# reilabs/gnark-whir

Measured on AMD Instinct MI355X. Metric: Groth16 proofs/sec for WHIR-verifier circuit (2^20 poly); G1 MSM pts/sec, higher is better.
Workload: dtype u32x8 Montgomery (BN254 Fr/Fp, exact modular integers)

## Files before the change

### gnark-whir_amd/binding.py

```python
from __future__ import annotations
import ctypes as C
import os
import numpy as np

_HERE = os.path.dirname(os.path.abspath(__file__))
LIB_PATH = os.environ.get("MI355X_GROTH16_LIB", os.path.join(_HERE, "libmi355x_groth16.so"))
_LIB = None

EXPORTS = [
    "mi_init", "mi_init_prio", "mi_shutdown", "mi_last_error", "mi_set_stream", "mi_pk_load", "mi_pk_load_dev", "mi_pk_free",
    "mi_ntt", "mi_ntt_dev", "mi_compute_h", "mi_compute_h_dev", "mi_msm_g1", "mi_msm_g1_dev", "mi_msm_g2",
    "mi_msm_g2_dev", "mi_groth16_prove", "mi_groth16_prove_dev", "mi_get_stats", "mi_g1_compress",
    "mi_g2_compress", "mi_proof_write", "mi_g1_sum", "mi_g2_sum", "mi_gen_scalars_dev", "mi_gen_g1_dev",
    "mi_gen_g2_dev", "mi_field_op_dev", "mi_debug_limb29_op_dev", "mi_debug_lazy_op_dev", "mi_debug_field_shape_dev", "mi_debug_pairing_dev", "mi_debug_fp12_op_dev", "mi_debug_decode_g1_dev", "mi_debug_decode_g2_dev", "mi_debug_hash_to_field_dev", "mi_debug_witness_decode_dev", "mi_debug_fp12_product_dev", "mi_debug_g1_scale128_dev", "mi_debug_g1_sum_tree_dev", "mi_debug_locate_points_dev", "mi_debug_locate_colsums_dev", "mi_debug_set_locate_round_nodes", "mi_g1_add_dev", "mi_g2_add_dev", "mi_bench_modmul_dev", "mi_bench_valu_dev", "mi_bench_gather_dev",
    "mi_dev_alloc", "mi_dev_free", "mi_dev_upload", "mi_dev_download", "mi_dev_sync",
    "mi_msm_precompute_g1_dev", "mi_msm_precompute_g2_dev", "mi_msm_g1_fixed_dev", "mi_msm_g2_fixed_dev", "mi_msm_table_to_rprime_g1_dev", "mi_msm_table_to_rprime_g2_dev", "mi_pk_table_plan",
    "mi_batch_scalar_mul_g1", "mi_batch_scalar_mul_g1_dev", "mi_batch_scalar_mul_g2", "mi_batch_scalar_mul_g2_dev",
    "mi_pedersen_pk_load", "mi_pedersen_pk_free", "mi_pedersen_commit", "mi_pedersen_prove_knowledge", "mi_pedersen_fold",
    "mi_debug_set_prove_fixed_base", "mi_debug_set_prove_schedule", "mi_debug_set_msm_batch_affine", "mi_debug_set_msm_group_bits", "mi_debug_inject_hip_failure", "mi_debug_set_ntt_plan", "mi_debug_set_ntt_threads", "mi_debug_set_ntt_wave_stages",
    "mi_debug_set_msm_plan", "mi_debug_set_msm_chunk", "mi_debug_set_msm_one_pass_sort", "mi_debug_set_msm_bound_levels", "mi_debug_set_msm_limb29", "mi_debug_set_msm_l1_waves", "mi_debug_set_msm_precompute_batched", "mi_debug_set_ntt_fuse_pair", "mi_debug_set_knob", "mi_debug_get_counter", "mi_debug_set_stream_plan", "mi_debug_set_trace_ranges", "mi_set_trace_ranges",
    "mi_prover_create", "mi_prover_destroy", "mi_prover_in_flight", "mi_prover_ctx", "mi_prover_last_error",
    "mi_prover_submit", "mi_prover_submit_dev", "mi_prover_wait", "mi_prover_commit", "mi_prover_submit_bsb22", "mi_prover_trim", "mi_ctx_trim",
    "mi_group_create", "mi_group_unique_id", "mi_group_create_rank", "mi_group_create_rank_ex", "mi_group_rank", "mi_group_destroy", "mi_group_world", "mi_group_local", "mi_group_ctx",
    "mi_group_last_error", "mi_group_transport", "mi_group_comm_ranks", "mi_group_device_pci", "mi_group_set_lead_share", "mi_group_wire_range", "mi_group_set_sharded_compute_h", "mi_compute_h_sharded_dev", "mi_groth16_prove_sharded_slices_dev", "mi_group_exchange_selftest", "mi_pk_load_sharded", "mi_pk_sharded_free",
    "mi_groth16_prove_sharded", "mi_groth16_prove_sharded_dev", "mi_pk_load_sharded_dev", "mi_msm_g1_sharded", "mi_msm_g2_sharded",
    "mi_msm_g1_sharded_dev", "mi_msm_g2_sharded_dev",
    "mi_pk_raw_inspect", "mi_pk_load_raw",
    "mi_whir_proof_decode", "mi_whir_proof_free", "mi_whir_proof_elements", "mi_whir_proof_statement_values", "mi_whir_element_shape", "mi_whir_parse_paths",
    "mi_whir_reverse", "mi_whir_prefix_decode_path", "mi_whir_limbs_to_fr", "mi_whir_interner_decode", "mi_whir_matrix_cells", "mi_whir_config_parse", "mi_whir_config_free",
]

SETUP_EXPORTS = ["mi_groth16_setup", "mi_groth16_setup_exponents", "mi_groth16_setup_get_stats"]
MAX_COMMITMENTS = 16
R1CS_EXPORTS = ["mi_r1cs_load", "mi_r1cs_free", "mi_r1cs_bytes", "mi_r1cs_eval", "mi_r1cs_eval_dev", "mi_r1cs_check_dev", "mi_r1cs_get_stats",
                "mi_groth16_prove_w", "mi_groth16_prove_w_dev", "mi_prover_submit_w", "mi_prover_submit_w_dev", "mi_prover_submit_w_bsb22"]
R1CS_A, R1CS_B, R1CS_C = 1, 2, 4
PROVE_W_EVAL_C = 1
VERIFY_EXPORTS = ["mi_vk_load", "mi_vk_free", "mi_pedersen_vk_make", "mi_groth16_verify", "mi_groth16_verify_batch"]
VERIFY_OK, VERIFY_PAIRING, VERIFY_PEDERSEN, VERIFY_MALFORMED = 0, 1, 2, 3
PAIRING_FINAL_EXP = 1
VERIFY_BYTES_EXPORTS = ["mi_vk_set_public_committed", "mi_groth16_verify_bytes", "mi_groth16_verify_bytes_batch", "mi_proof_read", "mi_hash_to_field"]
VERIFY_COMBINED_EXPORTS = ["mi_groth16_verify_combined", "mi_groth16_verify_bytes_combined"]
VERIFY_LOCATE_EXPORTS = ["mi_groth16_verify_locate", "mi_groth16_verify_bytes_locate"]
KEYFILE_EXPORTS = ["mi_g1_decompress_dev", "mi_g2_decompress_dev", "mi_g1_compress_dev", "mi_g2_compress_dev", "mi_pk_stream_inspect", "mi_pk_load_stream",
                   "mi_keyfile_get_stats", "mi_pk_stream_size", "mi_pk_write_dev", "mi_groth16_setup_to_stream"]
KEYFILE_RAW, KEYFILE_COMPRESSED = 0, 1
KEYFILE_NO_SUBGROUP_CHECK, KEYFILE_SUBGROUP_BY_R = 1, 2
NO_BAD_INDEX = (1 << 64) - 1
VKFILE_EXPORTS = ["mi_vk_stream_inspect", "mi_vk_stream_size", "mi_vk_write", "mi_vk_load_stream", "mi_groth16_setup_to_streams",
                  "mi_public_witness_write", "mi_public_witness_read", "mi_groth16_verify_files", "mi_groth16_verify_files_batch",
                  "mi_groth16_verify_files_combined", "mi_groth16_verify_files_locate"]
PHASE2_EXPORTS = ["mi_phase2_init", "mi_phase2_contribute", "mi_phase2_seal", "mi_phase2_to_streams", "mi_phase2_free", "mi_phase2_get_stats",
                  "mi_phase2_get_array"]
PHASE2_G1_A, PHASE2_G1_B, PHASE2_G2_B, PHASE2_G1_K, PHASE2_G1_Z, PHASE2_VK_K, PHASE2_BASIS = 0, 1, 2, 3, 4, 5, 6
PHASE2_CHECK_EXPORTS = ["mi_srs_check_powers", "mi_srs_check_get_stats", "mi_phase2_set_transcript_id", "mi_phase2_contribute_proved",
                        "mi_phase2_records_verify", "mi_phase2_verify_adopt", "mi_phase2_verify_get_stats"]
SRS_BAD_GENERATORS, SRS_BAD_TAU_G1, SRS_BAD_ALPHA_G1, SRS_BAD_BETA_G1, SRS_BAD_TAU_G2, SRS_BAD_BETA_G2 = 1, 2, 4, 8, 16, 32
PHASE2_BAD_RECORD, PHASE2_BAD_DELTA, PHASE2_BAD_Z, PHASE2_BAD_K = 1, 2, 4, 8
PHASE2_RECORD_WORDS = 24


class PkDesc(C.Structure):
    _fields_ = [
        ("log_n", C.c_uint32), ("nb_public", C.c_uint32), ("nb_wires", C.c_uint64),
        ("g1_a", C.c_void_p), ("n_g1_a", C.c_uint64), ("g1_b", C.c_void_p), ("n_g1_b", C.c_uint64),
        ("g1_k", C.c_void_p), ("n_g1_k", C.c_uint64), ("g1_z", C.c_void_p), ("n_g1_z", C.c_uint64),
        ("g2_b", C.c_void_p), ("n_g2_b", C.c_uint64),
        ("alpha1", C.c_uint64 * 8), ("beta1", C.c_uint64 * 8), ("delta1", C.c_uint64 * 8),
        ("beta2", C.c_uint64 * 16), ("delta2", C.c_uint64 * 16),
        ("infinity_a", C.c_void_p), ("infinity_b", C.c_void_p),
        ("committed_wires", C.c_void_p), ("n_committed", C.c_uint64),
    ]

# ... 202 lines not shown
    d.n_commitments = 0 if ped is None else int(ped.shape[0])
    d.ped = None if ped is None else ped.ctypes.data
    off = idx = None
    if lists is not None:
        off = np.cumsum([0] + [len(l) for l in lists]).astype(np.uint32)
        idx = np.array([j for l in lists for j in l], np.uint32)
        d.pc_offsets = off.ctypes.data
        d.pc_indices = idx.ctypes.data if len(idx) else None
    return d, (k, ped, off, idx)


def vk_stream_size(n_k, n_commitments=0, n_indices=0, encoding=KEYFILE_COMPRESSED):
    d = VkFileDesc(); d.n_k, d.n_commitments = int(n_k), int(n_commitments)
    off = np.array([0] * int(n_commitments) + [int(n_indices)], np.uint32); d.pc_offsets = off.ctypes.data
    n = C.c_size_t()
    if load().mi_vk_stream_size(C.byref(d), C.c_uint32(encoding), C.byref(n)) != 0:
        raise MiError("mi_vk_stream_size refused its arguments")
    return int(n.value)


def public_witness_write(values, cap=None) -> bytes:
    v = _u64(values).reshape(-1, 4); n = v.shape[0]
    cap = 12 + 32 * n if cap is None else cap
    out = (C.c_uint8 * max(cap, 1))(); need = C.c_size_t()
    if load().mi_public_witness_write(_p(v) if n else None, C.c_size_t(n), out, C.c_size_t(cap), C.byref(need)) != 0:
        raise MiError(f"mi_public_witness_write: MI_EINVAL ({need.value} bytes needed)")
    return C.string_at(out, need.value)


def public_witness_read(data: bytes, cap=None):
    buf = (C.c_uint8 * max(len(data), 1)).from_buffer_copy(data or b"\0")
    cap = max((len(data) - 12) // 32, 0) if cap is None else cap
    out = np.zeros((max(cap, 1), 4), np.uint64); n = C.c_size_t()
    if load().mi_public_witness_read(buf, C.c_size_t(len(data)), _p(out), C.c_size_t(cap), C.byref(n)) != 0:
        raise MiError("mi_public_witness_read: MI_EINVAL")
    return out[:int(n.value)].copy()


class VerifyLocateStats(C.Structure):
    _fields_ = [("rounds", C.c_uint32), ("nodes_tested", C.c_uint64), ("judged_alone", C.c_uint64), ("malformed", C.c_uint64), ("rejected", C.c_uint64)]

    def as_dict(self):
        return {n: int(getattr(self, n)) for n, _ in self._fields_}


class Bsb22Input(C.Structure):
    _fields_ = [("key", C.c_void_p), ("values", C.c_void_p), ("n", C.c_size_t)]


class Stats(C.Structure):
    _fields_ = [(n, C.c_float) for n in ("h2d_ms", "compute_h_ms", "filter_ms", "msm_a_ms", "msm_b1_ms", "msm_k_ms",
                                         "msm_z_ms", "msm_b2_ms", "assemble_ms", "total_ms")] + [
        ("g1_accum_kernel_ms", C.c_float), ("g1_accum_pairs", C.c_uint64), ("g1_accum_launches", C.c_uint32),
        ("ntt_kernel_ms", C.c_float), ("ntt_elems", C.c_uint64), ("ntt_launches", C.c_uint32), ("g1_accum_entries", C.c_uint64), ("g1_level1_additions", C.c_uint64)]

    def as_dict(self):
        return {n: getattr(self, n) for n, _ in self._fields_}


class MiError(RuntimeError):
    pass


def load():
    global _LIB
    if _LIB is None:
        if not os.path.exists(LIB_PATH):
            raise MiError(f"{LIB_PATH} missing: run `python -c 'import __graft_entry__ as g; g.build()'`")
        _LIB = C.CDLL(LIB_PATH)
        _LIB.mi_last_error.restype = C.c_char_p
        _LIB.mi_proof_write.restype = C.c_size_t
        _LIB.mi_prover_last_error.restype = C.c_char_p
        _LIB.mi_prover_ctx.restype = C.c_void_p
        _LIB.mi_prover_in_flight.restype = C.c_uint32
        _LIB.mi_group_ctx.restype = C.c_void_p
        _LIB.mi_group_last_error.restype = C.c_char_p
    return _LIB


DIST_UNIFORM, DIST_WHIR = 0, 1


def dist_mix(bit_pm, byte_pm, u64_pm=0):
    assert 0 <= bit_pm and 0 <= byte_pm and 0 <= u64_pm and bit_pm + byte_pm + u64_pm <= 1000
    return 0x40000000 | (bit_pm << 20) | (byte_pm << 10) | u64_pm


def _p(a):
    if a is None:
        return None
    if isinstance(a, np.ndarray):
        return a.ctypes.data_as(C.c_void_p)
    return C.c_void_p(int(a))


def _u64(a):
    return np.ascontiguousarray(a, dtype=np.uint64)


class DevArray:

    def __init__(self, ctx, nbytes):
        self.ctx, self.nbytes = ctx, int(nbytes)
        ptr = C.c_void_p()
        ctx._ck(ctx.lib.mi_dev_alloc(ctx.h, C.c_size_t(self.nbytes), C.byref(ptr)))
        self.ptr = ptr.value

# ... 91 lines not shown
        recs = np.ascontiguousarray(recs, dtype=np.uint32).reshape(-1, 24); n = recs.shape[0]
        di = self.to_dev(recs); do = self.alloc(max(64 * n, 32))
        self._ck(self.lib.mi_debug_lazy_op_dev(self.h, C.c_int(op), _p(do.ptr), _p(di.ptr), C.c_size_t(n)))
        out = do.download((n, 16), np.uint32) if n else np.zeros((0, 16), np.uint32)
        di.free(); do.free()
        return out

    def field_shape(self, shape, recs):
        recs = np.ascontiguousarray(recs, dtype=np.uint32).reshape(-1, 32); n = recs.shape[0]
        di = self.to_dev(recs); do = self.alloc(max(128 * n, 32))
        self._ck(self.lib.mi_debug_field_shape_dev(self.h, C.c_int(shape), _p(do.ptr), _p(di.ptr), C.c_size_t(n)))
        out = do.download((n, 32), np.uint32) if n else np.zeros((0, 32), np.uint32)
        di.free(); do.free()
        return out

    def ec_add(self, a, b, g2=False):
        a, b = _u64(a), _u64(b); n = a.shape[0]
        da, db = self.to_dev(a), self.to_dev(b); do = self.alloc(a.nbytes)
        f = self.lib.mi_g2_add_dev if g2 else self.lib.mi_g1_add_dev
        self._ck(f(self.h, _p(do.ptr), _p(da.ptr), _p(db.ptr), C.c_size_t(n)))
        out = do.download(a.shape)
        for x in (da, db, do): x.free()
        return out

    def bench_modmul(self, field, n_threads, iters):
        s = self.alloc(1024 * 32); ms = C.c_float()
        self._ck(self.lib.mi_bench_modmul_dev(self.h, field, C.c_size_t(n_threads), C.c_uint32(iters), _p(s.ptr), C.byref(ms)))
        s.free(); return ms.value

    def bench_gather(self, table_ptr, n_entries, n_threads, iters):
        s = self.alloc(1024); ms = C.c_float()
        self._ck(self.lib.mi_bench_gather_dev(self.h, _p(table_ptr), C.c_size_t(n_entries), C.c_size_t(n_threads), C.c_uint32(iters), _p(s.ptr), C.byref(ms)))
        s.free(); return ms.value

    def bench_valu(self, kind, n_threads, iters):
        s = self.alloc(1024); ms = C.c_float()
        self._ck(self.lib.mi_bench_valu_dev(self.h, kind, C.c_size_t(n_threads), C.c_uint32(iters), _p(s.ptr), C.byref(ms)))
        s.free(); return ms.value

    def ntt(self, a, log_n, flags):
        a = _u64(a).copy(); self._ck(self.lib.mi_ntt(self.h, _p(a), C.c_uint32(log_n), C.c_uint32(flags))); return a

    def ntt_dev(self, dptr, log_n, flags):
        self._ck(self.lib.mi_ntt_dev(self.h, _p(dptr), C.c_uint32(log_n), C.c_uint32(flags)))

    def compute_h(self, log_n, a, b, c):
        h = np.zeros((1 << log_n, 4), np.uint64)
        a, b, c = _u64(a), _u64(b), (None if c is None else _u64(c))
        self._ck(self.lib.mi_compute_h(self.h, C.c_uint32(log_n), _p(a), _p(b), _p(c), C.c_size_t(a.shape[0]), _p(h)))
        return h

    def compute_h_dev(self, log_n, a, b, c, n_constraints, h):
        self._ck(self.lib.mi_compute_h_dev(self.h, C.c_uint32(log_n), _p(a), _p(b), _p(c), C.c_size_t(n_constraints), _p(h)))

    def msm_g1(self, pts, sc, flags=0):
        out = np.zeros(12, np.uint64); pts, sc = _u64(pts), _u64(sc)
        self._ck(self.lib.mi_msm_g1(self.h, _p(pts), _p(sc), C.c_size_t(pts.shape[0]), C.c_uint32(flags), _p(out))); return out

    def msm_g2(self, pts, sc, flags=0):
        out = np.zeros(24, np.uint64); pts, sc = _u64(pts), _u64(sc)
        self._ck(self.lib.mi_msm_g2(self.h, _p(pts), _p(sc), C.c_size_t(pts.shape[0]), C.c_uint32(flags), _p(out))); return out

    def msm_g1_dev(self, pts_ptr, sc_ptr, n, flags=0):
        out = np.zeros(12, np.uint64)
        self._ck(self.lib.mi_msm_g1_dev(self.h, _p(pts_ptr), _p(sc_ptr), C.c_size_t(n), C.c_uint32(flags), _p(out))); return out

    def msm_g2_dev(self, pts_ptr, sc_ptr, n, flags=0):
        out = np.zeros(24, np.uint64)
        self._ck(self.lib.mi_msm_g2_dev(self.h, _p(pts_ptr), _p(sc_ptr), C.c_size_t(n), C.c_uint32(flags), _p(out))); return out

    def msm_precompute(self, base_ptr, n, c, g2=False):
        nwin = (256 + c - 1) // c
        pre = self.alloc((128 if g2 else 64) * n * nwin)
        f = self.lib.mi_msm_precompute_g2_dev if g2 else self.lib.mi_msm_precompute_g1_dev
        self._ck(f(self.h, _p(base_ptr), C.c_size_t(n), C.c_uint32(c), _p(pre.ptr)))
        return pre

    def msm_table_to_rprime(self, pre_ptr, n_points, g2=False):
        f = self.lib.mi_msm_table_to_rprime_g2_dev if g2 else self.lib.mi_msm_table_to_rprime_g1_dev
        self._ck(f(self.h, _p(pre_ptr), C.c_size_t(n_points)))

    def pk_table_plan(self, pkh):
        c = (C.c_uint32 * 3)()
        self._ck(self.lib.mi_pk_table_plan(pkh, c))
        return tuple(int(x) for x in c)

    def msm_fixed_dev(self, pre_ptr, sc_ptr, n, c, flags=0, g2=False):
        out = np.zeros(24 if g2 else 12, np.uint64)
        f = self.lib.mi_msm_g2_fixed_dev if g2 else self.lib.mi_msm_g1_fixed_dev
        self._ck(f(self.h, _p(pre_ptr), _p(sc_ptr), C.c_size_t(n), C.c_uint32(c), C.c_uint32(flags), _p(out)))
        return out

    def pk_load(self, pk: dict, device_points=False):
        d = PkDesc(); keep = []
        d.log_n, d.nb_public, d.nb_wires = pk["log_n"], pk["nb_public"], pk["nb_wires"]
        for name in ("g1_a", "g1_b", "g1_k", "g1_z", "g2_b"):
            if device_points:
                ptr, cnt = pk[name]
                setattr(d, name, int(ptr)); setattr(d, "n_" + name, int(cnt))
            else:
                arr = _u64(pk[name]); keep.append(arr)
                setattr(d, name, arr.ctypes.data); setattr(d, "n_" + name, arr.shape[0])
        for name, k in (("alpha1", 8), ("beta1", 8), ("delta1", 8), ("beta2", 16), ("delta2", 16)):
            setattr(d, name, (C.c_uint64 * k)(*[int(v) for v in _u64(pk[name]).reshape(-1)]))
        ia = np.ascontiguousarray(pk["infinity_a"], dtype=np.uint8); ib = np.ascontiguousarray(pk["infinity_b"], dtype=np.uint8)
        keep += [ia, ib]
# ... 920 lines not shown
```

### gnark-whir_amd/csrc/ctx.h

```cpp
#pragma once
#include <hip/hip_runtime.h>
#include <atomic>
#include <functional>
#include <mutex>
#include <string>
#include <vector>
#include <cstdio>
#include "../../include/mi355x_groth16.h"
#include "../../include/mi355x_groth16_group.h"
#include "../../include/mi355x_whir_ingest.h"
#include "../../include/mi355x_groth16_debug.h"
#include "../../include/mi355x_groth16_setup.h"
#include "../../include/mi355x_groth16_r1cs.h"
#include "../../include/mi355x_groth16_keyfile.h"
#include "../../include/mi355x_groth16_phase2.h"
#include "../../include/mi355x_groth16_phase2_check.h"

struct DevBuf {
    void *p = nullptr;
    size_t cap = 0;
};

enum {
    WS_H_B = 0,
    WS_H_C = 1,
    WS_HOST_IO0 = 2,
    WS_HOST_IO1 = 3,
    WS_FB_SUMS = 4,
    WS_FB_INV = 5,
    WS_R1CS_A = 6,
    WS_R1CS_B = 7,
    WS_R1CS_C = 8,
    WS_R1CS_PARTIAL = 9,
    WS_R1CS_CHECK = 10,
    WS_R1CS_W = 11,
    WS_SCAN = 12,
    WS_VERIFY = 13,
    WS_H = 14,
    WS_VERIFY_BYTES = 15,
    WS_PROVE_IN = 16,
    WS_B_WIRES = 17,
    WS_VERIFY_LOCATE = 18,
    WS_POK_VALUES = 19,
    WS_FB_TABLE = 20,
    WS_FB_SCALARS = 21,
    WS_FB_OUT = 22,
    WS_RPRIME = 23,
    WS_COUNT = 24
};
enum {
    EV_T0 = 0,
    EV_T1 = 1,
    EV_W_READY = 2,
    EV_H_READY = 3,
    EV_PROVE_BEGIN = 11,
    EV_R1CS_BEGIN = 12,
    EV_R1CS_END = 13,
    EV_COUNT = 24
};

enum {
    MSM_SLOT_A = 0,
    MSM_SLOT_B1 = 1,
    MSM_SLOT_B2 = 2,
    MSM_SLOT_K = 3,
    MSM_SLOT_Z = 4,
    MSM_SLOT_POK = 5,
    MI_MSM_SLOTS = 6
};
#define MI_ZHOOK_SLOT MSM_SLOT_Z
enum {
    MSM_EV_SORT_DONE = 0,
    MSM_EV_L1_BEGIN = 1,
    MSM_EV_L1_END = 2,
    MSM_EV_JOB_BEGIN = 3,
    MSM_EV_JOB_END = 4,
    MSM_EV_BUCKETS = 5,
    MSM_EV_MAX_LANDED = 6,
    MSM_EV_COUNT = 7
};
enum { B_DIGITS, B_H, B_S, B_SORTED, B_LEVELS, B_PART0, B_PART1, B_BUCKET, B_SCAN, B_WIN, B_PVAL, B_C1, B_CHUNKS, B_ITEMTAB, B_MAX, B_BA_NODES, B_BA_PREFIX, B_BA_TOT, B_COUNT_ };
struct MsmHostWords {
    unsigned char wsum[128][256];
    uint32_t entries, pad0_[3];
    uint32_t exact_total, pad1_[3];
    uint32_t max_bucket, pad2_[7];
};
static_assert(offsetof(MsmHostWords, entries) == sizeof(MsmHostWords::wsum) && offsetof(MsmHostWords, exact_total) == offsetof(MsmHostWords, entries) + 16 &&
              offsetof(MsmHostWords, max_bucket) == offsetof(MsmHostWords, entries) + 32 && sizeof(MsmHostWords) == 128 * 256 + 64, "the words lie where the kernels store them");
struct MsmSlot {
    hipStream_t stream = nullptr;
    hipEvent_t ev[MSM_EV_COUNT]{};
    bool max_pending = false;
    uint32_t max_key_count = 0;
    DevBuf buf[B_COUNT_];
    MsmHostWords *host_wsum = nullptr;
    uint32_t n = 0, c = 0, G = 0;
    uint64_t entries_cap = 0;
    uint64_t stat_pairs = 0;
    uint32_t nwin_keys = 0;
    uint32_t nwin_digits = 0;
    bool active = false, timed = false;
    bool deferred = false;
    uint32_t tail_seg = 0;
    const uint32_t *entries_src = nullptr;
    const std::function<hipEvent_t()> *accum_gate = nullptr;
};

struct mi_ctx {
    int dev = 0;
    hipStream_t stream = nullptr;
    bool own_stream = false;
    hipStream_t copy_stream = nullptr;
    std::string err;
    std::mutex err_m;
    mi_stats stats{};
    mi_setup_stats setup_stats{};
    mi_phase2_stats phase2_stats{};
    mi_srs_check_stats srs_check_stats{}, phase2_verify_stats{};
    mi_keyfile_stats keyfile_stats{};
    mi_r1cs_stats r1cs_stats{};
    bool r1cs_timed = false;
    hipEvent_t ev[EV_COUNT]{};
    alignas(16) unsigned char ntt_state[384];
    alignas(16) unsigned char msm_knobs[128];
    DevBuf ws[WS_COUNT];
    MsmSlot msm[MI_MSM_SLOTS];
    int cu_count = 256;
    int prio_scheme = 0;
    uint32_t fixed_knob[3] = {0, 0, 0};
    std::atomic<uint64_t> generic_sorts_two_pass{0}, generic_sorts_one_pass{0};
    std::atomic<uint64_t> dense_item_sorts{0};
    uint64_t z_count_fused_launches = 0;
    struct ZCountHook { bool armed = false, done = false; int slot = -1; uint32_t n = 0, c = 0; alignas(8) unsigned char shape[64]; uint32_t *C1 = nullptr; const void *h = nullptr;  } zhook;
    uint32_t locate_round_nodes = 0;
    uint32_t hold_accum = 0;
};

static_assert(sizeof(mi_ctx::ws) == WS_COUNT * sizeof(DevBuf) && WS_RPRIME == WS_COUNT - 1, "WS_* names every slot of mi_ctx::ws up to its end");
static_assert(EV_R1CS_END < EV_COUNT && sizeof(mi_ctx::ev) == EV_COUNT * sizeof(hipEvent_t), "EV_* index mi_ctx::ev");
static_assert(MSM_SLOT_POK == MI_MSM_SLOTS - 1 && sizeof(mi_ctx::msm) == MI_MSM_SLOTS * sizeof(MsmSlot) && MSM_EV_MAX_LANDED == MSM_EV_COUNT - 1 &&
              sizeof(MsmSlot::buf) == B_COUNT_ * sizeof(DevBuf), "MSM_SLOT_* name every slot of mi_ctx::msm, MSM_EV_* every event of a slot, B_* every workspace");

#include <atomic>
extern std::atomic<int> mi_fault_countdown;
static inline bool mi_fault_hit() {
    if (mi_fault_countdown.load(std::memory_order_relaxed) <= 0) return false;
    return mi_fault_countdown.fetch_sub(1, std::memory_order_relaxed) == 1;
}
static inline void mi_set_err(struct mi_ctx *ctx, const std::string &msg);
#define MI_CHECK_HIP(ctx, call)                                                                       \
    do {                                                                                              \
        hipError_t e__ = mi_fault_hit() ? hipErrorUnknown : (call);                                   \
        if (e__ != hipSuccess) {                                                                      \
                        \
            if (e__ == hipErrorOutOfMemory) (void)hipGetLastError();                                  \
            mi_set_err((ctx), std::string(#call) + ": " + hipGetErrorString(e__));                    \
            return e__ == hipErrorOutOfMemory ? MI_ENOMEM : MI_EHIP;                                  \
        }                                                                                             \
    } while (0)
#define MI_FAIL(ctx, code, msg)                                                                       \
    do {                                                                                              \
        mi_set_err((ctx), (msg));                                                                     \
        return (code);                                                                                \
    } while (0)
#define MI_TRY(expr)                                                                                  \
    do {                                                                                              \
        int32_t rc__ = (expr);                                                                        \
        if (rc__ != MI_OK) return rc__;                                                               \
    } while (0)

extern std::atomic<int> mi_ranges_on;
void mi_range_push(const char *name);
void mi_range_pop();
struct MiRange {
    bool on;
    explicit MiRange(const char *name) : on(mi_ranges_on.load(std::memory_order_relaxed) != 0) { if (on) mi_range_push(name); }
    ~MiRange() { if (on) mi_range_pop(); }
    MiRange(const MiRange &) = delete;
    MiRange &operator=(const MiRange &) = delete;
};
extern thread_local std::string *mi_err_sink;
static inline void mi_set_err(struct mi_ctx *ctx, const std::string &msg) {
    if (mi_err_sink) { *mi_err_sink = msg; return; }
    std::lock_guard<std::mutex> lk(ctx->err_m);
    ctx->err = msg;
}

static inline int32_t mi_reserve(mi_ctx *ctx, DevBuf &b, size_t bytes) {
    if (bytes <= b.cap) return MI_OK;
    if (b.p) { MI_CHECK_HIP(ctx, hipFree(b.p)); b.p = nullptr; b.cap = 0; }
    size_t want = bytes + bytes / 8 + 256;
    MI_CHECK_HIP(ctx, hipMalloc(&b.p, want));
    b.cap = want;
    return MI_OK;
}

static inline bool mi_try_reserve(DevBuf &b, size_t bytes) {
    if (bytes <= b.cap) return true;
    if (b.p) { (void)hipFree(b.p); b.p = nullptr; b.cap = 0; }
    const size_t want = bytes + bytes / 8 + 256;
    if (hipMalloc(&b.p, want) != hipSuccess) { (void)hipGetLastError(); b.p = nullptr; return false; }
    b.cap = want;
    return true;
}

static inline unsigned mi_blocks_of(uint64_t n, uint32_t per) { return (unsigned)((n + per - 1) / per); }

int32_t mi_copy_stream(mi_ctx *ctx, hipStream_t *out);
int32_t mi_ntt_dev_impl(mi_ctx *ctx, mi_fr *inout_dev, uint32_t log_n, uint32_t flags);
int32_t mi_compute_h_dev_impl(mi_ctx *ctx, uint32_t log_n, const mi_fr *a, const mi_fr *b, const mi_fr *c,
                              size_t n_constraints, mi_fr *h_out);
int32_t mi_compute_h_part(mi_ctx *ctx, uint32_t log_n, int part, const mi_fr *src, size_t n_constraints, mi_fr *h_out, const mi_fr *src2 = nullptr);
void mi_ntt_state_init(mi_ctx *ctx);
size_t mi_ntt_table_bytes(mi_ctx *ctx);
void mi_ntt_state_free(mi_ctx *ctx);
bool mi_ntt_set_knob(mi_ctx *ctx, const char *name, int64_t value);
void mi_ntt_state_trim(mi_ctx *ctx);
int32_t mi_msm_state_init(mi_ctx *ctx);
enum { MI_PRIO_SOLO = 0,
       MI_PRIO_POOL_FIRST = 1,
       MI_PRIO_POOL_SECOND = 2,
       MI_PRIO_POOL_REST = 3 };
void mi_msm_state_free(mi_ctx *ctx);
int32_t mi_msm_enqueue(mi_ctx *ctx, int slot, int sort_slot, int curve, const void *pts_dev, const void *scalars_dev, size_t n,
                       uint32_t flags, hipEvent_t wait_ev, bool timed, uint32_t precomp_c = 0, size_t stat_pairs = 0,
                       uint32_t generic_c = 0 );
int32_t mi_msm_precompute(mi_ctx *ctx, int curve, const void *base_dev, void *pre_dev, size_t n, uint32_t c);
int32_t mi_msm_finish(mi_ctx *ctx, int slot, int curve, void *out_xyzz_host);
int32_t mi_msm_z_count_arm(mi_ctx *ctx, int slot, size_t n, uint32_t c);
#define MI_MSM_DEFER_REDUCE 0x100u
#define MI_MSM_EXACT_SIZE 0x200u
#define MI_MSM_PTS_RPRIME 0x400u
struct MsmBucketView {
    void *bucket = nullptr;
    size_t nkeys = 0, xyzz_bytes = 0;
    uint32_t seg = 0, c = 0, nwin = 0;
    hipStream_t stream = nullptr;
    hipEvent_t ready = nullptr;
};
int32_t mi_msm_bucket_view(mi_ctx *ctx, int slot, int curve, MsmBucketView *v);
int32_t mi_msm_reduce_enqueue(mi_ctx *ctx, int slot, int curve);
bool mi_msm_limb29_enabled(mi_ctx *ctx);
uint32_t mi_msm_auto_c(size_t n);
const struct MsmCurveOps &mi_msm_ops(int curve);
```

### gnark-whir_amd/csrc/msm.hip

```cpp
#include "ctx.h"
#include "msm2_core.cuh"
#include "scan_u32.cuh"
#include "msm_curve_ops.h"
#include "key_plan.h"
#include <algorithm>
#include <cstring>
#include <cstdlib>
#include <new>

struct MsmKnobs {
    u32 c = 0, L1 = 0, L2 = 0, seg = 0, G = 0;
    u32 no_rprime = 0;
    u32 ba_rounds = 0;
    u32 l1_waves = 3;
    u32 precompute_unbatched = 0;
    u32 std_partials = 0;
    u32 one_pass_sort = 0;
    u32 chunk = 0;
    u32 gbits = 0;
    u32 bound_levels = 0;
    u32 l1_wg = 4;
    u32 g2_wg = 1;
    u32 z_waves = 0;
    u32 g1_grid_per_cu = 0, g2_grid_per_cu = 0;
// ... 212 lines not shown
__global__ void __launch_bounds__(64) k_msm_prep1_sums(MsmShape s, const u32 *S, u32 L, u32 *start, u32 *cnt, u32 *items, u32 *bucket, u32 bucket_words, u32 *block_sums) {
    size_t base = (size_t)blockIdx.x * SCAN_BLOCK + (size_t)threadIdx.x * SCAN_PER_THREAD;
    u32 sum = 0;
    for (u32 k = 0; k < SCAN_PER_THREAD; k++) {
        const u32 key = (u32)(base + k);
        if (base + k < s.nkeys) {
            msm_prep_level1(s, S, L, start, cnt, items, key);
            sum += items[key];
            if (cnt[key] == 0) {
                uint4 *b = reinterpret_cast<uint4 *>(bucket + (size_t)key * bucket_words);
                for (u32 q = 0; q < bucket_words / 4; q++) b[q] = make_uint4(0, 0, 0, 0);
            }
        }
    }
    if (blockIdx.x == 0 && threadIdx.x < 16) bucket[(size_t)s.nkeys * bucket_words + threadIdx.x] = 0;
    u32 total;
    wave_exclusive_scan(sum, &total);
    if (threadIdx.x == 0) block_sums[blockIdx.x] = total;
}
__global__ void __launch_bounds__(64) k_msm_finish_list(u32 nkeys, const u32 *items, u32 small_max, u32 *list_small, u32 *list_big, u32 *counters) {
    const u32 key = blockIdx.x * 64 + threadIdx.x, lane = threadIdx.x;
    const u32 c = key < nkeys ? items[key] : 0;
    const bool small = c > 1 && c <= small_max, big = c > small_max;
    const unsigned long long ms = __ballot(small), mb = __ballot(big), below = (1ull << lane) - 1;
    u32 base_s = 0, base_b = 0;
    if (lane == 0) {
        if (ms) base_s = atomicAdd(&counters[0], (u32)__popcll(ms));
        if (mb) base_b = atomicAdd(&counters[1], (u32)__popcll(mb));
    }
    base_s = (u32)__shfl((int)base_s, 0); base_b = (u32)__shfl((int)base_b, 0);
    if (small) list_small[base_s + (u32)__popcll(ms & below)] = key;
    if (big) list_big[base_b + (u32)__popcll(mb & below)] = key;
}
static u32 auto_c(u32 n) {
    u32 lg = 0;
    while ((2u << lg) <= n) lg++;
    int c = (int)lg - 4;
    if (c < 3) c = 3;
    if (c > 16) c = 16;
    return (u32)c;
}
static u32 msm_auto_seg(u32 nbuckets) { return nbuckets >= (1u << 16) ? 16u : nbuckets >= 256 ? 8u : 2u; }
static MsmShape slot_shape(const MsmSlot &sl) { return msm_shape(sl.n, sl.c, sl.G); }
static MsmShape key_shape(const MsmSlot &sl) {
    MsmShape s;
    s.c = sl.c; s.nwin = sl.nwin_keys; s.nbuckets = 1u << (sl.c - 1); s.nkeys = s.nwin * s.nbuckets; s.nslices = sl.G; s.n = sl.n;
    return s;
}

static std::atomic<int> g_stream_plan{1};
extern "C" int32_t mi_debug_get_counter(mi_ctx *ctx, const char *name, uint64_t *out) {
    if (!ctx || !name || !out) return MI_EINVAL;
    if (!std::strcmp(name, "z_count_fused_launches")) { *out = ctx->z_count_fused_launches; return MI_OK; }
    if (!std::strcmp(name, "dense_item_sorts")) { *out = ctx->dense_item_sorts.load(); return MI_OK; }
    if (!std::strcmp(name, "generic_sorts_two_pass")) { *out = ctx->generic_sorts_two_pass.load(); return MI_OK; }
    if (!std::strcmp(name, "generic_sorts_one_pass")) { *out = ctx->generic_sorts_one_pass.load(); return MI_OK; }
    if (!std::strcmp(name, "hip_failure_countdown")) { const int v = mi_fault_countdown.load(); *out = v > 0 ? (uint64_t)v : 0; return MI_OK; }
    MI_FAIL(ctx, MI_EINVAL, std::string("unknown counter: ") + name);
}
extern "C" int32_t mi_debug_set_stream_plan(int32_t plan) {
    if (plan < 0 || plan > 2) return MI_EINVAL;
    g_stream_plan.store(plan);
    return MI_OK;
}
int32_t mi_msm_state_init(mi_ctx *ctx) {
    new (ctx->msm_knobs) MsmKnobs();
    (void)hipFuncSetAttribute((const void *)k_msm_hist, hipFuncAttributeMaxDynamicSharedMemorySize, 160 * 1024);
    (void)hipFuncSetAttribute((const void *)k_msm_scatter, hipFuncAttributeMaxDynamicSharedMemorySize, 160 * 1024);
    (void)hipFuncSetAttribute((const void *)k_msm2_hist2, hipFuncAttributeMaxDynamicSharedMemorySize, 160 * 1024);
#define MI_PART_LDS(C) (void)hipFuncSetAttribute((const void *)k_msm2_partition<C>, hipFuncAttributeMaxDynamicSharedMemorySize, 160 * 1024)
    for (u32 c = 15; c <= 22; c++) { MSM2_FOR_C(c, MI_PART_LDS) }
#undef MI_PART_LDS
    (void)hipFuncSetAttribute((const void *)k_msm2_scatter2, hipFuncAttributeMaxDynamicSharedMemorySize, 160 * 1024);
    (void)hipFuncSetAttribute((const void *)k_msm2_scatter2_staged, hipFuncAttributeMaxDynamicSharedMemorySize, 160 * 1024);
    int prio_lo = 0, prio_hi = 0;
    (void)hipDeviceGetStreamPriorityRange(&prio_lo, &prio_hi);
    const int plan = g_stream_plan.load();
    for (int idx = 0; idx < MI_MSM_SLOTS; idx++) {
        if (plan >= 1 && idx == MSM_SLOT_K) continue;
        if (plan >= 2 && idx == MSM_SLOT_B1) continue;
        MsmSlot &sl = ctx->msm[idx];
        int pw = 0, pz = prio_lo;
        if (ctx->prio_scheme == MI_PRIO_POOL_FIRST) { pw = prio_hi; pz = 0; }
        if (ctx->prio_scheme == MI_PRIO_POOL_REST) pw = pz = prio_lo;
        MI_CHECK_HIP(ctx, hipStreamCreateWithPriority(&sl.stream, hipStreamNonBlocking, idx == MSM_SLOT_Z ? pz : pw));
    }
    if (ctx->msm[MSM_SLOT_K].stream) (void)hipStreamDestroy(ctx->msm[MSM_SLOT_K].stream);
    if (plan >= 2) ctx->msm[MSM_SLOT_B1].stream = ctx->msm[MSM_SLOT_A].stream;
    ctx->msm[MSM_SLOT_K].stream = ctx->msm[MSM_SLOT_B1].stream;
    for (auto &sl : ctx->msm) {
        for (auto &e : sl.ev) MI_CHECK_HIP(ctx, hipEventCreate(&e));
        MI_CHECK_HIP(ctx, hipHostMalloc(&sl.host_wsum, sizeof(MsmHostWords)));
    }
    return MI_OK;
}
void mi_msm_state_free(mi_ctx *ctx) {
    for (int i = 0; i < MI_MSM_SLOTS; i++) for (int j = i + 1; j < MI_MSM_SLOTS; j++) if (ctx->msm[j].stream == ctx->msm[i].stream) ctx->msm[j].stream = nullptr;
    for (auto &sl : ctx->msm) {
        if (sl.stream) { (void)hipStreamSynchronize(sl.stream); (void)hipStreamDestroy(sl.stream); }
        for (auto &e : sl.ev) if (e) (void)hipEventDestroy(e);
        if (sl.host_wsum) (void)hipHostFree(sl.host_wsum);
        for (auto &b : sl.buf) if (b.p) (void)hipFree(b.p);
    }
}

__global__ void __launch_bounds__(256) k_max_u32(const u32 *v, u32 n, u32 *out) {
// ... 76 lines not shown
        MI_CHECK_HIP(ctx, hipGetLastError());
        if (p.time_first && level == 0) MI_CHECK_HIP(ctx, hipEventRecord(sl.ev[MSM_EV_L1_END], st));
        const u64 m_next = (m + a.L - 1) / a.L;
        if (m_next <= 1) break;
        const MsmKnobs *kn = knobs_of(ctx);
        if (kn->finisher && ops.finish_keys && m_next <= (kn->finisher_max ? kn->finisher_max : ops.finish_max) && level >= kn->finisher_min_level) {
            u32 *counters = (u32 *)((char *)p.final_out + (size_t)nkeys * ops.xyzz_bytes);
            hipLaunchKernelGGL(k_msm_finish_list, dim3((nkeys + 63) / 64), dim3(64), 0, st, nkeys, cur.items, MSM_FIN_SMALL, nxt.start, nxt.cnt, counters);
            const u32 nb_small = std::min((nkeys + ops.finish_T - 1) / ops.finish_T, (u32)ctx->cu_count * 8), nb_big = std::min(nkeys, (u32)ctx->cu_count * 4);
            ops.finish_keys(st, nb_small, nb_big, a.partial_out, nxt.start, nxt.cnt, counters, cur.item_start, cur.items, p.final_out, l1.form.rp_partials ? 1u : 0u);
            MI_CHECK_HIP(ctx, hipGetLastError());
            break;
        }
        const bool fused = scan_blocks <= SCAN_MAX_INLINE_BLOCKS;
        if (fused) {
            MI_TRY(mi_reserve(ctx, sl.buf[B_SCAN], (size_t)(scan_blocks + 1) * 4));
            hipLaunchKernelGGL(k_msm_prep_next_sums, dim3(scan_blocks), dim3(SCAN_THREADS), 0, st, nkeys, cur.items, cur.item_start, p.L_next, nxt.start, nxt.cnt, nxt.items, (u32 *)sl.buf[B_SCAN].p);
        } else {
            hipLaunchKernelGGL(k_msm_prep_next, dim3((nkeys + 63) / 64), dim3(64), 0, st, nkeys, cur.items, cur.item_start, p.L_next, nxt.start, nxt.cnt, nxt.items);
            MI_CHECK_HIP(ctx, hipGetLastError());
        }
        MI_TRY(exclusive_scan(ctx, st, nxt.items, nkeys, nxt.item_start, sl.buf[B_SCAN], nullptr, nullptr, nullptr, fused));
        u64 nb = items_bound / p.L_next + (items_bound < nkeys ? items_bound : nkeys) + 1;
        items_bound = nb < items_bound ? nb : items_bound;
        m = m_next; a.L = p.L_next; a.partial_in = a.partial_out;
        LevelArrays t = cur; cur = nxt; nxt = t;
    }
    return MI_OK;
}

static int32_t msm2_sort_enqueue(mi_ctx *ctx, MsmSlot &sl, const Fr *scalars, u32 n, u32 flags, u32 c, bool wkeys = false, bool exact = false);
static int32_t msm_sort_enqueue(mi_ctx *ctx, MsmSlot &sl, const Fr *scalars, u32 n, u32 flags, u32 generic_c, bool exact) {
    MsmKnobs *kn = knobs_of(ctx);
    sl.n = n;
    sl.c = kn->c ? kn->c : (generic_c >= 2 && generic_c <= 16 ? generic_c : auto_c(n));
    if (sl.c == 16 && !kn->one_pass_sort && n >= (1u << 18) && (u64)n * 16 < ((u64)1 << 31)) {
        ctx->generic_sorts_two_pass++;
        return msm2_sort_enqueue(ctx, sl, scalars, n, flags, 16, true, exact);
    }
    ctx->generic_sorts_one_pass++;
    sl.G = kn->G ? kn->G : (n / 8192 > 64 ? 64 : (n / 8192 ? n / 8192 : 1));
    const MsmShape s = slot_shape(sl);
    sl.nwin_keys = sl.nwin_digits = s.nwin;
    const u64 T_bound = (u64)s.nwin * n;
    sl.entries_cap = T_bound;
    if (s.nwin > 128) MI_FAIL(ctx, MI_EINVAL, "msm: too many windows");
    MI_TRY(mi_reserve(ctx, sl.buf[B_DIGITS], T_bound * 2 + 64));
    MI_TRY(mi_reserve(ctx, sl.buf[B_H], ((size_t)s.nkeys * s.nslices + 1) * 4));
    MI_TRY(mi_reserve(ctx, sl.buf[B_S], ((size_t)s.nkeys * 2 + 2) * 4));
    MI_TRY(mi_reserve(ctx, sl.buf[B_SORTED], (T_bound + 1) * 4));
    int16_t *digits = (int16_t *)sl.buf[B_DIGITS].p;
    u32 *H = (u32 *)sl.buf[B_H].p, *keystart = (u32 *)sl.buf[B_S].p, *total = keystart + s.nkeys + 1, *sorted = (u32 *)sl.buf[B_SORTED].p;
    hipStream_t st = sl.stream;
    hipLaunchKernelGGL(k_msm_digits, dim3((n + 255) / 256), dim3(256), 0, st, s, scalars, (flags & MI_MSM_SCALARS_CANONICAL) ? 0 : 1, digits);
    const size_t lds_bytes = (size_t)s.nbuckets * 4;
    hipLaunchKernelGGL(k_msm_hist, dim3(s.nslices, s.nwin), dim3(1024), lds_bytes, st, s, digits, H);
    MI_CHECK_HIP(ctx, hipGetLastError());
    hipLaunchKernelGGL(k_msm_colsum, dim3((s.nkeys + 255) / 256), dim3(256), 0, st, s, H, total);
    MI_CHECK_HIP(ctx, hipGetLastError());
    MI_TRY(fetch_max_and_scan_keys(ctx, sl, total, s.nkeys, keystart, true));
    hipLaunchKernelGGL(k_msm_scatter, dim3(s.nslices, s.nwin), dim3(1024), lds_bytes, st, s, digits, keystart, H, sorted);
    MI_CHECK_HIP(ctx, hipGetLastError());
    MI_CHECK_HIP(ctx, hipEventRecord(sl.ev[MSM_EV_SORT_DONE], st));
    return MI_OK;
}

static Msm2Shape msm2_plan_shape(const MsmKnobs *kn, u32 n, u32 c, bool wkeys) {
    const u32 G = n ? (n + MSM2_SLICE - 1) / MSM2_SLICE : 1;
    const u32 chunk = kn->chunk ? kn->chunk : 8192;
    u32 gbits = kn->gbits ? kn->gbits : 11;
    if (gbits > 15) gbits = 15;
    const u32 keys_total = (wkeys ? msm_nwin(c) : 1u) << (c - 1);
    while ((keys_total >> gbits) > MSM2_MAX_GROUPS) gbits++;
    return msm2_shape(n, c, G, chunk, gbits, wkeys ? 1u : 0u);
}
int32_t mi_msm_z_count_arm(mi_ctx *ctx, int slot, size_t n, uint32_t c) {
    static_assert(sizeof(Msm2Shape) <= sizeof(ctx->zhook.shape), "Msm2Shape travels in ctx->zhook.shape");
    ctx->zhook.armed = ctx->zhook.done = false; ctx->zhook.h = nullptr;
    const MsmKnobs *kn = knobs_of(ctx);
    if (!kn->z_count_fused || slot != MSM_SLOT_Z || c < 17 || c > 22 || n < MSM2_SLICE || n > ((size_t)1 << 27)) return MI_OK;
    const Msm2Shape s = msm2_plan_shape(kn, (u32)n, c, false);
    if ((u64)s.nwin * n >= ((u64)1 << 31) || (n + s.nslices - 1) / s.nslices != MSM2_SLICE) return MI_OK;
    MsmSlot &sl = ctx->msm[slot];
    MI_TRY(mi_reserve(ctx, sl.buf[B_C1], ((size_t)s.ngroups * s.nslices + 1) * 4 * 2));
    std::memcpy(ctx->zhook.shape, &s, sizeof(s));
    ctx->zhook.slot = slot; ctx->zhook.n = (u32)n; ctx->zhook.c = c; ctx->zhook.C1 = (u32 *)sl.buf[B_C1].p;
    ctx->zhook.armed = true;
    return MI_OK;
}
static int32_t msm2_sort_enqueue(mi_ctx *ctx, MsmSlot &sl, const Fr *scalars, u32 n, u32 flags, u32 c, bool wkeys, bool exact) {
    MsmKnobs *kn = knobs_of(ctx);
    if (!wkeys && (c < 17 || c > 22)) MI_FAIL(ctx, MI_EINVAL, "fixed-base msm: window bits must be 17..22");
    const Msm2Shape s = msm2_plan_shape(kn, n, c, wkeys);
    const u32 G = s.nslices, chunk = s.chunk;
    sl.n = n; sl.c = c; sl.G = G; sl.nwin_keys = wkeys ? s.nwin : 1; sl.nwin_digits = s.nwin;
    const u64 T_bound = (u64)s.nwin * n;
    if (T_bound >= ((u64)1 << 31)) MI_FAIL(ctx, MI_EINVAL, "fixed-base msm: windows * n must stay below 2^31");
    MI_TRY(mi_reserve(ctx, sl.buf[B_C1], ((size_t)s.ngroups * G + 1) * 4 * 2));
    MI_TRY(mi_reserve(ctx, sl.buf[B_CHUNKS], ((size_t)s.ngroups + 1) * 4 * 3));
    MI_TRY(mi_reserve(ctx, sl.buf[B_S], ((size_t)s.nkeys * 2 + 2) * 4));
    u32 *C1 = (u32 *)sl.buf[B_C1].p, *S1 = C1 + (size_t)s.ngroups * G + 1;
    const int mont = (flags & MI_MSM_SCALARS_CANONICAL) ? 0 : 1;
    hipStream_t st = sl.stream;
    u32 per = kn->count_per >= 1 && kn->count_per <= 64 ? kn->count_per : 32u;
    while (per > 1 && per * s.ngroups > 8192) per >>= 1;
    bool counted = false;
    if (&sl == &ctx->msm[MSM_SLOT_Z]) {
        counted = ctx->zhook.done && ctx->zhook.slot == MSM_SLOT_Z && ctx->zhook.n == n && ctx->zhook.c == c && ctx->zhook.C1 == C1 && ctx->zhook.h == (const void *)scalars && mont && !wkeys;
        ctx->zhook.done = false;
    }
    if (!counted) {
#define MI_LAUNCH_COUNT(C) hipLaunchKernelGGL(k_msm2_count<C>, dim3((G + per - 1) / per), dim3(512), 0, st, s, scalars, mont, per, C1)
    MSM2_FOR_C(s.c, MI_LAUNCH_COUNT)
#undef MI_LAUNCH_COUNT
    }
    MI_CHECK_HIP(ctx, hipGetLastError());
    u32 *host_total = &sl.host_wsum->exact_total;
    MI_TRY(exclusive_scan(ctx, st, C1, (size_t)s.ngroups * G, S1, sl.buf[B_SCAN], exact ? host_total : nullptr));
    u64 T = T_bound;
    if (exact) {
        MI_CHECK_HIP(ctx, hipStreamSynchronize(st));
        T = *host_total;
        if (T > T_bound) MI_FAIL(ctx, MI_EHIP, "msm: counted more entries than windows * n");
    }
    sl.entries_cap = T;
    const u32 chunks_bound = (u32)(T / chunk) + s.ngroups + 1;
    MI_TRY(mi_reserve(ctx, sl.buf[B_DIGITS], T * 2 + 64));
    MI_TRY(mi_reserve(ctx, sl.buf[B_PVAL], (T + 1) * 4));
    MI_TRY(mi_reserve(ctx, sl.buf[B_H], (size_t)chunks_bound * s.gsize * 4));
    MI_TRY(mi_reserve(ctx, sl.buf[B_SORTED], (T + 1) * 4));
    uint16_t *part_lo = (uint16_t *)sl.buf[B_DIGITS].p;
    u32 *part_val = (u32 *)sl.buf[B_PVAL].p, *gstart = (u32 *)sl.buf[B_CHUNKS].p, *cstart = gstart + s.ngroups + 1, *nchunks = cstart + s.ngroups + 1;
    u32 *H2 = (u32 *)sl.buf[B_H].p, *keystart = (u32 *)sl.buf[B_S].p, *total = keystart + s.nkeys + 1, *sorted = (u32 *)sl.buf[B_SORTED].p;
    const u32 cap = ((n + G - 1) / G) * s.nwin;
    const size_t part_lds = ((size_t)3 * s.ngroups + 1 + 256 + cap) * 4 + (size_t)cap * 2 * 2;
    if (part_lds > 160 * 1024) MI_FAIL(ctx, MI_EINVAL, "fixed-base msm: pass-1 slice does not fit in LDS");
#define MI_LAUNCH_PART(C) hipLaunchKernelGGL(k_msm2_partition<C>, dim3(((G + 7) / 8) * 8), dim3(MSM2_PART_THREADS), part_lds, st, s, scalars, mont, S1, cap, part_lo, part_val)
    MSM2_FOR_C(s.c, MI_LAUNCH_PART)
#undef MI_LAUNCH_PART
    MI_TRY(mi_reserve(ctx, sl.buf[B_MAX], 64));
    const u32 key_blocks = (s.nkeys + SCAN_BLOCK - 1) / SCAN_BLOCK;
    const bool fuse_keys = key_blocks > 1 && key_blocks <= SCAN_MAX_INLINE_BLOCKS;
    MI_TRY(mi_reserve(ctx, sl.buf[B_SCAN], (size_t)(key_blocks + 1) * 4));
    u32 *key_bs = (u32 *)sl.buf[B_SCAN].p;
    hipLaunchKernelGGL(k_msm2_chunk_count_scan, dim3(1), dim3(64), 0, st, s, S1, gstart, nchunks, cstart, (u32 *)sl.buf[B_MAX].p, key_bs, fuse_keys ? key_blocks : 0u);
    MI_CHECK_HIP(ctx, hipGetLastError());
    hipLaunchKernelGGL(k_msm2_hist2, dim3(chunks_bound), dim3(1024), s.gsize * 4, st, s, gstart, cstart, part_lo, H2);
    hipLaunchKernelGGL(k_msm2_colsum, dim3((s.nkeys + 63) / 64), dim3(64), 0, st, s, cstart, H2, total, (u32 *)sl.buf[B_MAX].p, fuse_keys ? key_bs : nullptr);
    MI_CHECK_HIP(ctx, hipGetLastError());
    MI_TRY(fetch_max_and_scan_keys(ctx, sl, total, s.nkeys, keystart, false, fuse_keys));
    const bool plain_scatter = kn->plain_scatter != 0;
    const size_t staged_lds = ((size_t)2 * s.gsize + 16 + chunk) * 4 + (size_t)chunk * 2;
    if (!plain_scatter && chunk <= MSM2_STAGE_PER * 1024 && staged_lds <= 80 * 1024)
        hipLaunchKernelGGL(k_msm2_scatter2_staged, dim3(chunks_bound + 8), dim3(1024), staged_lds, st, s, gstart, cstart, keystart, H2, part_lo, part_val, sorted);
    else
        hipLaunchKernelGGL(k_msm2_scatter2, dim3(chunks_bound + 8), dim3(1024), s.gsize * 4, st, s, gstart, cstart, keystart, H2, part_lo, part_val, sorted);
    MI_CHECK_HIP(ctx, hipGetLastError());
    MI_CHECK_HIP(ctx, hipEventRecord(sl.ev[MSM_EV_SORT_DONE], st));
    return MI_OK;
}

static int32_t msm_tail_enqueue(mi_ctx *ctx, const MsmCurveOps &ops, MsmSlot &acc);
static int32_t msm_accum_enqueue(mi_ctx *ctx, const MsmCurveOps &ops, MsmSlot &srt, MsmSlot &acc, const void *pts, bool timed, bool defer_reduce, bool rprime) {
// ... 284 lines not shown
int32_t mi_msm_table_to_rprime_g1_dev(mi_ctx *ctx, mi_g1_affine *pre_dev, size_t n_points) { return table_to_rprime(ctx, 1, pre_dev, n_points); }
int32_t mi_msm_table_to_rprime_g2_dev(mi_ctx *ctx, mi_g2_affine *pre_dev, size_t n_points) { return table_to_rprime(ctx, 2, pre_dev, n_points); }
int32_t mi_msm_g1_fixed_dev(mi_ctx *ctx, const mi_g1_affine *pre_dev, const mi_fr *scalars_dev, size_t n, uint32_t c, uint32_t flags, mi_g1_jac *out) {
    if (!ctx || !out || ((!pre_dev || !scalars_dev) && n) || (flags & ~3u)) return MI_EINVAL;
    return msm_fixed_dev_entry<Fp>(ctx, 1, pre_dev, scalars_dev, n, c, flags, out);
}
int32_t mi_msm_g2_fixed_dev(mi_ctx *ctx, const mi_g2_affine *pre_dev, const mi_fr *scalars_dev, size_t n, uint32_t c, uint32_t flags, mi_g2_jac *out) {
    if (!ctx || !out || ((!pre_dev || !scalars_dev) && n) || (flags & ~3u)) return MI_EINVAL;
    return msm_fixed_dev_entry<Fp2>(ctx, 2, pre_dev, scalars_dev, n, c, flags, out);
}
int32_t mi_debug_set_msm_limb29(mi_ctx *ctx, uint32_t on) {
    if (!ctx || on > 2) return MI_EINVAL;
    knobs_of(ctx)->no_rprime = on ? 0 : 1;
    knobs_of(ctx)->std_partials = on == 2 ? 1 : 0;
    return MI_OK;
}
int32_t mi_debug_set_msm_precompute_batched(mi_ctx *ctx, uint32_t on) {
    if (!ctx || on > 1) return MI_EINVAL;
    knobs_of(ctx)->precompute_unbatched = on ? 0 : 1;
    return MI_OK;
}
int32_t mi_debug_set_msm_batch_affine(mi_ctx *ctx, uint32_t rounds) {
    if (!ctx || rounds > 4) return MI_EINVAL;
    knobs_of(ctx)->ba_rounds = rounds;
    return MI_OK;
}
int32_t mi_debug_set_msm_l1_waves(mi_ctx *ctx, uint32_t waves) {
    if (!ctx || (waves != 2 && waves != 3)) return MI_EINVAL;
    knobs_of(ctx)->l1_waves = waves;
    return MI_OK;
}
int32_t mi_debug_set_knob(mi_ctx *ctx, const char *name, int64_t value) {
    if (!ctx || !name) return MI_EINVAL;
    MsmKnobs *k = knobs_of(ctx);
    const auto is = [name](const char *n) { return std::strcmp(name, n) == 0; };
    const bool wg_ok = value == 1 || value == 2 || value == 4;
    if (is("l1_wg") && wg_ok) k->l1_wg = (u32)value;
    else if (is("g2_wg") && wg_ok) k->g2_wg = (u32)value;
    else if (is("l1_waves") && (value == 2 || value == 3)) k->l1_waves = (u32)value;
    else if (is("z_waves") && (value == 0 || value == 2)) k->z_waves = (u32)value;
    else if (is("g1_grid_per_cu") && value >= 0 && value <= 65536) k->g1_grid_per_cu = (u32)value;
    else if (is("g2_grid_per_cu") && value >= 0 && value <= 65536) k->g2_grid_per_cu = (u32)value;
    else if (is("count_per") && value >= 0 && value <= 64) k->count_per = (u32)value;
    else if (is("plain_scatter") && (value == 0 || value == 1)) k->plain_scatter = (u32)value;
    else if (is("z_count_fused") && (value == 0 || value == 1)) k->z_count_fused = (u32)value;
    else if (is("flat_item_l1") && (value == 0 || value == 1 || (value >= 4 && value <= 64))) k->flat_L1 = (u32)value;
    else if (is("dense_item_l1") && (value == 0 || value == 1 || (value >= 4 && value <= 64))) k->dense_L1 = (u32)value;
    else if (is("finisher") && (value == 0 || value == 1)) k->finisher = (u32)value;
    else if (is("finisher_max") && value >= 0 && value <= (1 << 20)) k->finisher_max = (u32)value;
    else if (is("item_l1") && (value == 0 || (value >= 2 && value <= 64))) k->L1 = (u32)value;
    else if (is("item_l2") && (value == 0 || (value >= 2 && value <= 64))) k->L2 = (u32)value;
    else if (is("reduce_seg") && value >= 0 && value <= 256) k->seg = (u32)value;
    else if (is("hold_accum") && (value == 0 || value == 1)) ctx->hold_accum = (uint32_t)value;
    else if (is("finisher_min_level") && value >= 0 && value <= 16) k->finisher_min_level = (u32)value;
    else if (mi_ntt_set_knob(ctx, name, value)) return MI_OK;
    else MI_FAIL(ctx, MI_EINVAL, std::string("mi_debug_set_knob: unknown knob or value out of range: ") + name);
    return MI_OK;
}
int32_t mi_debug_set_msm_bound_levels(mi_ctx *ctx, uint32_t on) {
    if (!ctx || on > 1) return MI_EINVAL;
    knobs_of(ctx)->bound_levels = on;
    return MI_OK;
}
int32_t mi_debug_set_msm_one_pass_sort(mi_ctx *ctx, uint32_t on) {
    if (!ctx || on > 1) return MI_EINVAL;
    knobs_of(ctx)->one_pass_sort = on;
    return MI_OK;
}
int32_t mi_debug_set_msm_chunk(mi_ctx *ctx, uint32_t chunk) {
    if (!ctx) return MI_EINVAL;
    knobs_of(ctx)->chunk = chunk;
    return MI_OK;
}
int32_t mi_debug_set_msm_group_bits(mi_ctx *ctx, uint32_t gbits) {
    if (!ctx || (gbits && (gbits < 6 || gbits > 15))) return MI_EINVAL;
    knobs_of(ctx)->gbits = gbits;
    return MI_OK;
}
int32_t mi_debug_set_msm_plan(mi_ctx *ctx, uint32_t c, uint32_t L1, uint32_t L2, uint32_t seg, uint32_t G) {
    if (!ctx || c == 1 || c > 16 || G > 1024 || L1 == 1 || L2 == 1) return MI_EINVAL;
    MsmKnobs *k = knobs_of(ctx);
    k->c = c; k->L1 = L1; k->L2 = L2; k->seg = seg; k->G = G;
    return MI_OK;
}
int32_t mi_debug_set_prove_schedule(mi_ctx *ctx, uint32_t hold_accum) {
    if (!ctx || hold_accum > 1) return MI_EINVAL;
    ctx->hold_accum = hold_accum;
    return MI_OK;
}
int32_t mi_debug_set_prove_fixed_base(mi_ctx *ctx, uint32_t c_ak, uint32_t c_b, uint32_t c_z) {
    if (!ctx) return MI_EINVAL;
    for (uint32_t c : {c_ak, c_b, c_z}) if (c > 1 && (c < 17 || c > 22)) return MI_EINVAL;
    ctx->fixed_knob[0] = c_ak; ctx->fixed_knob[1] = c_b; ctx->fixed_knob[2] = c_z;
    return MI_OK;
}
int32_t mi_msm_g1(mi_ctx *ctx, const mi_g1_affine *pts, const mi_fr *scalars, size_t n, uint32_t flags, mi_g1_jac *out) {
    return msm_host_entry<Fp>(ctx, 1, pts, scalars, n, flags, out);
}
int32_t mi_msm_g2(mi_ctx *ctx, const mi_g2_affine *pts, const mi_fr *scalars, size_t n, uint32_t flags, mi_g2_jac *out) {
    return msm_host_entry<Fp2>(ctx, 2, pts, scalars, n, flags, out);
}
int32_t mi_msm_g1_dev(mi_ctx *ctx, const mi_g1_affine *pts_dev, const mi_fr *scalars_dev, size_t n, uint32_t flags, mi_g1_jac *out) {
    if (!ctx || !out || ((!pts_dev || !scalars_dev) && n) || (flags & ~1u)) return MI_EINVAL;
    return msm_dev_entry<Fp>(ctx, 1, pts_dev, scalars_dev, n, flags, out);
}
int32_t mi_msm_g2_dev(mi_ctx *ctx, const mi_g2_affine *pts_dev, const mi_fr *scalars_dev, size_t n, uint32_t flags, mi_g2_jac *out) {
// ... 5 lines not shown
```

### gnark-whir_amd/csrc/ntt.hip

```cpp
#include "ctx.h"
#include "ntt_wave.cuh"
#include "msm2_core.cuh"
#include <cstring>
#include <cstdlib>

struct NttState {
    u32 log_n = 0xffffffffu;
    Fr *small_f = nullptr, *small_i = nullptr, *tw64k_f = nullptr, *tw64k_i = nullptr;
    Fr *tw_lo_f = nullptr, *tw_hi_f = nullptr, *tw_lo_i = nullptr, *tw_hi_i = nullptr;
    Fr *g_lo = nullptr, *g_hi = nullptr, *gi_lo = nullptr, *gi_hi = nullptr, *ninv = nullptr;
    Fr *g_hi_n = nullptr, *gi_hi_nd = nullptr;
    Fr *ninv_den = nullptr;
    u32 tw_h = 0;
    Fr *d_tw_inv = nullptr, *d_tw_fwd = nullptr, *d_sc_fwd = nullptr, *d_sc_inv = nullptr;
    u32 d_log_n = 0xffffffffu, d_log_r0 = 0, d_npass = 0;
    u32 direct_min_log_n = 12;
    u32 log_e = 9, max_contig = 9, max_strided = 7, threads = 256;
    u32 lds_floor = 0;
    u32 plan_set = 0;
    u32 wave_stages = 1;
    u32 fuse_pair = 1;
    u32 fuse_triple = 1;
    u32 fuse_last = 1;
};
struct NttKnobs { u32 log_e, max_contig, max_strided; };
static NttKnobs knobs_for(const struct NttState *st, u32 log_n);
static NttState *state_of(mi_ctx *ctx) {
    static_assert(sizeof(NttState) <= 384, "NttState lives in ctx->ntt_state");
    return reinterpret_cast<NttState *>(ctx->ntt_state);
}

__global__ void k_ntt_pass(Fr *dst, const Fr *src, NttPass p, NttTables t);
__global__ void k_ntt_pass_wave(Fr *dst, const Fr *src, NttPass p, NttTables t);
__global__ void k_ntt_contig_pair(Fr *data, NttPass pi, NttTables ti, NttPass pf, NttTables tf);
__global__ void k_ntt_strided_triple(Fr *a, const Fr *b, NttPass pc, NttTables tc, NttPass pl, NttTables tl);
__global__ void k_ntt_strided_triple8(Fr *a, const Fr *b, NttPass pc, NttTables tc, NttPass pl, NttTables tl);
__global__ void k_ntt_contig_last_sub(Fr *A, const Fr *Cin, NttPass pa, NttTables ta, NttPass pc, NttTables tc);
template <int CC> __global__ void k_ntt_contig_last_sub_count(Fr *A, const Fr *Cin, NttPass pa, NttTables ta, NttPass pc, NttTables tc, Msm2Shape zs, u32 *C1);
void mi_ntt_state_init(mi_ctx *ctx) {
    static_assert(sizeof(NttState) <= sizeof(ctx->ntt_state), "NttState lives in ctx->ntt_state");
    new (ctx->ntt_state) NttState();
    (void)hipFuncSetAttribute((const void *)k_ntt_pass, hipFuncAttributeMaxDynamicSharedMemorySize, 160 * 1024);
    (void)hipFuncSetAttribute((const void *)k_ntt_pass_wave, hipFuncAttributeMaxDynamicSharedMemorySize, 160 * 1024);
    (void)hipFuncSetAttribute((const void *)k_ntt_contig_pair, hipFuncAttributeMaxDynamicSharedMemorySize, 160 * 1024);
    (void)hipFuncSetAttribute((const void *)k_ntt_strided_triple, hipFuncAttributeMaxDynamicSharedMemorySize, 160 * 1024);
    (void)hipFuncSetAttribute((const void *)k_ntt_strided_triple8, hipFuncAttributeMaxDynamicSharedMemorySize, 160 * 1024);
    (void)hipFuncSetAttribute((const void *)k_ntt_contig_last_sub, hipFuncAttributeMaxDynamicSharedMemorySize, 160 * 1024);
    (void)hipFuncSetAttribute((const void *)k_ntt_contig_last_sub_count<17>, hipFuncAttributeMaxDynamicSharedMemorySize, 160 * 1024);
    (void)hipFuncSetAttribute((const void *)k_ntt_contig_last_sub_count<18>, hipFuncAttributeMaxDynamicSharedMemorySize, 160 * 1024);
    (void)hipFuncSetAttribute((const void *)k_ntt_contig_last_sub_count<19>, hipFuncAttributeMaxDynamicSharedMemorySize, 160 * 1024);
    (void)hipFuncSetAttribute((const void *)k_ntt_contig_last_sub_count<20>, hipFuncAttributeMaxDynamicSharedMemorySize, 160 * 1024);
    (void)hipFuncSetAttribute((const void *)k_ntt_contig_last_sub_count<21>, hipFuncAttributeMaxDynamicSharedMemorySize, 160 * 1024);
    (void)hipFuncSetAttribute((const void *)k_ntt_contig_last_sub_count<22>, hipFuncAttributeMaxDynamicSharedMemorySize, 160 * 1024);
}
bool mi_ntt_set_knob(mi_ctx *ctx, const char *name, int64_t value) {
    if (!std::strcmp(name, "ntt_lds_floor_kb") && value >= 0 && value <= 160) { state_of(ctx)->lds_floor = (u32)value * 1024u; return true; }
    return false;
}
void mi_ntt_state_free(mi_ctx *ctx) {
    NttState *st = state_of(ctx);
    Fr **all[] = {&st->small_f, &st->small_i, &st->tw64k_f, &st->tw64k_i, &st->g_hi_n, &st->gi_hi_nd, &st->tw_lo_f, &st->tw_hi_f, &st->tw_lo_i, &st->tw_hi_i,
                  &st->g_lo, &st->g_hi, &st->gi_lo, &st->gi_hi, &st->ninv, &st->ninv_den, &st->d_tw_inv, &st->d_tw_fwd, &st->d_sc_fwd, &st->d_sc_inv};
    for (Fr **p : all) if (*p) { (void)hipFree(*p); *p = nullptr; }
}

void mi_ntt_state_trim(mi_ctx *ctx) {
    mi_ntt_state_free(ctx);
    NttState *st = state_of(ctx);
    st->log_n = 0xffffffffu; st->d_log_n = 0xffffffffu; st->d_log_r0 = 0; st->d_npass = 0;
}
size_t mi_ntt_table_bytes(mi_ctx *ctx) {
    const NttState *st = state_of(ctx);
    size_t b = 0;
    if (st->small_f) b += (size_t)(2 * 2048 + 2 * 65536) * sizeof(Fr);
    if (st->log_n != 0xffffffffu) {
        const size_t nlo = (size_t)1 << st->tw_h, nhi = (size_t)1 << (st->log_n - st->tw_h);
        b += (4 * nlo + 6 * nhi + 2) * sizeof(Fr);
    }
    for (const Fr *p : {st->d_tw_inv, st->d_tw_fwd, st->d_sc_fwd, st->d_sc_inv}) if (p) b += sizeof(Fr) << st->d_log_n;
    return b;
}

static NttKnobs knobs_for(const NttState *st, u32 log_n) {
    if (st->plan_set) return NttKnobs{st->log_e, st->max_contig, st->max_strided};
    if (log_n == 24) return NttKnobs{10, 8, 8};
    if (log_n >= 25) return NttKnobs{10, 10, 8};
    return NttKnobs{st->log_e, st->max_contig, st->max_strided};
}

__global__ void k_pow_table(Fr *out, u32 count, Fr base, Fr c, u32 shift) {
    u32 j = blockIdx.x * blockDim.x + threadIdx.x;
    if (j >= count) return;
    u64 e = (u64)j << shift;
    Fr acc = c, b = base;
    while (e) {
        if (e & 1) acc = acc * b;
        b = fe_sqr(b);
        e >>= 1;
    }
    out[j] = acc;
}

__global__ void __launch_bounds__(1024) k_ntt_pass(Fr *dst, const Fr *src, NttPass p, NttTables t) {
    extern __shared__ U4 lds[];
    const u64 tile = blockIdx.x;
    ntt_tile_load(p, t, src, tile, threadIdx.x, blockDim.x, lds);
    __syncthreads();
    for (u32 s = 0; s < p.log_r; s++) {
        ntt_tile_stage(p, t, s, threadIdx.x, blockDim.x, lds);
        __syncthreads();
    }
    ntt_tile_store(p, t, dst, tile, threadIdx.x, blockDim.x, lds);
}

#ifndef MI_NTT_WAVES_PER_EU
#define MI_NTT_WAVES_PER_EU 1
#endif
__global__ void __launch_bounds__(256, MI_NTT_WAVES_PER_EU) k_ntt_pass_wave(Fr *dst, const Fr *src, NttPass p, NttTables t) {
    extern __shared__ U4 lds[];
    const u64 tile = blockIdx.x;
    const u32 PL = ntt_plane_slots(p);
    ntt_tile_load(p, t, src, tile, threadIdx.x, blockDim.x, lds);
    __syncthreads();
    if (!p.dit)
        for (u32 s = 0; s + 7 < p.log_r; s++) {
            ntt_tile_stage(p, t, s, threadIdx.x, blockDim.x, lds);
            __syncthreads();
        }
    const u32 lane = threadIdx.x & 63, wave = threadIdx.x >> 6, nwaves = blockDim.x >> 6;
    const u32 nsub = 1u << (p.log_r + p.log_c - 7);
    for (u32 sb = wave; sb < nsub; sb += nwaves) {
        const u32 col = sb & ((1u << p.log_c) - 1), base = (sb >> p.log_c) << 7;
// ... 97 lines not shown
    reg_stages(pc, true, tc.small);
    __syncthreads();
#pragma unroll
    for (u32 k = 0; k < 2; k++) {
        if (k >= nb) break;
        const u32 bf = threadIdx.x + 256 * k, col = bf & (C - 1), j = bf >> pc.log_c;
        Fr x = lds_get(lds, PL, ntt_lds_slot(pc, j, col));
        Fr y = lds_get(lds, PL, ntt_lds_slot(pc, j + 128, col));
        ntt_bfly_dit(x, y, j ? &tc.small[j << 4] : nullptr);
        keep[2 * k] = x; keep[2 * k + 1] = y;
    }
    __syncthreads();
    ntt_tile_load(pc, tc, b, tile, threadIdx.x, blockDim.x, lds);
    __syncthreads();
    reg_stages(pc, true, tc.small);
    __syncthreads();
#pragma unroll
    for (u32 k = 0; k < 2; k++) {
        if (k >= nb) break;
        const u32 bf = threadIdx.x + 256 * k, col = bf & (C - 1), j = bf >> pc.log_c;
        Fr x = lds_get(lds, PL, ntt_lds_slot(pc, j, col));
        Fr y = lds_get(lds, PL, ntt_lds_slot(pc, j + 128, col));
        ntt_bfly_dit(x, y, j ? &tc.small[j << 4] : nullptr);
        Fr p0 = ntt_mul_lazy2(x, keep[2 * k]), p1 = ntt_mul_lazy2(y, keep[2 * k + 1]);
        ntt_bfly_dif(p0, p1, j ? &tl.small[j << 4] : nullptr);
        lds_put(lds, PL, ntt_lds_slot(pl, j, col), p0);
        lds_put(lds, PL, ntt_lds_slot(pl, j + 128, col), p1);
    }
    __syncthreads();
    reg_stages(pl, false, tl.small);
    __syncthreads();
    ntt_tile_store(pl, tl, a, tile, threadIdx.x, blockDim.x, lds);
}

__device__ __forceinline__ void ntt_wave_pass_to_lds(const NttPass &p, const NttTables &t, const Fr *src, u64 tile, U4 *lds) {
    const u32 PL = ntt_plane_slots(p);
    ntt_tile_load(p, t, src, tile, threadIdx.x, blockDim.x, lds);
    __syncthreads();
    for (u32 s = 0; s + 7 < p.log_r; s++) {
        ntt_tile_stage(p, t, s, threadIdx.x, blockDim.x, lds);
        __syncthreads();
    }
    const u32 lane = threadIdx.x & 63, wave = threadIdx.x >> 6, nwaves = blockDim.x >> 6;
    const u32 nsub = 1u << (p.log_r + p.log_c - 7);
    for (u32 sb = wave; sb < nsub; sb += nwaves) {
        const u32 col = sb & ((1u << p.log_c) - 1), base = (sb >> p.log_c) << 7;
        Fr x0 = lds_get(lds, PL, ntt_lds_slot(p, base + lane, col)), x1 = lds_get(lds, PL, ntt_lds_slot(p, base + lane + 64, col));
        wave_ntt128(x0, x1, lane, false, t.small);
        lds_put(lds, PL, ntt_lds_slot(p, base + 2 * lane, col), x0);
        lds_put(lds, PL, ntt_lds_slot(p, base + 2 * lane + 1, col), x1);
    }
    __syncthreads();
}
template <int CC>
__device__ __forceinline__ void ntt_contig_last_sub_body(Fr *A, const Fr *Cin, const NttPass &pa, const NttTables &ta, const NttPass &pc, const NttTables &tc,
                                                         const Msm2Shape &zs, u32 *C1) {
    extern __shared__ U4 lds[];
    const u64 tile = blockIdx.x;
    const u32 E = 1u << (pa.log_r + pa.log_c), PL = ntt_plane_slots(pa);
    u32 *cnt = reinterpret_cast<u32 *>(lds + 2 * PL);
    const u32 nsl = E / MSM2_SLICE;
    if (CC >= 0) for (u32 k = threadIdx.x; k < nsl * zs.ngroups; k += blockDim.x) cnt[k] = 0;
    Fr keep[4];
    ntt_wave_pass_to_lds(pc, tc, Cin, tile, lds);
#pragma unroll
    for (u32 k = 0; k < 4; k++) {
        const u32 e = threadIdx.x + k * blockDim.x;
        if (e >= E) break;
        const u32 rho = e & ((1u << pc.log_r) - 1), col = e >> pc.log_r;
        Fr v = lds_get(lds, PL, ntt_lds_slot(pc, rho, col)), f;
        if (ntt_edge_factor(pc, tc, rho, ntt_global_index(pc, tile, rho, col), 1, f)) v = fe_mul_lazy(v, f);
        keep[k] = v;
    }
    __syncthreads();
    ntt_wave_pass_to_lds(pa, ta, A, tile, lds);
#pragma unroll
    for (u32 k = 0; k < 4; k++) {
        const u32 e = threadIdx.x + k * blockDim.x;
        if (e >= E) break;
        const u32 rho = e & ((1u << pa.log_r) - 1), col = e >> pa.log_r;
        const u64 g = ntt_global_index(pa, tile, rho, col);
        Fr v = lds_get(lds, PL, ntt_lds_slot(pa, rho, col)), f;
        if (ntt_edge_factor(pa, ta, rho, g, 1, f)) v = fe_mul_lazy(v, f);
        const Fr hv = fe_canon(fe_sub_plus2p(fe_condsub_2p(v), fe_condsub_2p(keep[k])));
        A[g] = hv;
        if (CC >= 0 && g < zs.n) {
            Msm2Digits dg;
            dg.start(hv, true);
            msm2_count_one<(CC >= 0 ? (u32)CC : 0u)>(zs, dg, cnt + (e / MSM2_SLICE) * zs.ngroups);
        }
    }
    if (CC >= 0) {
        __syncthreads();
        const u32 s0 = (u32)tile * nsl;
        for (u32 k = threadIdx.x; k < nsl * zs.ngroups; k += blockDim.x) {
            const u32 j = k / zs.ngroups, gq = k % zs.ngroups;
            if (s0 + j < zs.nslices) C1[(size_t)gq * zs.nslices + s0 + j] = cnt[k];
        }
    }
}
__global__ void __launch_bounds__(256) k_ntt_contig_last_sub(Fr *A, const Fr *Cin, NttPass pa, NttTables ta, NttPass pc, NttTables tc) {
    ntt_contig_last_sub_body<-1>(A, Cin, pa, ta, pc, tc, Msm2Shape{}, nullptr);
}
template <int CC>
__global__ void __launch_bounds__(256) k_ntt_contig_last_sub_count(Fr *A, const Fr *Cin, NttPass pa, NttTables ta, NttPass pc, NttTables tc, Msm2Shape zs, u32 *C1) {
    ntt_contig_last_sub_body<CC>(A, Cin, pa, ta, pc, tc, zs, C1);
}

__global__ void k_tw_layout(Fr *out, u32 log_n, u32 log_r, Fr w) {
    const u32 g = blockIdx.x * blockDim.x + threadIdx.x;
    if (g >= (1u << log_n)) return;
    const u32 log_s = log_n - log_r;
    u32 e = (g & ((1u << log_s) - 1)) * bitrev_u32(g >> log_s, log_r);
    Fr acc = Fr::one(), b = w;
    while (e) { if (e & 1) acc = acc * b; b = fe_sqr(b); e >>= 1; }
    out[g] = acc;
}
__global__ void k_sc_layout(Fr *out, u32 log_n, Fr base, Fr c) {
    const u32 i = blockIdx.x * blockDim.x + threadIdx.x;
    if (i >= (1u << log_n)) return;
    u32 e = bitrev_u32(i, log_n);
    Fr acc = c, b = base;
    while (e) { if (e & 1) acc = acc * b; b = fe_sqr(b); e >>= 1; }
    out[i] = acc;
}

static int32_t build_table(mi_ctx *ctx, Fr **slot, u32 count, const Fr &base, const Fr &c, u32 shift) {
    if (*slot) { MI_CHECK_HIP(ctx, hipFree(*slot)); *slot = nullptr; }
    MI_CHECK_HIP(ctx, hipMalloc((void **)slot, sizeof(Fr) * (count ? count : 1)));
    hipLaunchKernelGGL(k_pow_table, dim3((count + 127) / 128), dim3(128), 0, ctx->stream, *slot, count, base, c, shift);
    MI_CHECK_HIP(ctx, hipGetLastError());
    return MI_OK;
}

static int32_t ensure_tables(mi_ctx *ctx, u32 log_n) {
    NttState *st = state_of(ctx);
    if (!st->small_f) {
        Fr w4096 = fr_domain_generator(12);
        MI_TRY(build_table(ctx, &st->small_f, 2048, w4096, Fr::one(), 0));
        MI_TRY(build_table(ctx, &st->small_i, 2048, fe_inv(w4096), Fr::one(), 0));
        Fr w64k = fr_domain_generator(16);
        MI_TRY(build_table(ctx, &st->tw64k_f, 65536, w64k, Fr::one(), 0));
        MI_TRY(build_table(ctx, &st->tw64k_i, 65536, fe_inv(w64k), Fr::one(), 0));
    }
    if (st->log_n == log_n) return MI_OK;
    Fr w = fr_domain_generator(log_n), wi = fe_inv(w);
    Fr g = fe_from_u32<FrParams>(5), gi = fe_inv(g);
    Fr nn = Fr::zero();
    nn.l[0] = (u32)(1u << log_n);
    Fr ninv = fe_inv(fe_to_mont(nn));
    u32 h = (log_n + 1) / 2;
    u32 nlo = 1u << h, nhi = 1u << (log_n - h);
    st->tw_h = h;
    MI_TRY(build_table(ctx, &st->tw_lo_f, nlo, w, Fr::one(), 0));
    MI_TRY(build_table(ctx, &st->tw_hi_f, nhi, w, Fr::one(), h));
    MI_TRY(build_table(ctx, &st->tw_lo_i, nlo, wi, Fr::one(), 0));
    MI_TRY(build_table(ctx, &st->tw_hi_i, nhi, wi, Fr::one(), h));
    MI_TRY(build_table(ctx, &st->g_lo, nlo, g, Fr::one(), 0));
    MI_TRY(build_table(ctx, &st->g_hi, nhi, g, Fr::one(), h));
    MI_TRY(build_table(ctx, &st->gi_lo, nlo, gi, Fr::one(), 0));
    MI_TRY(build_table(ctx, &st->gi_hi, nhi, gi, ninv, h));
    MI_TRY(build_table(ctx, &st->ninv, 1, Fr::one(), ninv, 0));
    Fr gn = g;
    for (u32 k = 0; k < log_n; k++) gn = fe_sqr(gn);
    Fr den = fe_inv(gn - Fr::one());
    MI_TRY(build_table(ctx, &st->g_hi_n, nhi, g, ninv, h));
    MI_TRY(build_table(ctx, &st->gi_hi_nd, nhi, gi, ninv * den, h));
    MI_TRY(build_table(ctx, &st->ninv_den, 1, Fr::one(), ninv * den, 0));
    st->log_n = log_n;
    return MI_OK;
}

static int32_t ensure_direct(mi_ctx *ctx, u32 log_n) {
    NttState *st = state_of(ctx);
    const NttKnobs kn = knobs_for(st, log_n);
    const NttPlan pl = ntt_make_plan(log_n, kn.max_contig, kn.max_strided);
    if (st->d_log_n == log_n && st->d_log_r0 == pl.log_r[0] && st->d_npass == pl.n_pass) return MI_OK;
    Fr **four[] = {&st->d_tw_inv, &st->d_tw_fwd, &st->d_sc_fwd, &st->d_sc_inv};
    for (Fr **p : four) if (*p) { (void)hipFree(*p); *p = nullptr; }
    st->d_log_n = 0xffffffffu;
    if (log_n < st->direct_min_log_n) return MI_OK;
    MI_TRY(ensure_tables(ctx, log_n));
    const size_t bytes = sizeof(Fr) << log_n;
    for (Fr **p : four)
        if (hipMalloc((void **)p, bytes) != hipSuccess) {
            (void)hipGetLastError();
            for (Fr **q : four) if (*q) { (void)hipFree(*q); *q = nullptr; }
            return MI_OK;
        }
    const Fr w = fr_domain_generator(log_n), wi = fe_inv(w), g = fe_from_u32<FrParams>(5), gi = fe_inv(g);
    Fr nn = Fr::zero();
    nn.l[0] = (u32)(1u << log_n);
    const Fr ninv = fe_inv(fe_to_mont(nn));
    Fr gn = g;
    for (u32 k = 0; k < log_n; k++) gn = fe_sqr(gn);
    const Fr den = fe_inv(gn - Fr::one());
    const unsigned blocks = (unsigned)(((size_t)1 << log_n) + 255) / 256;
    if (pl.n_pass > 1) {
        hipLaunchKernelGGL(k_tw_layout, dim3(blocks), dim3(256), 0, ctx->stream, st->d_tw_inv, log_n, pl.log_r[0], wi);
        hipLaunchKernelGGL(k_tw_layout, dim3(blocks), dim3(256), 0, ctx->stream, st->d_tw_fwd, log_n, pl.log_r[0], w);
    }
    hipLaunchKernelGGL(k_sc_layout, dim3(blocks), dim3(256), 0, ctx->stream, st->d_sc_fwd, log_n, g, ninv);
    hipLaunchKernelGGL(k_sc_layout, dim3(blocks), dim3(256), 0, ctx->stream, st->d_sc_inv, log_n, gi, ninv * den);
    MI_CHECK_HIP(ctx, hipGetLastError());
    st->d_log_n = log_n; st->d_log_r0 = pl.log_r[0]; st->d_npass = pl.n_pass;
    return MI_OK;
}

static int32_t ntt_run(mi_ctx *ctx, Fr *dst, const Fr *src, u32 n_valid, u32 log_n, u32 flags, u32 variant = 0,
                       const Fr *load_mul = nullptr, const Fr *store_sub = nullptr, u32 skip = 0, NttPass *cap = nullptr, NttTables *cap_t = nullptr) {
    NttState *st = state_of(ctx);
    MI_TRY(ensure_tables(ctx, log_n));
    const bool inverse = flags & MI_NTT_INVERSE, coset = flags & MI_NTT_COSET, dit = flags & MI_NTT_DIT;
    NttTables t{};
    t.small = inverse ? st->small_i : st->small_f;
    t.tw_lo = inverse ? st->tw_lo_i : st->tw_lo_f;
    t.tw_hi = inverse ? st->tw_hi_i : st->tw_hi_f;
    t.tw_h = st->tw_h;
    t.tw_64k = inverse ? st->tw64k_i : st->tw64k_f;
    u32 load_scale = 0, store_scale = 0;
    if (coset && !inverse) { t.sc_lo = st->g_lo; t.sc_hi = variant == 2 ? st->g_hi_n : st->g_hi; load_scale = dit ? 1 : 2; }
    else if (coset && inverse) { t.sc_lo = st->gi_lo; t.sc_hi = variant == 3 ? st->gi_hi_nd : st->gi_hi; store_scale = dit ? 4 : 3; }
    else if (inverse && variant != 1) { t.sc_lo = t.sc_hi = variant == 4 ? st->ninv_den : st->ninv; store_scale = 5; }
    if (load_mul && (load_scale || dit)) MI_FAIL(ctx, MI_EINVAL, "internal: load_mul on a pass whose load side already has a factor");

    const NttKnobs kn = knobs_for(st, log_n);
    NttPlan pl = ntt_make_plan(log_n, kn.max_contig, kn.max_strided);
    u32 log_s[8];
    for (u32 i = 0, acc = log_n; i < pl.n_pass; i++) { acc -= pl.log_r[i]; log_s[i] = acc; }
    const Fr *cur_src = src;
    for (u32 step = 0; step < pl.n_pass; step++) {
        u32 i = dit ? pl.n_pass - 1 - step : step;
        NttPass p{};
        p.log_n = log_n; p.log_r = pl.log_r[i]; p.log_s = log_s[i];
        u32 room = kn.log_e > p.log_r ? kn.log_e - p.log_r : 0;
        u32 avail = p.log_s == 0 ? log_n - p.log_r : p.log_s;
        p.log_c = room < avail ? room : avail;
        p.dit = dit ? 1 : 0;
        p.twiddle = p.log_s != 0;
        p.scale = 0;
        if (step == 0 && load_scale) p.scale = load_scale;
        if (step == pl.n_pass - 1 && store_scale) {
            if (p.scale) MI_FAIL(ctx, MI_EINVAL, "internal: load and store scale on one pass");
            p.scale = store_scale;
        }
        p.n_valid = step == 0 ? n_valid : (1u << log_n);
        if (step == 0) p.load_mul = load_mul;
        if (step == pl.n_pass - 1) p.store_sub = store_sub;
        if (step == pl.n_pass - 1 && (variant == 0 || variant == 3)) p.canon = 1;
        const bool direct = variant != 0 && st->d_log_n == log_n && st->d_sc_fwd;
        if (direct && p.twiddle && i == 0 && pl.n_pass > 1) p.tw_direct = inverse ? st->d_tw_inv : st->d_tw_fwd;
        if (direct && variant == 2 && p.scale == 1) p.sc_direct = st->d_sc_fwd;
        if (direct && variant == 3 && p.scale == 3) p.sc_direct = st->d_sc_inv;
        const bool wave = p.log_r >= 7 && st->wave_stages;
        p.lds_pad = wave && p.log_s != 0 ? 1 : 0;
        if (((skip & 1) && step == 0) || ((skip & 2) && step == pl.n_pass - 1)) {
            if (cap) { *cap = p; *cap_t = t; }
            cur_src = dst;
            continue;
        }
        if (skip & 4) continue;
        u32 tiles = 1u << (log_n - p.log_r - p.log_c);
        size_t lds_bytes = (size_t)32 * ntt_plane_slots(p);
        if (st->lds_floor > lds_bytes) lds_bytes = st->lds_floor;
        u32 E = 1u << (p.log_r + p.log_c);
        u32 threads = E / 2 >= st->threads ? st->threads : (E / 2 >= 64 ? E / 2 : 64);
        if (wave) hipLaunchKernelGGL(k_ntt_pass_wave, dim3(tiles), dim3(threads > 256 ? 256 : threads), lds_bytes, ctx->stream, dst, cur_src, p, t);
        else hipLaunchKernelGGL(k_ntt_pass, dim3(tiles), dim3(threads), lds_bytes, ctx->stream, dst, cur_src, p, t);
        MI_CHECK_HIP(ctx, hipGetLastError());
        cur_src = dst;
        ctx->stats.ntt_launches++;
    }
    if (!(skip & 4)) ctx->stats.ntt_elems += (u64)1 << log_n;
    return MI_OK;
}

int32_t mi_ntt_dev_impl(mi_ctx *ctx, mi_fr *inout_dev, uint32_t log_n, uint32_t flags) {
    return ntt_run(ctx, (Fr *)inout_dev, (const Fr *)inout_dev, 1u << log_n, log_n, flags);
}

struct ComputeHPlan {
    bool pair, triple, last;
    NttPass pc, plast;
    NttTables tc, tlast;
};
static int32_t compute_h_plan(mi_ctx *ctx, uint32_t log_n, Fr *A, ComputeHPlan &cp) {
    const size_t n = (size_t)1 << log_n;
    NttState *st = state_of(ctx);
    const NttKnobs kn = knobs_for(st, log_n);
    const NttPlan pl = ntt_make_plan(log_n, kn.max_contig, kn.max_strided);
    cp.pair = st->fuse_pair && st->wave_stages && pl.n_pass >= 2 && pl.log_r[pl.n_pass - 1] >= 7;
    cp.triple = st->fuse_triple && st->wave_stages && pl.n_pass >= 2 && (pl.log_r[0] == 7 || pl.log_r[0] == 8);
    {
        const u32 lr = pl.log_r[pl.n_pass - 1];
        const u32 room = kn.log_e > lr ? kn.log_e - lr : 0, avail = log_n - lr, lc = room < avail ? room : avail;
        cp.last = st->fuse_last && st->wave_stages && pl.n_pass >= 2 && lr >= 7 && (1u << (lr + lc)) <= 4 * 256;
    }
    cp.pc = NttPass{}; cp.plast = NttPass{}; cp.tc = NttTables{}; cp.tlast = NttTables{};
    if (cp.triple) {
        MI_TRY(ntt_run(ctx, A, A, (u32)n, log_n, MI_NTT_DIT | MI_NTT_COSET, 2, nullptr, nullptr, 2 | 4, &cp.pc, &cp.tc));
        MI_TRY(ntt_run(ctx, A, A, (u32)n, log_n, MI_NTT_INVERSE | MI_NTT_COSET, 3, nullptr, nullptr, 1 | 4, &cp.plast, &cp.tlast));
        const NttPass &pc = cp.pc, &plast = cp.plast;
        cp.triple = pc.log_r == plast.log_r && pc.log_s == plast.log_s && pc.log_c == plast.log_c && pc.log_s != 0 && pc.lds_pad == plast.lds_pad && !pc.scale && !plast.scale &&
                    ((pc.log_r == 7 && pc.log_c <= 3) ||
                     (pc.log_r == 8 && pc.log_c >= 1 && pc.log_c <= 2));
    }
    return MI_OK;
}
int32_t mi_compute_h_part(mi_ctx *ctx, uint32_t log_n, int part, const mi_fr *src, size_t n_constraints, mi_fr *h_out, const mi_fr *src2) {
    static const char *const range_names[4] = {"mi.computeH.a.enqueue", "mi.computeH.b.enqueue", "mi.computeH.c.enqueue", "mi.computeH.last.enqueue"};
    const MiRange range(range_names[part & 3]);
    const size_t n = (size_t)1 << log_n;
    MI_TRY(ensure_direct(ctx, log_n));
    MI_TRY(mi_reserve(ctx, ctx->ws[WS_H_B], n * sizeof(Fr)));
    MI_TRY(mi_reserve(ctx, ctx->ws[WS_H_C], n * sizeof(Fr)));
    Fr *A = (Fr *)h_out, *B = (Fr *)ctx->ws[WS_H_B].p, *C = (Fr *)ctx->ws[WS_H_C].p;
    ComputeHPlan cp;
    MI_TRY(compute_h_plan(ctx, log_n, A, cp));
    const u32 first_skip = cp.pair ? 1u : 0u;
    if (part == 0 || part == 1) {
        Fr *v = part == 0 ? A : B;
        if (!cp.pair) {
            MI_TRY(ntt_run(ctx, v, (const Fr *)src, (u32)n_constraints, log_n, MI_NTT_INVERSE, 1));
        } else {
            NttPass pi{}, pf{};
            NttTables ti{}, tf{};
            MI_TRY(ntt_run(ctx, v, (const Fr *)src, (u32)n_constraints, log_n, MI_NTT_INVERSE, 1, nullptr, nullptr, 2, &pi, &ti));
            MI_TRY(ntt_run(ctx, v, v, (u32)n, log_n, MI_NTT_DIT | MI_NTT_COSET, 2, nullptr, nullptr, 1 | 4, &pf, &tf));
            if (pi.log_r != pf.log_r || pi.log_c != pf.log_c || pi.log_s || pf.log_s) MI_FAIL(ctx, MI_EINVAL, "internal: contiguous pass pair does not match");
            hipLaunchKernelGGL(k_ntt_contig_pair, dim3(1u << (log_n - pi.log_r - pi.log_c)), dim3(256), (size_t)32 * ntt_plane_slots(pi), ctx->stream, v, pi, ti, pf, tf);
            MI_CHECK_HIP(ctx, hipGetLastError());
            ctx->stats.ntt_launches++;
        }
        NttPass px{};
        NttTables tx{};
        return ntt_run(ctx, v, v, (u32)n, log_n, MI_NTT_DIT | MI_NTT_COSET, 2, nullptr, nullptr, first_skip | (cp.triple ? 2u : 0u), &px, &tx);
    }
    if (part == 2) {
        NttPass px{};
        NttTables tx{};
        return ntt_run(ctx, C, (const Fr *)src, (u32)n_constraints, log_n, MI_NTT_INVERSE, 4, (const Fr *)src2, nullptr, cp.last ? 2u : 0u, &px, &tx);
    }
    auto last_fused = [&]() -> int32_t {
        NttPass pa{}, pcl{};
        NttTables ta{}, tcl{};
        MI_TRY(ntt_run(ctx, C, C, (u32)n, log_n, MI_NTT_INVERSE, 4, nullptr, nullptr, 2 | 4, &pcl, &tcl));
        MI_TRY(ntt_run(ctx, A, A, (u32)n, log_n, MI_NTT_INVERSE | MI_NTT_COSET, 3, nullptr, nullptr, 2 | 4, &pa, &ta));
        if (pa.log_r != pcl.log_r || pa.log_c != pcl.log_c || pa.log_s || pcl.log_s || pa.dit || pcl.dit || pa.lds_pad != pcl.lds_pad)
            MI_FAIL(ctx, MI_EINVAL, "internal: the two last passes of computeH do not match");
        const u32 E = 1u << (pa.log_r + pa.log_c);
        Msm2Shape zs{};
        bool count = ctx->zhook.armed && ctx->zhook.C1;
        if (count) {
            std::memcpy(&zs, ctx->zhook.shape, sizeof(zs));
            count = E % MSM2_SLICE == 0 && E / MSM2_SLICE <= 4 && zs.n <= n && (u64)zs.nslices * MSM2_SLICE == n && zs.c >= 17 && zs.c <= 22 && !zs.wkeys &&
                    (size_t)32 * ntt_plane_slots(pa) + (size_t)(E / MSM2_SLICE) * zs.ngroups * 4 <= 160 * 1024;
        }
        ctx->zhook.armed = false;
        if (count) {
            const size_t lds_bytes = (size_t)32 * ntt_plane_slots(pa) + (size_t)(E / MSM2_SLICE) * zs.ngroups * 4;
#define MI_LAST_COUNT(CW) do { \
            hipLaunchKernelGGL(k_ntt_contig_last_sub_count<CW>, dim3(1u << (log_n - pa.log_r - pa.log_c)), dim3(256), lds_bytes, ctx->stream, A, (const Fr *)C, pa, ta, pcl, tcl, zs, ctx->zhook.C1); } while (0)
            switch (zs.c) { case 17: MI_LAST_COUNT(17); break; case 18: MI_LAST_COUNT(18); break; case 19: MI_LAST_COUNT(19); break; case 20: MI_LAST_COUNT(20); break;
                            case 21: MI_LAST_COUNT(21); break; default: MI_LAST_COUNT(22); break; }
#undef MI_LAST_COUNT
            ctx->zhook.done = true; ctx->zhook.h = A;
            ctx->z_count_fused_launches++;
        } else {
            hipLaunchKernelGGL(k_ntt_contig_last_sub, dim3(1u << (log_n - pa.log_r - pa.log_c)), dim3(256), (size_t)32 * ntt_plane_slots(pa), ctx->stream, A, (const Fr *)C, pa, ta, pcl, tcl);
        }
        MI_CHECK_HIP(ctx, hipGetLastError());
        ctx->stats.ntt_launches++;
        return MI_OK;
    };
    if (!cp.triple) {
        if (!cp.last) return ntt_run(ctx, A, A, (u32)n, log_n, MI_NTT_INVERSE | MI_NTT_COSET, 3, B, C);
        NttPass px{};
        NttTables tx{};
        MI_TRY(ntt_run(ctx, A, A, (u32)n, log_n, MI_NTT_INVERSE | MI_NTT_COSET, 3, B, nullptr, 2, &px, &tx));
        return last_fused();
    }
    const NttPass &pc = cp.pc;
    if (pc.log_r == 7)
        hipLaunchKernelGGL(k_ntt_strided_triple, dim3(1u << (log_n - pc.log_r - pc.log_c)), dim3(64u << pc.log_c), (size_t)32 * ntt_plane_slots(pc), ctx->stream,
                           A, (const Fr *)B, pc, cp.tc, cp.plast, cp.tlast);
    else
        hipLaunchKernelGGL(k_ntt_strided_triple8, dim3(1u << (log_n - pc.log_r - pc.log_c)), dim3(256), (size_t)32 * ntt_plane_slots(pc), ctx->stream,
                           A, (const Fr *)B, pc, cp.tc, cp.plast, cp.tlast);
    MI_CHECK_HIP(ctx, hipGetLastError());
    ctx->stats.ntt_launches++;
    if (!cp.last) return ntt_run(ctx, A, A, (u32)n, log_n, MI_NTT_INVERSE | MI_NTT_COSET, 3, nullptr, C, 1);
    NttPass px{};
    NttTables tx{};
    MI_TRY(ntt_run(ctx, A, A, (u32)n, log_n, MI_NTT_INVERSE | MI_NTT_COSET, 3, nullptr, nullptr, 1 | 2, &px, &tx));
    return last_fused();
}
int32_t mi_compute_h_dev_impl(mi_ctx *ctx, uint32_t log_n, const mi_fr *a, const mi_fr *b, const mi_fr *c,
                              size_t n_constraints, mi_fr *h_out) {
    MI_TRY(mi_compute_h_part(ctx, log_n, 0, a, n_constraints, h_out));
    MI_TRY(mi_compute_h_part(ctx, log_n, 1, b, n_constraints, h_out));
    if (c) MI_TRY(mi_compute_h_part(ctx, log_n, 2, c, n_constraints, h_out));
    else MI_TRY(mi_compute_h_part(ctx, log_n, 2, a, n_constraints, h_out, b));
    return mi_compute_h_part(ctx, log_n, 3, nullptr, n_constraints, h_out);
}

static void stats_begin(mi_ctx *ctx) { std::memset(&ctx->stats, 0, sizeof(ctx->stats)); }

extern "C" {
int32_t mi_debug_set_ntt_plan(mi_ctx *ctx, uint32_t log_e, uint32_t max_contig, uint32_t max_strided) {
    if (!ctx || log_e < 1 || log_e > 12 || max_contig < 1 || max_contig > 12 || max_contig > log_e || max_strided < 1 || max_strided > 12 || max_strided > log_e)
        return MI_EINVAL;
    NttState *st = state_of(ctx);
    st->log_e = log_e; st->max_contig = max_contig; st->max_strided = max_strided; st->plan_set = 1;
    return MI_OK;
}
int32_t mi_debug_set_ntt_wave_stages(mi_ctx *ctx, uint32_t on, uint32_t direct_min_log_n) {
    if (!ctx || on > 1) return MI_EINVAL;
    NttState *st = state_of(ctx);
    st->wave_stages = on; st->direct_min_log_n = direct_min_log_n;
    st->d_npass = 0;
    return MI_OK;
}
int32_t mi_debug_set_ntt_fuse_pair(mi_ctx *ctx, uint32_t on) {
    if (!ctx || on > 7) return MI_EINVAL;
    state_of(ctx)->fuse_pair = on & 1u;
    state_of(ctx)->fuse_triple = (on >> 1) & 1u;
    state_of(ctx)->fuse_last = (on >> 2) & 1u;
    return MI_OK;
}
int32_t mi_debug_set_ntt_threads(mi_ctx *ctx, uint32_t threads) {
    if (!ctx || threads < 64 || threads > 1024 || (threads & (threads - 1))) return MI_EINVAL;
    state_of(ctx)->threads = threads;
    return MI_OK;
}
int32_t mi_ntt_dev(mi_ctx *ctx, mi_fr *inout_dev, uint32_t log_n, uint32_t flags) {
    if (!ctx || !inout_dev || log_n > 28 || (flags & ~7u)) return MI_EINVAL;
    stats_begin(ctx);
    MI_CHECK_HIP(ctx, hipEventRecord(ctx->ev[EV_T0], ctx->stream));
    MI_TRY(mi_ntt_dev_impl(ctx, inout_dev, log_n, flags));
    MI_CHECK_HIP(ctx, hipEventRecord(ctx->ev[EV_T1], ctx->stream));
    MI_CHECK_HIP(ctx, hipEventSynchronize(ctx->ev[EV_T1]));
    MI_CHECK_HIP(ctx, hipEventElapsedTime(&ctx->stats.ntt_kernel_ms, ctx->ev[EV_T0], ctx->ev[EV_T1]));
    return MI_OK;
}
int32_t mi_ntt(mi_ctx *ctx, mi_fr *inout, uint32_t log_n, uint32_t flags) {
    if (!ctx || !inout || log_n > 28 || (flags & ~7u)) return MI_EINVAL;
    size_t bytes = sizeof(Fr) << log_n;
    MI_TRY(mi_reserve(ctx, ctx->ws[WS_HOST_IO0], bytes));
    MI_CHECK_HIP(ctx, hipMemcpyAsync(ctx->ws[WS_HOST_IO0].p, inout, bytes, hipMemcpyHostToDevice, ctx->stream));
    MI_TRY(mi_ntt_dev(ctx, (mi_fr *)ctx->ws[WS_HOST_IO0].p, log_n, flags));
    MI_CHECK_HIP(ctx, hipMemcpyAsync(inout, ctx->ws[WS_HOST_IO0].p, bytes, hipMemcpyDeviceToHost, ctx->stream));
    MI_CHECK_HIP(ctx, hipStreamSynchronize(ctx->stream));
    return MI_OK;
}
int32_t mi_compute_h_dev(mi_ctx *ctx, uint32_t log_n, const mi_fr *a, const mi_fr *b, const mi_fr *c,
                         size_t n_constraints, mi_fr *h_out) {
    if (!ctx || !a || !b || !h_out || log_n > 28 || n_constraints > ((size_t)1 << log_n)) return MI_EINVAL;
    stats_begin(ctx);
    MI_CHECK_HIP(ctx, hipEventRecord(ctx->ev[EV_T0], ctx->stream));
    MI_TRY(mi_compute_h_dev_impl(ctx, log_n, a, b, c, n_constraints, h_out));
    MI_CHECK_HIP(ctx, hipEventRecord(ctx->ev[EV_T1], ctx->stream));
    MI_CHECK_HIP(ctx, hipEventSynchronize(ctx->ev[EV_T1]));
    MI_CHECK_HIP(ctx, hipEventElapsedTime(&ctx->stats.compute_h_ms, ctx->ev[EV_T0], ctx->ev[EV_T1]));
    ctx->stats.ntt_kernel_ms = ctx->stats.compute_h_ms;
    return MI_OK;
}
int32_t mi_compute_h(mi_ctx *ctx, uint32_t log_n, const mi_fr *a, const mi_fr *b, const mi_fr *c,
                     size_t n_constraints, mi_fr *h_out) {
    if (!ctx || !a || !b || !h_out || log_n > 28 || n_constraints > ((size_t)1 << log_n)) return MI_EINVAL;
    size_t nb = n_constraints * sizeof(Fr), full = sizeof(Fr) << log_n;
    MI_TRY(mi_reserve(ctx, ctx->ws[WS_HOST_IO0], full));
    MI_TRY(mi_reserve(ctx, ctx->ws[WS_HOST_IO1], nb * 3 + 96));
    char *in = (char *)ctx->ws[WS_HOST_IO1].p;
    MI_CHECK_HIP(ctx, hipMemcpyAsync(in, a, nb, hipMemcpyHostToDevice, ctx->stream));
    MI_CHECK_HIP(ctx, hipMemcpyAsync(in + nb, b, nb, hipMemcpyHostToDevice, ctx->stream));
    if (c) MI_CHECK_HIP(ctx, hipMemcpyAsync(in + 2 * nb, c, nb, hipMemcpyHostToDevice, ctx->stream));
    MI_TRY(mi_compute_h_dev(ctx, log_n, (mi_fr *)in, (mi_fr *)(in + nb), c ? (mi_fr *)(in + 2 * nb) : nullptr, n_constraints, (mi_fr *)ctx->ws[WS_HOST_IO0].p));
    MI_CHECK_HIP(ctx, hipMemcpyAsync(h_out, ctx->ws[WS_HOST_IO0].p, full, hipMemcpyDeviceToHost, ctx->stream));
    MI_CHECK_HIP(ctx, hipStreamSynchronize(ctx->stream));
    return MI_OK;
}
}
```

### gnark-whir_amd/csrc/prove.hip

```cpp
#include "prove_internal.h"
#include "r1cs_internal.h"
#include <cstring>
#include <vector>
#include <chrono>
#include <cstdlib>

__global__ void k_expand_points(G1Aff *full, const G1Aff *compact, const u32 *idx, size_t n) {
    size_t i = (size_t)blockIdx.x * blockDim.x + threadIdx.x;
    if (i < n) full[idx[i]] = compact[i];
}
__global__ void k_gather_fr(Fr *out, const Fr *W, const u32 *idx, size_t n) {
    size_t i = (size_t)blockIdx.x * blockDim.x + threadIdx.x;
    if (i < n) out[i] = W[idx[i]];
}

static size_t point_bytes(int curve) { return curve == 1 ? sizeof(G1Aff) : sizeof(G2Aff); }
static int32_t upload(mi_ctx *ctx, void **dst, const void *src, size_t bytes) {
    MI_CHECK_HIP(ctx, hipMalloc(dst, bytes ? bytes : 32));
    if (bytes) MI_CHECK_HIP(ctx, hipMemcpyAsync(*dst, src, bytes, hipMemcpyHostToDevice, ctx->stream));
    return MI_OK;
}

static int32_t check_header(mi_ctx *ctx, const mi_pk_desc *d, bool slices, const ShardRange *sr, ShardRange *r) {
    if (d->log_n > 28 || d->nb_public > d->nb_wires || !d->infinity_a || !d->infinity_b) MI_FAIL(ctx, MI_EINVAL, "pk: bad header");
    const u64 N = (u64)1 << d->log_n;
    if (!slices && d->n_g1_z + 1 < N) MI_FAIL(ctx, MI_EINVAL, "pk: G1.Z needs at least 2^log_n - 1 points");
    if (d->nb_wires >= ((u64)1 << 31)) MI_FAIL(ctx, MI_EINVAL, "pk: too many wires");
    if (d->n_g2_b != d->n_g1_b) MI_FAIL(ctx, MI_EINVAL, "pk: G1.B and G2.B differ in length");
    *r = sr ? *sr : ShardRange{0, d->nb_wires, 0, N - 1};
    if (r->w_lo > r->w_hi || r->w_hi > d->nb_wires || r->z_lo > r->z_hi || r->z_hi > N - 1) MI_FAIL(ctx, MI_EINVAL, "pk: bad shard range");
    if (r->w_hi - r->w_lo > MI_MSM_MAX_PAIRS || r->z_hi - r->z_lo > MI_MSM_MAX_PAIRS)
        MI_FAIL(ctx, MI_EINVAL, "pk: a per-device MSM would exceed 2^27 pairs (log_n = 28, or more than 2^27 wires on one device): "
                                "load the key with mi_pk_load_sharded over enough devices");
    return MI_OK;
}
enum { ARR_A, ARR_B1, ARR_K, ARR_Z, ARR_B2 };
static int32_t take_arrays(mi_ctx *ctx, mi_pk *pk, const mi_pk_desc *d, const WireIndices &wi, u64 n_z, bool device_points, bool adopt, void *arr[5], u32 *idx[3]) {
    const void *given[5] = {d->g1_a, d->g1_b, d->g1_k, d->g1_z, d->g2_b};
    const u64 first[5] = {wi.a0, wi.b0, wi.k0, pk->z_lo, wi.b0}, n[5] = {wi.a.size(), wi.b.size(), wi.k.size(), n_z, wi.b.size()};
    auto key_upload = [&](void **dst, const void *src, size_t bytes, int kind) { const int32_t rc = upload(ctx, dst, src, bytes); if (*dst) pk->own(*dst, bytes, kind); return rc; };
    for (int i = 0; i < 5; i++) {
        const size_t size = point_bytes(i == ARR_B2 ? 2 : 1);
        if (!device_points) MI_TRY(key_upload(&arr[i], (const char *)given[i] + first[i] * size, n[i] * size, KEY_MEM_BASES));
        else { arr[i] = (void *)given[i]; if (adopt) pk->own(arr[i], n[i] * size, KEY_MEM_BASES); }
    }
    const std::vector<u32> *wires[3] = {&wi.a, &wi.b, &wi.k};
    for (int i = 0; i < 3; i++) MI_TRY(key_upload((void **)&idx[i], wires[i]->data(), wires[i]->size() * 4, KEY_MEM_INDICES));
    return MI_OK;
}
static int32_t expand_per_wire(mi_ctx *ctx, mi_pk *pk, void **full, const void *compact, const u32 *idx, size_t n) {
    const size_t bytes = (size_t)pk->nb_wires * sizeof(G1Aff);
    MI_CHECK_HIP(ctx, hipMalloc(full, bytes ? bytes : 64));
    pk->own(*full, bytes, KEY_MEM_BASES);
    MI_CHECK_HIP(ctx, hipMemsetAsync(*full, 0, bytes, ctx->stream));
    if (n) hipLaunchKernelGGL(k_expand_points, dim3((unsigned)((n + 255) / 256)), dim3(256), 0, ctx->stream, (G1Aff *)*full, (const G1Aff *)compact, idx, n);
    MI_CHECK_HIP(ctx, hipGetLastError());
    return MI_OK;
}
static void plan_tables(mi_ctx *ctx, mi_pk *pk, const FixedBasePlan *forced) {
    size_t free_b = 0, total_b = 0;
    if (hipMemGetInfo(&free_b, &total_b) != hipSuccess) free_b = 0;
    const FixedBasePlan own = fixed_base_plan(ctx->fixed_knob, free_b / 3, pk->group[KEY_AK].n, pk->group[KEY_B].n, pk->group[KEY_Z].n);
    for (int g = 0; g < 3; g++) pk->group[g].c = forced && !ctx->fixed_knob[g] ? forced->c[g] : own.c[g];
}
static int32_t build_table(mi_ctx *ctx, mi_pk *pk, void **table, const void *plain, size_t n, int curve, u32 c) {
    const size_t bytes = msm_nwin(c) * n * point_bytes(curve);
// ... 166 lines not shown
    if (!pk) return MI_EINVAL;
    return pedersen_msm(ctx, pk, true, values, n, pok);
}
int32_t mi_pedersen_fold(const mi_g1_affine *points, size_t n, const mi_fr *challenge, mi_g1_affine *out) {
    if ((!points && n) || !challenge || !out) return MI_EINVAL;
    Fr ch, pw = Fr::one();
    std::memcpy(&ch, challenge, 32);
    G1X acc = G1X::inf();
    for (size_t i = 0; i < n; i++) {
        G1Aff p;
        std::memcpy(&p, &points[i], sizeof(p));
        G1X t = i ? host_scalar_mul<Fp>(p, fe_from_mont(pw)) : G1X::from_affine(p);
        xyzz_add(acc, t);
        pw = pw * ch;
    }
    if (n == 1) { std::memcpy(out, &points[0], sizeof(*out)); return MI_OK; }
    G1Aff a = xyzz_to_affine(acc);
    std::memcpy(out, &a, sizeof(a));
    return MI_OK;
}
int32_t mi_get_mem_ledger(mi_ctx *ctx, const mi_pk *pk, mi_mem_ledger *out) {
    if (!ctx || !out) return MI_EINVAL;
    std::memset(out, 0, sizeof(*out));
    if (pk) { out->key_bases = pk->mem[KEY_MEM_BASES]; out->key_tables = pk->mem[KEY_MEM_TABLES]; out->key_indices = pk->mem[KEY_MEM_INDICES]; }
    out->ctx_ntt_tables = mi_ntt_table_bytes(ctx);
    for (int i = 0; i < WS_COUNT; i++) {
        const size_t cap = ctx->ws[i].cap;
        if (i == WS_H_B || i == WS_H_C || i == WS_H) out->ctx_ntt_vectors += cap; else out->ctx_other += cap;
    }
    for (const auto &sl : ctx->msm) for (const auto &b : sl.buf) out->ctx_msm += b.cap;
    return MI_OK;
}
int32_t mi_pk_table_plan(const mi_pk *pk, uint32_t c_out[3]) {
    if (!pk || !c_out) return MI_EINVAL;
    for (int g = 0; g < 3; g++) c_out[g] = pk->group[g].c;
    return MI_OK;
}
int32_t mi_pk_load(mi_ctx *ctx, const mi_pk_desc *d, mi_pk **out) {
    if (d && (!d->g1_a && d->n_g1_a)) return MI_EINVAL;
    return mi_pk_load_range(ctx, d, out, false, nullptr);
}
int32_t mi_pk_load_dev(mi_ctx *ctx, const mi_pk_desc *d, mi_pk **out) { return mi_pk_load_range(ctx, d, out, true, nullptr); }
int32_t mi_pk_free(mi_ctx *ctx, mi_pk *pk) {
    if (!ctx || !pk) return MI_EINVAL;
    (void)hipStreamSynchronize(ctx->stream);
    for (const mi_pk::Alloc &a : pk->owned) if (a.p) (void)hipFree(a.p);
    delete pk;
    return MI_OK;
}

}

static void arm_accum_gate(mi_ctx *ctx, int slot, const std::function<hipEvent_t()> *accum_gate) { ctx->msm[slot].accum_gate = accum_gate; }
static int32_t enqueue_b_msms(mi_ctx *ctx, mi_pk *pk, const mi_fr *W, hipEvent_t ev_w, bool defer, const std::function<hipEvent_t()> *accum_gate) {
    (void)hipSetDevice(ctx->dev);
    const uint32_t fl = (defer ? MI_MSM_DEFER_REDUCE : 0) | MI_MSM_EXACT_SIZE | (pk->rprime ? MI_MSM_PTS_RPRIME : 0);
    const KeyGroup &B = pk->group[KEY_B];
    MI_TRY(mi_reserve(ctx, ctx->ws[WS_B_WIRES], (B.n + 1) * sizeof(Fr)));
    hipStream_t st = ctx->msm[MSM_SLOT_B1].stream;
    if (ev_w) MI_CHECK_HIP(ctx, hipStreamWaitEvent(st, ev_w, 0));
    if (B.n) hipLaunchKernelGGL(k_gather_fr, dim3((unsigned)((B.n + 255) / 256)), dim3(256), 0, st, (Fr *)ctx->ws[WS_B_WIRES].p, (const Fr *)W, pk->idx_b, B.n);
    MI_CHECK_HIP(ctx, hipGetLastError());
    arm_accum_gate(ctx, MSM_SLOT_B1, accum_gate);
    MI_TRY(mi_msm_enqueue(ctx, MSM_SLOT_B1, -1, 1, B.bases[0].pts, ctx->ws[WS_B_WIRES].p, B.n, fl, nullptr, false, B.c, B.bases[0].stat_pairs, B.gen_c));
    arm_accum_gate(ctx, MSM_SLOT_B2, accum_gate);
    return mi_msm_enqueue(ctx, MSM_SLOT_B2, MSM_SLOT_B1, 2, B.bases[1].pts, nullptr, B.n, fl, nullptr, false, B.c, B.bases[1].stat_pairs);
}
static int32_t enqueue_ak_msms(mi_ctx *ctx, mi_pk *pk, const mi_fr *W, hipEvent_t ev_w, bool defer, const std::function<hipEvent_t()> *accum_gate) {
    (void)hipSetDevice(ctx->dev);
    const uint32_t fl = (defer ? MI_MSM_DEFER_REDUCE : 0) | MI_MSM_EXACT_SIZE | (pk->rprime ? MI_MSM_PTS_RPRIME : 0);
    const KeyGroup &AK = pk->group[KEY_AK];
    arm_accum_gate(ctx, MSM_SLOT_A, accum_gate);
    MI_TRY(mi_msm_enqueue(ctx, MSM_SLOT_A, -1, 1, AK.bases[0].pts, W, AK.n, fl, ev_w, true, AK.c, AK.bases[0].stat_pairs, AK.gen_c));
    arm_accum_gate(ctx, MSM_SLOT_K, accum_gate);
    return mi_msm_enqueue(ctx, MSM_SLOT_K, MSM_SLOT_A, 1, AK.bases[1].pts, nullptr, AK.n, fl, nullptr, false, AK.c, AK.bases[1].stat_pairs);
}
void WireMsms::start(mi_ctx *ctx, mi_pk *pk, const mi_fr *W, hipEvent_t ev_w, bool defer, const std::function<hipEvent_t()> *accum_gate) {
    auto group = [&](std::future<int32_t> &f, int32_t (*enqueue)(mi_ctx *, mi_pk *, const mi_fr *, hipEvent_t, bool, const std::function<hipEvent_t()> *)) {
        try {
            f = std::async(std::launch::async, [=]() -> int32_t { try { return enqueue(ctx, pk, W, ev_w, defer, accum_gate); } catch (...) { return MI_ENOMEM; } });
        } catch (...) {
            int32_t r = MI_ENOMEM;
            try { r = enqueue(ctx, pk, W, ev_w, defer, nullptr); } catch (...) {}
            if (rc_inline == MI_OK) rc_inline = r;
        }
    };
    group(f_b, enqueue_b_msms);
    group(f_ak, enqueue_ak_msms);
}
int32_t WireMsms::join() {
    int32_t rc = rc_inline;
    for (std::future<int32_t> *f : {&f_b, &f_ak})
        if (f->valid()) { const int32_t r = f->get(); if (rc == MI_OK) rc = r; }
    return rc;
}
int32_t mi_prove_enqueue_wire_msms(mi_ctx *ctx, mi_pk *pk, const mi_fr *W, hipEvent_t ev_w, bool defer) {
    WireMsms wires;
    wires.start(ctx, pk, W, ev_w, defer, nullptr);
    return wires.join();
}
int32_t mi_prove_enqueue_z_msm(mi_ctx *ctx, mi_pk *pk, const mi_fr *h, hipEvent_t ev_h, bool defer) {
    const uint32_t fl = (defer ? MI_MSM_DEFER_REDUCE : 0) | (pk->rprime ? MI_MSM_PTS_RPRIME : 0);
    const KeyGroup &Z = pk->group[KEY_Z];
    return mi_msm_enqueue(ctx, MSM_SLOT_Z, -1, 1, Z.bases[0].pts, h, Z.n, fl, ev_h, true, Z.c, Z.bases[0].stat_pairs, Z.gen_c);
}

template <class Fn>
static auto async_or_inline(Fn fn) -> std::future<decltype(fn())> {
    try {
        return std::async(std::launch::async, fn);
    } catch (...) {
        std::promise<decltype(fn())> p;
        p.set_value(fn());
        return p.get_future();
    }
}
void ProofAssembler::start(const mi_pk *pk_, const mi_fr *r_m, const mi_fr *s_m) {
    pk = pk_;
    Fr r, s;
    std::memcpy(&r, r_m, 32); std::memcpy(&s, s_m, 32);
    rc = fe_from_mont(r); sc = fe_from_mont(s); krc = fe_from_mont(fe_neg(r * s));
    f_r = async_or_inline([this] { return host_scalar_mul<Fp>(pk->delta1, rc); });
    f_s = async_or_inline([this] { return host_scalar_mul<Fp>(pk->delta1, sc); });
    f_kr = async_or_inline([this] { return host_scalar_mul<Fp>(pk->delta1, krc); });
    s_delta2 = host_scalar_mul<Fp2>(pk->delta2, sc);
    r_delta = f_r.get(); s_delta = f_s.get(); kr_delta = f_kr.get();
}
void ProofAssembler::have_a_b1(const G1X &msm_a, const G1X &msm_b1) {
    G1X ar = msm_a;
    xyzz_madd(ar, pk->alpha1, false);
    xyzz_add(ar, r_delta);
    G1X bs1 = msm_b1;
    xyzz_madd(bs1, pk->beta1, false);
    xyzz_add(bs1, s_delta);
    ar_aff = xyzz_to_affine(ar); bs1_aff = xyzz_to_affine(bs1);
    f_sar = async_or_inline([this] { return host_scalar_mul<Fp>(ar_aff, sc); });
    r_bs1 = host_scalar_mul<Fp>(bs1_aff, rc);
}
void ProofAssembler::finish(const G1X &msm_k, const G2X &msm_b2, const G1X &msm_z, mi_proof_out *out) {
    G1X s_ar = f_sar.get();
    G1X krs = msm_k;
    xyzz_add(krs, msm_z);
    xyzz_add(krs, kr_delta);
    xyzz_add(krs, s_ar);
    xyzz_add(krs, r_bs1);
    G2X bs = msm_b2;
    xyzz_madd(bs, pk->beta2, false);
    xyzz_add(bs, s_delta2);
    G1Aff krs_aff = xyzz_to_affine(krs);
    G2Aff bs_aff = xyzz_to_affine(bs);
    std::memcpy(&out->ar, &ar_aff, 64); std::memcpy(&out->bs, &bs_aff, 128); std::memcpy(&out->krs, &krs_aff, 64);
}

struct HostInputs { const mi_fr *W, *a, *b, *c; };
struct WEval { const mi_r1cs *r1cs; bool eval_c; };
struct AbcGate { const std::function<bool(int)> *abc;  bool abc_arrived;  };

static int32_t check_key_fits(mi_ctx *ctx, const mi_pk *pk, size_t n_wires) {
    if (pk->wire_lo || pk->n_z_msm != ((u64)1 << pk->log_n) - 1) MI_FAIL(ctx, MI_EINVAL, "prove: this key is one part of a sharded key (use mi_groth16_prove_sharded)");
    if (n_wires != pk->nb_wires) MI_FAIL(ctx, MI_EINVAL, "prove: witness size (n_wires) does not match the proving key");
    return MI_OK;
}

static int32_t prove_common(mi_ctx *ctx, mi_pk *pk, const mi_fr *W, size_t n_wires, const mi_fr *a, const mi_fr *b, const mi_fr *c,
                            size_t n_constraints, const mi_fr *r_m, const mi_fr *s_m, mi_proof_out *out, mi_stats *stats, const HostInputs *host,
                            const AbcGate *gate = nullptr, const WEval *weval = nullptr) {
    if (!ctx || !pk || !r_m || !s_m || !out) return MI_EINVAL;
    const MiRange range_all("mi.prove");
    if (weval) n_constraints = weval->r1cs->nc;
    if ((!W && n_wires) || (!weval && (!a || !b) && n_constraints)) MI_FAIL(ctx, MI_EINVAL, "prove: null W, a or b with a non-zero count");
    if (host && ((!host->W && n_wires) || (!weval && (!host->a || !host->b) && n_constraints))) MI_FAIL(ctx, MI_EINVAL, "prove: null host W, a or b with a non-zero count");
    const bool derive_c = weval ? !weval->eval_c : host ? !host->c : !c;
    const size_t N = (size_t)1 << pk->log_n;
    MI_TRY(check_key_fits(ctx, pk, n_wires));
    if (n_constraints > N) MI_FAIL(ctx, MI_EINVAL, "prove: witness size does not match the proving key");
    std::memset(&ctx->stats, 0, sizeof(ctx->stats));
    const auto t_begin = std::chrono::steady_clock::now();
    hipEvent_t *ev = ctx->ev;
    MI_TRY(mi_reserve(ctx, ctx->ws[WS_H], N * sizeof(Fr)));
    mi_fr *h = (mi_fr *)ctx->ws[WS_H].p;
    std::promise<hipEvent_t> h_recorded;
    bool h_promised = false;
    const std::shared_future<hipEvent_t> h_fut = h_recorded.get_future().share();
    const std::function<hipEvent_t()> h_gate = [h_fut] { return h_fut.get(); };
    const bool hold = ctx->hold_accum && !host && (!gate || gate->abc_arrived);
    WireMsms wires;

    struct { std::function<int32_t(hipEvent_t *)> w_resident; std::function<int32_t(int)> make_abc; } arrival;
    const mi_fr *abc[3] = {a, b, c};
    std::chrono::steady_clock::time_point t_up;
    hipStream_t cps = nullptr;
    if (host) {
        auto upload = [&, ctx](const mi_fr *dst, const mi_fr *src, size_t bytes) -> int32_t {
            const MiRange range("mi.prove.upload");
            if (bytes) MI_CHECK_HIP(ctx, hipMemcpyAsync((void *)dst, src, bytes, hipMemcpyHostToDevice, cps));
            MI_CHECK_HIP(ctx, hipStreamSynchronize(cps));
            ctx->stats.h2d_ms = std::chrono::duration<float, std::milli>(std::chrono::steady_clock::now() - t_up).count();
            return MI_OK;
        };
        arrival.w_resident = [&, upload](hipEvent_t *ev_w) -> int32_t {
            t_up = std::chrono::steady_clock::now();
            MI_TRY(mi_copy_stream(ctx, &cps));
            MI_CHECK_HIP(ctx, hipStreamSynchronize(ctx->stream));
            *ev_w = nullptr;
            return upload(W, host->W, n_wires * sizeof(mi_fr));
        };
        arrival.make_abc = [&, upload](int k) -> int32_t { return upload(abc[k], k == 0 ? host->a : k == 1 ? host->b : host->c, n_constraints * sizeof(mi_fr)); };
    } else if (gate) {
        arrival.w_resident = [](hipEvent_t *ev_w) -> int32_t { *ev_w = nullptr; return MI_OK; };
        arrival.make_abc = [&](int k) -> int32_t { if (!(*gate->abc)(k + 1)) MI_FAIL(ctx, MI_EHIP, "prove: the upload of a, b, c failed"); return MI_OK; };
    } else {
        arrival.w_resident = [&](hipEvent_t *ev_w) -> int32_t { *ev_w = ev[EV_PROVE_BEGIN]; return MI_OK; };
        arrival.make_abc = [](int) -> int32_t { return MI_OK; };
    }
    if (weval) arrival.make_abc = [&](int k) -> int32_t { return k ? MI_OK : mi_r1cs_eval_ws(ctx, weval->r1cs, W, weval->eval_c, &abc[0], &abc[1], &abc[2]); };

    auto main_part = [&]() -> int32_t {
        MI_CHECK_HIP(ctx, hipEventRecord(ev[EV_PROVE_BEGIN], ctx->stream));
        hipEvent_t ev_w = nullptr;
        MI_TRY(arrival.w_resident(&ev_w));
        wires.start(ctx, pk, W, ev_w, false, hold ? &h_gate : nullptr);
        MI_TRY(arrival.make_abc(0));
        MI_TRY(mi_compute_h_part(ctx, pk->log_n, 0, abc[0], n_constraints, h));
        MI_TRY(arrival.make_abc(1));
        MI_TRY(mi_compute_h_part(ctx, pk->log_n, 1, abc[1], n_constraints, h));
        if (derive_c) MI_TRY(mi_compute_h_part(ctx, pk->log_n, 2, abc[0], n_constraints, h, abc[1]));
        else { MI_TRY(arrival.make_abc(2)); MI_TRY(mi_compute_h_part(ctx, pk->log_n, 2, abc[2], n_constraints, h)); }
        if (pk->group[KEY_Z].c) MI_TRY(mi_msm_z_count_arm(ctx, MSM_SLOT_Z, pk->n_z_msm, pk->group[KEY_Z].c));
        const int32_t rc_h = mi_compute_h_part(ctx, pk->log_n, 3, nullptr, n_constraints, h);
        ctx->zhook.armed = false;
        MI_TRY(rc_h);
        MI_CHECK_HIP(ctx, hipEventRecord(ev[EV_H_READY], ctx->stream));
        h_recorded.set_value(ev[EV_H_READY]); h_promised = true;
        return mi_prove_enqueue_z_msm(ctx, pk, h, ev[EV_H_READY]);
    };
    {
        int32_t rc = main_part();
        if (!h_promised) h_recorded.set_value(nullptr);
        { const int32_t r = wires.join(); if (rc == MI_OK) rc = r; }
        if (rc != MI_OK) {
            ctx->zhook.armed = ctx->zhook.done = false;
            const std::string keep = ctx->err;
            G1X t1; G2X t2;
            for (int sl : {MSM_SLOT_A, MSM_SLOT_B1, MSM_SLOT_K, MSM_SLOT_Z}) (void)mi_msm_finish(ctx, sl, 1, &t1);
            (void)mi_msm_finish(ctx, MSM_SLOT_B2, 2, &t2);
            (void)hipStreamSynchronize(ctx->stream);
            mi_set_err(ctx, keep);
            return rc;
        }
    }
    ProofAssembler as;
    { const MiRange range("mi.prove.blinding"); as.start(pk, r_m, s_m); }
    G1X msm_a, msm_b1, msm_k, msm_z;
    G2X msm_b2;
    MI_TRY(mi_msm_finish(ctx, MSM_SLOT_A, 1, &msm_a));
    MI_TRY(mi_msm_finish(ctx, MSM_SLOT_B1, 1, &msm_b1));
    const auto t_asm0 = std::chrono::steady_clock::now();
    as.have_a_b1(msm_a, msm_b1);
    MI_TRY(mi_msm_finish(ctx, MSM_SLOT_K, 1, &msm_k));
    MI_TRY(mi_msm_finish(ctx, MSM_SLOT_B2, 2, &msm_b2));
    MI_TRY(mi_msm_finish(ctx, MSM_SLOT_Z, 1, &msm_z));
    MI_CHECK_HIP(ctx, hipStreamSynchronize(ctx->stream));
    const auto t_gpu_done = std::chrono::steady_clock::now();
    { const MiRange range("mi.prove.assemble"); as.finish(msm_k, msm_b2, msm_z, out); }
    const auto t_end = std::chrono::steady_clock::now();
    mi_stats &st = ctx->stats;
    auto ms = [](std::chrono::steady_clock::time_point x, std::chrono::steady_clock::time_point y) {
        return std::chrono::duration<float, std::milli>(y - x).count();
    };
    auto slot_ms = [&](int slot, float *dst) -> int32_t {
        MI_CHECK_HIP(ctx, hipEventElapsedTime(dst, ctx->msm[slot].ev[MSM_EV_JOB_BEGIN], ctx->msm[slot].ev[MSM_EV_JOB_END]));
        return MI_OK;
    };
    MI_CHECK_HIP(ctx, hipEventElapsedTime(&st.compute_h_ms, ev[EV_PROVE_BEGIN], ev[EV_H_READY]));
    if (pk->nb_wires) MI_TRY(slot_ms(MSM_SLOT_A, &st.msm_a_ms));
    if (pk->group[KEY_B].n) { MI_TRY(slot_ms(MSM_SLOT_B1, &st.msm_b1_ms)); MI_TRY(slot_ms(MSM_SLOT_B2, &st.msm_b2_ms)); }
    if (pk->nb_wires) MI_TRY(slot_ms(MSM_SLOT_K, &st.msm_k_ms));
    if (N > 1) MI_TRY(slot_ms(MSM_SLOT_Z, &st.msm_z_ms));
    st.assemble_ms = ms(t_gpu_done, t_end);
    st.filter_ms = ms(t_asm0, t_gpu_done);
    st.total_ms = ms(t_begin, t_end);
    if (stats) *stats = st;
    return MI_OK;
}

int32_t mi_groth16_prove_dev_gated(mi_ctx *ctx, mi_pk *pk, const mi_fr *W, size_t n_wires, const mi_fr *a, const mi_fr *b, const mi_fr *c, size_t n_constraints,
                                   const mi_fr *r, const mi_fr *s, mi_proof_out *out, mi_stats *stats, const std::function<bool(int)> &abc_ready, bool abc_arrived) {
    const AbcGate gate{&abc_ready, abc_arrived};
    return prove_common(ctx, pk, W, n_wires, a, b, c, n_constraints, r, s, out, stats, nullptr, &gate);
}

static int32_t check_w_inputs(mi_ctx *ctx, const mi_pk *pk, const mi_r1cs *r1cs, const mi_fr *W, size_t n_wires, uint32_t flags) {
    if (!r1cs) MI_FAIL(ctx, MI_EINVAL, "prove_w: r1cs is null");
    if (!W) MI_FAIL(ctx, MI_EINVAL, "prove_w: W is null");
    if (flags & ~MI_PROVE_W_EVAL_C) MI_FAIL(ctx, MI_EINVAL, "prove_w: unknown flag");
    if (r1cs->dev != ctx->dev) MI_FAIL(ctx, MI_EINVAL, "prove_w: the r1cs was loaded on another device");
    MI_TRY(check_key_fits(ctx, pk, n_wires));
    if (n_wires != r1cs->nb_wires) MI_FAIL(ctx, MI_EINVAL, "prove_w: n_wires does not match the r1cs");
    if (pk->log_n != r1cs->log_n) MI_FAIL(ctx, MI_EINVAL, "prove_w: the key's log_n is not the domain of the r1cs's n_constraints");
    return MI_OK;
}

extern "C" {
int32_t mi_groth16_prove_w_dev(mi_ctx *ctx, mi_pk *pk, const mi_r1cs *r1cs, const mi_fr *W_dev, size_t n_wires, uint32_t flags,
                               const mi_fr *r, const mi_fr *s, mi_proof_out *out, mi_stats *stats) {
    if (!ctx || !pk || !r || !s || !out) return MI_EINVAL;
    MI_TRY(check_w_inputs(ctx, pk, r1cs, W_dev, n_wires, flags));
    const WEval we{r1cs, (flags & MI_PROVE_W_EVAL_C) != 0};
    return prove_common(ctx, pk, W_dev, n_wires, nullptr, nullptr, nullptr, 0, r, s, out, stats, nullptr, nullptr, &we);
}
int32_t mi_groth16_prove_w(mi_ctx *ctx, mi_pk *pk, const mi_r1cs *r1cs, const mi_fr *W, size_t n_wires, uint32_t flags,
                           const mi_fr *r, const mi_fr *s, mi_proof_out *out, mi_stats *stats) {
    if (!ctx || !pk || !r || !s || !out) return MI_EINVAL;
    MI_TRY(check_w_inputs(ctx, pk, r1cs, W, n_wires, flags));
    MI_TRY(mi_reserve(ctx, ctx->ws[WS_PROVE_IN], n_wires * 32 + 128));
    const HostInputs host{W, nullptr, nullptr, nullptr};
    const WEval we{r1cs, (flags & MI_PROVE_W_EVAL_C) != 0};
    return prove_common(ctx, pk, (mi_fr *)ctx->ws[WS_PROVE_IN].p, n_wires, nullptr, nullptr, nullptr, 0, r, s, out, stats, &host, nullptr, &we);
}
int32_t mi_groth16_prove_dev(mi_ctx *ctx, mi_pk *pk, const mi_fr *W, size_t n_wires, const mi_fr *a, const mi_fr *b, const mi_fr *c,
                             size_t n_constraints, const mi_fr *r, const mi_fr *s, mi_proof_out *out, mi_stats *stats) {
    return prove_common(ctx, pk, W, n_wires, a, b, c, n_constraints, r, s, out, stats, nullptr);
}
int32_t mi_groth16_prove(mi_ctx *ctx, mi_pk *pk, const mi_fr *W, size_t n_wires, const mi_fr *a, const mi_fr *b, const mi_fr *c,
                         size_t n_constraints, const mi_fr *r, const mi_fr *s, mi_proof_out *out, mi_stats *stats) {
    if (!ctx || !pk || !r || !s || !out) return MI_EINVAL;
    const size_t wb = n_wires * 32, cb = n_constraints * 32;
    MI_TRY(mi_reserve(ctx, ctx->ws[WS_PROVE_IN], wb + 3 * cb + 128));
    char *base = (char *)ctx->ws[WS_PROVE_IN].p;
    const HostInputs host{W, a, b, c};
    return prove_common(ctx, pk, (mi_fr *)base, n_wires, (mi_fr *)(base + wb), (mi_fr *)(base + wb + cb), (mi_fr *)(base + wb + 2 * cb),
                        n_constraints, r, s, out, stats, &host);
}
}
// ... 1 lines not shown
```

### gnark-whir_amd/csrc/prove_internal.h

```cpp
#pragma once
#include "ctx.h"
#include "curve.cuh"
#include "msm_curve_ops.h"
#include "key_plan.h"
#include <functional>
#include <future>

struct KeyGroup {
    u32 c = 0;
    u32 gen_c = 0;
    u64 n = 0;
    struct { void *pts = nullptr; u64 stat_pairs = 0; } bases[2];
};
enum { KEY_AK, KEY_B, KEY_Z };
static constexpr int KEY_GROUP_MSMS[3] = {2, 2, 1}, KEY_GROUP_CURVE[3][2] = {{1, 1}, {1, 2}, {1, 1}};
enum { KEY_MEM_BASES, KEY_MEM_TABLES, KEY_MEM_INDICES };

struct mi_pk {
    u32 log_n = 0, nb_public = 0;
    u64 nb_wires = 0;
    KeyGroup group[3];
    const u32 *idx_b = nullptr;
    bool rprime = false;
    G1Aff alpha1, beta1, delta1;
    G2Aff beta2, delta2;
    u64 wire_lo = 0, z_lo = 0, n_z_msm = 0;
    struct Alloc { void *p; u64 bytes; int kind; };
    std::vector<Alloc> owned;
    u64 mem[3] = {0, 0, 0};
    void own(void *p, u64 bytes, int kind) { owned.push_back({p, bytes, kind}); mem[kind] += bytes; }
    void drop(void *p) { for (Alloc &a : owned) if (p && a.p == p) { (void)hipFree(p); mem[a.kind] -= a.bytes; a.p = nullptr; } }
};

struct ShardRange { u64 w_lo, w_hi, z_lo, z_hi; };
int32_t mi_pk_load_range(mi_ctx *ctx, const mi_pk_desc *d, mi_pk **out, bool device_points, const ShardRange *sr, const FixedBasePlan *forced = nullptr,
                         bool adopt = false, bool *took_arrays = nullptr);
extern "C" int32_t mi_pedersen_pk_adopt(mi_ctx *ctx, void *basis_dev, void *basis_exp_sigma_dev, size_t n, mi_pedersen_pk **out);
int32_t mi_pedersen_pok_enqueue(mi_ctx *ctx, mi_pedersen_pk *pk, const mi_fr *values, size_t n);
int32_t mi_pedersen_pok_collect(mi_ctx *ctx, mi_g1_affine *pok_or_null);
struct WireMsms {
    std::future<int32_t> f_b, f_ak;
    int32_t rc_inline = MI_OK;
    void start(mi_ctx *ctx, mi_pk *pk, const mi_fr *W_dev, hipEvent_t ev_w, bool defer_reduce, const std::function<hipEvent_t()> *accum_gate);
    int32_t join();
};
int32_t mi_prove_enqueue_wire_msms(mi_ctx *ctx, mi_pk *pk, const mi_fr *W_dev, hipEvent_t ev_w, bool defer_reduce = false);
int32_t mi_prove_enqueue_z_msm(mi_ctx *ctx, mi_pk *pk, const mi_fr *h_dev, hipEvent_t ev_h, bool defer_reduce = false);

int32_t mi_groth16_prove_dev_gated(mi_ctx *ctx, mi_pk *pk, const mi_fr *W_dev, size_t n_wires, const mi_fr *a_dev, const mi_fr *b_dev, const mi_fr *c_dev,
                                   size_t n_constraints, const mi_fr *r, const mi_fr *s, mi_proof_out *out, mi_stats *stats,
                                   const std::function<bool(int)> &abc_ready, bool abc_arrived);

struct ProofAssembler {
    const mi_pk *pk = nullptr;
    Fr rc, sc, krc;
    std::future<G1X> f_r, f_s, f_kr, f_sar;
    G2X s_delta2;
    G1X r_delta, s_delta, kr_delta, r_bs1;
    G1Aff ar_aff, bs1_aff;
    void start(const mi_pk *pk_, const mi_fr *r_m, const mi_fr *s_m);
    void have_a_b1(const G1X &msm_a, const G1X &msm_b1);
    void finish(const G1X &msm_k, const G2X &msm_b2, const G1X &msm_z, mi_proof_out *out);
};
```

### include/mi355x_groth16.h

```cpp
#ifndef MI355X_GROTH16_H
#define MI355X_GROTH16_H
#include <stddef.h>
#include <stdint.h>

#ifdef __cplusplus
extern "C" {
#endif

#define MI_OK 0
#define MI_EINVAL (-1)
#define MI_EHIP (-2)
#define MI_ENOMEM (-3)
#define MI_ENODEV (-4)

typedef struct { uint64_t l[4]; } mi_fr;
typedef struct { uint64_t l[4]; } mi_fp;
typedef struct { mi_fp a0, a1; } mi_fp2;
typedef struct { mi_fp x, y; } mi_g1_affine;
typedef struct { mi_fp x, y, z; } mi_g1_jac;
typedef struct { mi_fp2 x, y; } mi_g2_affine;
typedef struct { mi_fp2 x, y, z; } mi_g2_jac;

typedef struct mi_ctx mi_ctx;
typedef struct mi_pk mi_pk;

#define MI_NTT_INVERSE 1u
#define MI_NTT_COSET 2u
#define MI_NTT_DIT 4u

#define MI_MSM_MAX_PAIRS (1ull << 27)
#define MI_MSM_SCALARS_CANONICAL 1u

typedef struct mi_pk_desc {
    uint32_t log_n;
    uint32_t nb_public;
    uint64_t nb_wires;
    const mi_g1_affine *g1_a;  uint64_t n_g1_a;
    const mi_g1_affine *g1_b;  uint64_t n_g1_b;
    const mi_g1_affine *g1_k;  uint64_t n_g1_k;
    const mi_g1_affine *g1_z;  uint64_t n_g1_z;
    const mi_g2_affine *g2_b;  uint64_t n_g2_b;
    mi_g1_affine alpha1, beta1, delta1;
    mi_g2_affine beta2, delta2;
    const uint8_t *infinity_a;
    const uint8_t *infinity_b;
    const uint32_t *committed_wires;
    uint64_t n_committed;
} mi_pk_desc;

typedef struct mi_proof_out {
    mi_g1_affine ar;
    mi_g2_affine bs;
    mi_g1_affine krs;
} mi_proof_out;

typedef struct mi_stats {
    float h2d_ms, compute_h_ms, filter_ms;
    float msm_a_ms, msm_b1_ms, msm_k_ms, msm_z_ms, msm_b2_ms;
    float assemble_ms, total_ms;
    float g1_accum_kernel_ms;
    uint64_t g1_accum_pairs;
    uint32_t g1_accum_launches;
    float ntt_kernel_ms;
    uint64_t ntt_elems;
    uint32_t ntt_launches;
    uint64_t g1_accum_entries;
    uint64_t g1_level1_additions;
} mi_stats;

int32_t mi_init(int device_id, mi_ctx **out);
int32_t mi_init_prio(int device_id, int prio_scheme, mi_ctx **out);
int32_t mi_shutdown(mi_ctx *ctx);
const char *mi_last_error(mi_ctx *ctx);
int32_t mi_set_stream(mi_ctx *ctx, void *hip_stream);

int32_t mi_pk_load(mi_ctx *ctx, const mi_pk_desc *desc, mi_pk **out);
int32_t mi_pk_load_dev(mi_ctx *ctx, const mi_pk_desc *desc, mi_pk **out);
int32_t mi_pk_free(mi_ctx *ctx, mi_pk *pk);

#define MI_PK_RAW_MAX_COMMITMENTS 16
typedef struct mi_pk_raw_info {
    uint32_t log_n, n_commitment_keys;
    uint64_t nb_wires, n_g1_a, n_g1_b, n_g1_z, n_g1_k, n_g2_b;
    uint64_t off_alpha1, off_g1_a, off_g1_b, off_g1_z, off_g1_k, off_beta2, off_g2_b, off_infinity_a, off_infinity_b;
    uint64_t n_basis[MI_PK_RAW_MAX_COMMITMENTS], off_basis[MI_PK_RAW_MAX_COMMITMENTS], off_basis_exp_sigma[MI_PK_RAW_MAX_COMMITMENTS];
} mi_pk_raw_info;
int32_t mi_pk_raw_inspect(const uint8_t *buf, size_t len, mi_pk_raw_info *info);
typedef struct mi_pedersen_pk mi_pedersen_pk;
int32_t mi_pk_load_raw(mi_ctx *ctx, const uint8_t *buf, size_t len, uint32_t nb_public, const uint32_t *committed_wires,
                       size_t n_committed, mi_pk **out, mi_pedersen_pk **ped_out, uint32_t *n_ped_out);

int32_t mi_ntt(mi_ctx *ctx, mi_fr *inout, uint32_t log_n, uint32_t flags);
int32_t mi_ntt_dev(mi_ctx *ctx, mi_fr *inout_dev, uint32_t log_n, uint32_t flags);

int32_t mi_compute_h(mi_ctx *ctx, uint32_t log_n, const mi_fr *a, const mi_fr *b, const mi_fr *c,
                     size_t n_constraints, mi_fr *h_out);
int32_t mi_compute_h_dev(mi_ctx *ctx, uint32_t log_n, const mi_fr *a_dev, const mi_fr *b_dev,
                         const mi_fr *c_dev, size_t n_constraints, mi_fr *h_out_dev);

int32_t mi_msm_g1(mi_ctx *ctx, const mi_g1_affine *pts, const mi_fr *scalars, size_t n,
                  uint32_t flags, mi_g1_jac *out);
int32_t mi_msm_g1_dev(mi_ctx *ctx, const mi_g1_affine *pts_dev, const mi_fr *scalars_dev, size_t n,
                      uint32_t flags, mi_g1_jac *out);
int32_t mi_msm_g2(mi_ctx *ctx, const mi_g2_affine *pts, const mi_fr *scalars, size_t n,
                  uint32_t flags, mi_g2_jac *out);
int32_t mi_msm_g2_dev(mi_ctx *ctx, const mi_g2_affine *pts_dev, const mi_fr *scalars_dev, size_t n,
                      uint32_t flags, mi_g2_jac *out);

int32_t mi_msm_precompute_g1_dev(mi_ctx *ctx, const mi_g1_affine *base_dev, size_t n, uint32_t c, mi_g1_affine *pre_dev);
int32_t mi_msm_precompute_g2_dev(mi_ctx *ctx, const mi_g2_affine *base_dev, size_t n, uint32_t c, mi_g2_affine *pre_dev);
int32_t mi_msm_table_to_rprime_g1_dev(mi_ctx *ctx, mi_g1_affine *pre_dev, size_t n_points);
int32_t mi_msm_table_to_rprime_g2_dev(mi_ctx *ctx, mi_g2_affine *pre_dev, size_t n_points);
#define MI_MSM_TABLE_RPRIME 2u
int32_t mi_msm_g1_fixed_dev(mi_ctx *ctx, const mi_g1_affine *pre_dev, const mi_fr *scalars_dev, size_t n, uint32_t c,
                            uint32_t flags, mi_g1_jac *out);
int32_t mi_msm_g2_fixed_dev(mi_ctx *ctx, const mi_g2_affine *pre_dev, const mi_fr *scalars_dev, size_t n, uint32_t c,
                            uint32_t flags, mi_g2_jac *out);

int32_t mi_groth16_prove(mi_ctx *ctx, mi_pk *pk, const mi_fr *W, size_t n_wires,
                         const mi_fr *a, const mi_fr *b, const mi_fr *c, size_t n_constraints,
// ... 69 lines not shown
```

### include/mi355x_groth16_debug.h

```cpp
#ifndef MI355X_GROTH16_DEBUG_H
#define MI355X_GROTH16_DEBUG_H
#include "mi355x_groth16.h"

#ifdef __cplusplus
extern "C" {
#endif

#define MI_DIST_UNIFORM 0
#define MI_DIST_WHIR 1
#define MI_DIST_MIX_FLAG 0x40000000
#define MI_DIST_MIX(bit_pm, byte_pm, u64_pm) (MI_DIST_MIX_FLAG | ((bit_pm) << 20) | ((byte_pm) << 10) | (u64_pm))
int32_t mi_gen_scalars_dev(mi_ctx *ctx, mi_fr *out_dev, size_t n, uint64_t seed, int dist);
int32_t mi_gen_g1_dev(mi_ctx *ctx, mi_g1_affine *out_dev, size_t n, uint64_t seed);
int32_t mi_gen_g2_dev(mi_ctx *ctx, mi_g2_affine *out_dev, size_t n, uint64_t seed);
int32_t mi_field_op_dev(mi_ctx *ctx, int field, int op, void *z_dev, const void *x_dev,
                        const void *y_dev, size_t n);
int32_t mi_g1_add_dev(mi_ctx *ctx, mi_g1_affine *out_dev, const mi_g1_affine *a_dev,
                      const mi_g1_affine *b_dev, size_t n);
int32_t mi_g2_add_dev(mi_ctx *ctx, mi_g2_affine *out_dev, const mi_g2_affine *a_dev,
                      const mi_g2_affine *b_dev, size_t n);
#define MI_LIMB29_IN_WORDS 144
#define MI_LIMB29_OUT_WORDS 80
int32_t mi_debug_limb29_op_dev(mi_ctx *ctx, int op, void *out_dev, const void *in_dev, size_t n);
#define MI_LAZY_IN_WORDS 24
#define MI_LAZY_OUT_WORDS 16
int32_t mi_debug_lazy_op_dev(mi_ctx *ctx, int op, void *out_dev, const void *in_dev, size_t n);
#define MI_SHAPE_IN_WORDS 32
#define MI_SHAPE_OUT_WORDS 32
int32_t mi_debug_field_shape_dev(mi_ctx *ctx, int shape, void *out_dev, const void *in_dev, size_t n);
#define MI_PAIRING_FINAL_EXP 1u
#define MI_FP12_WORDS 96
int32_t mi_debug_pairing_dev(mi_ctx *ctx, const mi_g1_affine *p_dev, const mi_g2_affine *q_dev, size_t n, mi_fp *gt_dev, uint32_t flags);
int32_t mi_debug_fp12_op_dev(mi_ctx *ctx, int op, mi_fp *z_dev, const mi_fp *x_dev, const mi_fp *y_dev, size_t n);
int32_t mi_debug_decode_g1_dev(mi_ctx *ctx, const uint8_t *enc_dev, size_t n, mi_g1_affine *out_dev, uint8_t *bad_dev);
int32_t mi_debug_decode_g2_dev(mi_ctx *ctx, const uint8_t *enc_dev, size_t n, mi_g2_affine *out_dev, uint8_t *bad_dev);
int32_t mi_debug_hash_to_field_dev(mi_ctx *ctx, const uint8_t *dst_dev, uint32_t dst_len, const uint8_t *msgs_dev, size_t msg_len, size_t n, mi_fr *out_dev);
int32_t mi_debug_witness_decode_dev(mi_ctx *ctx, const uint8_t *values_dev, size_t n, uint32_t n_pub, mi_fr *out_dev, uint8_t *bad_dev);

int32_t mi_debug_fp12_product_dev(mi_ctx *ctx, const mi_fp *x_dev, size_t n, mi_fp *out_dev);
int32_t mi_debug_g1_scale128_dev(mi_ctx *ctx, const mi_g1_affine *p_dev, const uint64_t *k_dev, size_t n, mi_g1_affine *out_dev);
int32_t mi_debug_g1_sum_tree_dev(mi_ctx *ctx, const mi_g1_affine *p_dev, size_t n, mi_g1_affine *levels_dev);
int32_t mi_debug_locate_points_dev(mi_ctx *ctx, const uint64_t *r_dev, const mi_g1_affine *krs_dev, const mi_g1_affine *cm_dev, const mi_g1_affine *pok_dev,
                                   const mi_fr *fold_dev, uint32_t nc, size_t n, mi_g1_affine *out_dev);
int32_t mi_debug_locate_colsums_dev(mi_ctx *ctx, const mi_fr *scal_dev, uint32_t ns, const mi_fr *r_dev, size_t n, uint32_t level, const uint32_t *nodes_dev,
                                    size_t m, mi_fr *sums_dev);
int32_t mi_debug_set_locate_round_nodes(mi_ctx *ctx, uint32_t cap);
int32_t mi_bench_gather_dev(mi_ctx *ctx, const void *table_dev, size_t n_entries, size_t n_threads, uint32_t iters,
                            void *scratch_dev, float *ms_out);
int32_t mi_bench_modmul_dev(mi_ctx *ctx, int field, size_t n_threads, uint32_t iters,
                            void *scratch_dev, float *ms_out);
int32_t mi_bench_valu_dev(mi_ctx *ctx, int kind, size_t n_threads, uint32_t iters,
                          void *scratch_dev, float *ms_out);
int32_t mi_debug_set_ntt_plan(mi_ctx *ctx, uint32_t log_e, uint32_t max_contig, uint32_t max_strided);
int32_t mi_debug_set_ntt_threads(mi_ctx *ctx, uint32_t threads);
int32_t mi_debug_set_ntt_wave_stages(mi_ctx *ctx, uint32_t on, uint32_t direct_min_log_n);
int32_t mi_debug_set_ntt_fuse_pair(mi_ctx *ctx, uint32_t on);
int32_t mi_debug_set_msm_plan(mi_ctx *ctx, uint32_t c, uint32_t L1, uint32_t L2, uint32_t seg, uint32_t G);
int32_t mi_debug_set_msm_chunk(mi_ctx *ctx, uint32_t chunk);
int32_t mi_debug_set_msm_group_bits(mi_ctx *ctx, uint32_t gbits);
int32_t mi_debug_set_prove_fixed_base(mi_ctx *ctx, uint32_t c_ak, uint32_t c_b, uint32_t c_z);
int32_t mi_debug_set_prove_schedule(mi_ctx *ctx, uint32_t hold_accum);
int32_t mi_debug_set_msm_bound_levels(mi_ctx *ctx, uint32_t on);
int32_t mi_debug_set_msm_one_pass_sort(mi_ctx *ctx, uint32_t on);
int32_t mi_debug_set_msm_limb29(mi_ctx *ctx, uint32_t on);
int32_t mi_debug_set_msm_l1_waves(mi_ctx *ctx, uint32_t waves);
int32_t mi_debug_set_msm_batch_affine(mi_ctx *ctx, uint32_t rounds);
int32_t mi_debug_set_msm_precompute_batched(mi_ctx *ctx, uint32_t on);
int32_t mi_debug_set_knob(mi_ctx *ctx, const char *name, int64_t value);
int32_t mi_debug_get_counter(mi_ctx *ctx, const char *name, uint64_t *out);
int32_t mi_debug_set_stream_plan(int32_t plan);
int32_t mi_debug_set_trace_ranges(int32_t on);
int32_t mi_debug_inject_hip_failure(int32_t nth);
int32_t mi_debug_ceremony_coeffs_dev(mi_ctx *ctx, const uint8_t seed[32], size_t n, mi_fr *out_dev);

#ifdef __cplusplus
}
#endif
#endif
```

Before: 33.40.

## Convert MSM scalars out of Montgomery form once instead of per pass

Wire scalars are converted from Montgomery form to canonical form once, into a new workspace buffer, before the A/K and B MSMs, so each MSM pass no longer decodes them again. The H polynomial's final inverse-NTT step now uses plain-form scale tables, so it emits canonical H directly and the fused Z count kernel and Z MSM can skip decoding too. The cost is an extra conversion kernel with a scratch buffer, an event dependency on the A stream, and extra plain twiddle tables. A knob turns it off, and new counters track decode counts.

```diff
diff --git a/gnark-whir_amd/binding.py b/gnark-whir_amd/binding.py
--- a/gnark-whir_amd/binding.py
+++ b/gnark-whir_amd/binding.py
@@ -18,7 +18,7 @@
     "mi_batch_scalar_mul_g1", "mi_batch_scalar_mul_g1_dev", "mi_batch_scalar_mul_g2", "mi_batch_scalar_mul_g2_dev",
     "mi_pedersen_pk_load", "mi_pedersen_pk_free", "mi_pedersen_commit", "mi_pedersen_prove_knowledge", "mi_pedersen_fold",
     "mi_debug_set_prove_fixed_base", "mi_debug_set_prove_schedule", "mi_debug_set_msm_batch_affine", "mi_debug_set_msm_group_bits", "mi_debug_inject_hip_failure", "mi_debug_set_ntt_plan", "mi_debug_set_ntt_threads", "mi_debug_set_ntt_wave_stages",
-    "mi_debug_set_msm_plan", "mi_debug_set_msm_chunk", "mi_debug_set_msm_one_pass_sort", "mi_debug_set_msm_bound_levels", "mi_debug_set_msm_limb29", "mi_debug_set_msm_l1_waves", "mi_debug_set_msm_precompute_batched", "mi_debug_set_ntt_fuse_pair", "mi_debug_set_knob", "mi_debug_get_counter", "mi_debug_set_stream_plan", "mi_debug_set_trace_ranges", "mi_set_trace_ranges",
+    "mi_debug_set_msm_plan", "mi_debug_set_msm_chunk", "mi_debug_set_msm_one_pass_sort", "mi_debug_set_msm_bound_levels", "mi_debug_set_msm_limb29", "mi_debug_set_msm_l1_waves", "mi_debug_set_msm_precompute_batched", "mi_debug_set_ntt_fuse_pair", "mi_debug_set_knob", "mi_debug_get_counter", "mi_debug_compute_h_plain_dev", "mi_debug_set_stream_plan", "mi_debug_set_trace_ranges", "mi_set_trace_ranges",
     "mi_prover_create", "mi_prover_destroy", "mi_prover_in_flight", "mi_prover_ctx", "mi_prover_last_error",
     "mi_prover_submit", "mi_prover_submit_dev", "mi_prover_wait", "mi_prover_commit", "mi_prover_submit_bsb22", "mi_prover_trim", "mi_ctx_trim",
     "mi_group_create", "mi_group_unique_id", "mi_group_create_rank", "mi_group_create_rank_ex", "mi_group_rank", "mi_group_destroy", "mi_group_world", "mi_group_local", "mi_group_ctx",
@@ -327,7 +327,8 @@
     _fields_ = [(n, C.c_float) for n in ("h2d_ms", "compute_h_ms", "filter_ms", "msm_a_ms", "msm_b1_ms", "msm_k_ms",
                                          "msm_z_ms", "msm_b2_ms", "assemble_ms", "total_ms")] + [
         ("g1_accum_kernel_ms", C.c_float), ("g1_accum_pairs", C.c_uint64), ("g1_accum_launches", C.c_uint32),
-        ("ntt_kernel_ms", C.c_float), ("ntt_elems", C.c_uint64), ("ntt_launches", C.c_uint32), ("g1_accum_entries", C.c_uint64), ("g1_level1_additions", C.c_uint64)]
+        ("ntt_kernel_ms", C.c_float), ("ntt_elems", C.c_uint64), ("ntt_launches", C.c_uint32), ("g1_accum_entries", C.c_uint64), ("g1_level1_additions", C.c_uint64),
+        ("scalar_decodes", C.c_uint64)]
 
     def as_dict(self):
         return {n: getattr(self, n) for n, _ in self._fields_}
@@ -525,6 +526,9 @@
 
     def compute_h_dev(self, log_n, a, b, c, n_constraints, h):
         self._ck(self.lib.mi_compute_h_dev(self.h, C.c_uint32(log_n), _p(a), _p(b), _p(c), C.c_size_t(n_constraints), _p(h)))
+
+    def debug_compute_h_plain_dev(self, log_n, a, b, c, n_constraints, h):
+        self._ck(self.lib.mi_debug_compute_h_plain_dev(self.h, C.c_uint32(log_n), _p(a), _p(b), _p(c), C.c_size_t(n_constraints), _p(h)))
 
     def msm_g1(self, pts, sc, flags=0):
         out = np.zeros(12, np.uint64); pts, sc = _u64(pts), _u64(sc)
diff --git a/gnark-whir_amd/csrc/ctx.h b/gnark-whir_amd/csrc/ctx.h
--- a/gnark-whir_amd/csrc/ctx.h
+++ b/gnark-whir_amd/csrc/ctx.h
@@ -46,13 +46,15 @@
     WS_FB_SCALARS = 21,
     WS_FB_OUT = 22,
     WS_RPRIME = 23,
-    WS_COUNT = 24
+    WS_W_CANON = 24,
+    WS_COUNT = 25
 };
 enum {
     EV_T0 = 0,
     EV_T1 = 1,
     EV_W_READY = 2,
     EV_H_READY = 3,
+    EV_W_CANON = 4,
     EV_PROVE_BEGIN = 11,
     EV_R1CS_BEGIN = 12,
     EV_R1CS_END = 13,
@@ -132,13 +134,16 @@
     std::atomic<uint64_t> generic_sorts_two_pass{0}, generic_sorts_one_pass{0};
     std::atomic<uint64_t> dense_item_sorts{0};
     uint64_t z_count_fused_launches = 0;
-    struct ZCountHook { bool armed = false, done = false; int slot = -1; uint32_t n = 0, c = 0; alignas(8) unsigned char shape[64]; uint32_t *C1 = nullptr; const void *h = nullptr;  } zhook;
+    uint64_t z_count_accepted = 0, z_count_form_refused = 0;
+    struct ZCountHook { bool armed = false, done = false; int slot = -1; uint32_t n = 0, c = 0; alignas(8) unsigned char shape[64]; uint32_t *C1 = nullptr; const void *h = nullptr;  bool plain = false;  } zhook;
+    std::atomic<uint64_t> scalar_decodes{0};
+    uint32_t scalars_once = 1;
     uint32_t locate_round_nodes = 0;
     uint32_t hold_accum = 0;
 };
 
-static_assert(sizeof(mi_ctx::ws) == WS_COUNT * sizeof(DevBuf) && WS_RPRIME == WS_COUNT - 1, "WS_* names every slot of mi_ctx::ws up to its end");
-static_assert(EV_R1CS_END < EV_COUNT && sizeof(mi_ctx::ev) == EV_COUNT * sizeof(hipEvent_t), "EV_* index mi_ctx::ev");
+static_assert(sizeof(mi_ctx::ws) == WS_COUNT * sizeof(DevBuf) && WS_W_CANON == WS_COUNT - 1, "WS_* names every slot of mi_ctx::ws up to its end");
+static_assert(EV_W_CANON < EV_PROVE_BEGIN && EV_R1CS_END < EV_COUNT && sizeof(mi_ctx::ev) == EV_COUNT * sizeof(hipEvent_t), "EV_* index mi_ctx::ev");
 static_assert(MSM_SLOT_POK == MI_MSM_SLOTS - 1 && sizeof(mi_ctx::msm) == MI_MSM_SLOTS * sizeof(MsmSlot) && MSM_EV_MAX_LANDED == MSM_EV_COUNT - 1 &&
               sizeof(MsmSlot::buf) == B_COUNT_ * sizeof(DevBuf), "MSM_SLOT_* name every slot of mi_ctx::msm, MSM_EV_* every event of a slot, B_* every workspace");
 
@@ -211,7 +216,7 @@
 int32_t mi_ntt_dev_impl(mi_ctx *ctx, mi_fr *inout_dev, uint32_t log_n, uint32_t flags);
 int32_t mi_compute_h_dev_impl(mi_ctx *ctx, uint32_t log_n, const mi_fr *a, const mi_fr *b, const mi_fr *c,
                               size_t n_constraints, mi_fr *h_out);
-int32_t mi_compute_h_part(mi_ctx *ctx, uint32_t log_n, int part, const mi_fr *src, size_t n_constraints, mi_fr *h_out, const mi_fr *src2 = nullptr);
+int32_t mi_compute_h_part(mi_ctx *ctx, uint32_t log_n, int part, const mi_fr *src, size_t n_constraints, mi_fr *h_out, const mi_fr *src2 = nullptr, bool plain_h = false);
 void mi_ntt_state_init(mi_ctx *ctx);
 size_t mi_ntt_table_bytes(mi_ctx *ctx);
 void mi_ntt_state_free(mi_ctx *ctx);
diff --git a/gnark-whir_amd/csrc/msm.hip b/gnark-whir_amd/csrc/msm.hip
--- a/gnark-whir_amd/csrc/msm.hip
+++ b/gnark-whir_amd/csrc/msm.hip
@@ -288,6 +288,8 @@
 extern "C" int32_t mi_debug_get_counter(mi_ctx *ctx, const char *name, uint64_t *out) {
     if (!ctx || !name || !out) return MI_EINVAL;
     if (!std::strcmp(name, "z_count_fused_launches")) { *out = ctx->z_count_fused_launches; return MI_OK; }
+    if (!std::strcmp(name, "z_count_accepted")) { *out = ctx->z_count_accepted; return MI_OK; }
+    if (!std::strcmp(name, "z_count_form_refused")) { *out = ctx->z_count_form_refused; return MI_OK; }
     if (!std::strcmp(name, "dense_item_sorts")) { *out = ctx->dense_item_sorts.load(); return MI_OK; }
     if (!std::strcmp(name, "generic_sorts_two_pass")) { *out = ctx->generic_sorts_two_pass.load(); return MI_OK; }
     if (!std::strcmp(name, "generic_sorts_one_pass")) { *out = ctx->generic_sorts_one_pass.load(); return MI_OK; }
@@ -470,6 +472,7 @@
     int16_t *digits = (int16_t *)sl.buf[B_DIGITS].p;
     u32 *H = (u32 *)sl.buf[B_H].p, *keystart = (u32 *)sl.buf[B_S].p, *total = keystart + s.nkeys + 1, *sorted = (u32 *)sl.buf[B_SORTED].p;
     hipStream_t st = sl.stream;
+    if (!(flags & MI_MSM_SCALARS_CANONICAL) && &sl != &ctx->msm[MSM_SLOT_POK]) ctx->scalar_decodes += n;
     hipLaunchKernelGGL(k_msm_digits, dim3((n + 255) / 256), dim3(256), 0, st, s, scalars, (flags & MI_MSM_SCALARS_CANONICAL) ? 0 : 1, digits);
     const size_t lds_bytes = (size_t)s.nbuckets * 4;
     hipLaunchKernelGGL(k_msm_hist, dim3(s.nslices, s.nwin), dim3(1024), lds_bytes, st, s, digits, H);
@@ -524,9 +527,13 @@
     while (per > 1 && per * s.ngroups > 8192) per >>= 1;
     bool counted = false;
     if (&sl == &ctx->msm[MSM_SLOT_Z]) {
-        counted = ctx->zhook.done && ctx->zhook.slot == MSM_SLOT_Z && ctx->zhook.n == n && ctx->zhook.c == c && ctx->zhook.C1 == C1 && ctx->zhook.h == (const void *)scalars && mont && !wkeys;
+        counted = ctx->zhook.done && ctx->zhook.slot == MSM_SLOT_Z && ctx->zhook.n == n && ctx->zhook.c == c && ctx->zhook.C1 == C1 && ctx->zhook.h == (const void *)scalars &&
+                  ctx->zhook.plain == !mont && !wkeys;
+        if (counted) ctx->z_count_accepted++;
+        else if (ctx->zhook.done && ctx->zhook.h == (const void *)scalars && ctx->zhook.plain != !mont) ctx->z_count_form_refused++;
         ctx->zhook.done = false;
     }
+    if (mont && &sl != &ctx->msm[MSM_SLOT_POK]) ctx->scalar_decodes += (u64)n * (counted ? 1u : 2u);
     if (!counted) {
 #define MI_LAUNCH_COUNT(C) hipLaunchKernelGGL(k_msm2_count<C>, dim3((G + per - 1) / per), dim3(512), 0, st, s, scalars, mont, per, C1)
     MSM2_FOR_C(s.c, MI_LAUNCH_COUNT)
@@ -917,6 +924,7 @@
     else if (is("item_l2") && (value == 0 || (value >= 2 && value <= 64))) k->L2 = (u32)value;
     else if (is("reduce_seg") && value >= 0 && value <= 256) k->seg = (u32)value;
     else if (is("hold_accum") && (value == 0 || value == 1)) ctx->hold_accum = (uint32_t)value;
+    else if (is("scalars_once") && (value == 0 || value == 1)) ctx->scalars_once = (uint32_t)value;
     else if (is("finisher_min_level") && value >= 0 && value <= 16) k->finisher_min_level = (u32)value;
     else if (mi_ntt_set_knob(ctx, name, value)) return MI_OK;
     else MI_FAIL(ctx, MI_EINVAL, std::string("mi_debug_set_knob: unknown knob or value out of range: ") + name);
diff --git a/gnark-whir_amd/csrc/ntt.hip b/gnark-whir_amd/csrc/ntt.hip
--- a/gnark-whir_amd/csrc/ntt.hip
+++ b/gnark-whir_amd/csrc/ntt.hip
@@ -14,6 +14,8 @@
     u32 tw_h = 0;
     Fr *d_tw_inv = nullptr, *d_tw_fwd = nullptr, *d_sc_fwd = nullptr, *d_sc_inv = nullptr;
     u32 d_log_n = 0xffffffffu, d_log_r0 = 0, d_npass = 0;
+    Fr *gi_hi_nd_plain = nullptr, *ninv_den_plain = nullptr, *d_sc_inv_plain = nullptr;
+    u32 p_log_n = 0xffffffffu, dp_log_n = 0xffffffffu;
     u32 direct_min_log_n = 12;
     u32 log_e = 9, max_contig = 9, max_strided = 7, threads = 256;
     u32 lds_floor = 0;
@@ -36,7 +38,7 @@
 __global__ void k_ntt_strided_triple(Fr *a, const Fr *b, NttPass pc, NttTables tc, NttPass pl, NttTables tl);
 __global__ void k_ntt_strided_triple8(Fr *a, const Fr *b, NttPass pc, NttTables tc, NttPass pl, NttTables tl);
 __global__ void k_ntt_contig_last_sub(Fr *A, const Fr *Cin, NttPass pa, NttTables ta, NttPass pc, NttTables tc);
-template <int CC> __global__ void k_ntt_contig_last_sub_count(Fr *A, const Fr *Cin, NttPass pa, NttTables ta, NttPass pc, NttTables tc, Msm2Shape zs, u32 *C1);
+template <int CC, bool PLAIN> __global__ void k_ntt_contig_last_sub_count(Fr *A, const Fr *Cin, NttPass pa, NttTables ta, NttPass pc, NttTables tc, Msm2Shape zs, u32 *C1);
 void mi_ntt_state_init(mi_ctx *ctx) {
     static_assert(sizeof(NttState) <= sizeof(ctx->ntt_state), "NttState lives in ctx->ntt_state");
     new (ctx->ntt_state) NttState();
@@ -46,12 +48,10 @@
     (void)hipFuncSetAttribute((const void *)k_ntt_strided_triple, hipFuncAttributeMaxDynamicSharedMemorySize, 160 * 1024);
     (void)hipFuncSetAttribute((const void *)k_ntt_strided_triple8, hipFuncAttributeMaxDynamicSharedMemorySize, 160 * 1024);
     (void)hipFuncSetAttribute((const void *)k_ntt_contig_last_sub, hipFuncAttributeMaxDynamicSharedMemorySize, 160 * 1024);
-    (void)hipFuncSetAttribute((const void *)k_ntt_contig_last_sub_count<17>, hipFuncAttributeMaxDynamicSharedMemorySize, 160 * 1024);
-    (void)hipFuncSetAttribute((const void *)k_ntt_contig_last_sub_count<18>, hipFuncAttributeMaxDynamicSharedMemorySize, 160 * 1024);
-    (void)hipFuncSetAttribute((const void *)k_ntt_contig_last_sub_count<19>, hipFuncAttributeMaxDynamicSharedMemorySize, 160 * 1024);
-    (void)hipFuncSetAttribute((const void *)k_ntt_contig_last_sub_count<20>, hipFuncAttributeMaxDynamicSharedMemorySize, 160 * 1024);
-    (void)hipFuncSetAttribute((const void *)k_ntt_contig_last_sub_count<21>, hipFuncAttributeMaxDynamicSharedMemorySize, 160 * 1024);
-    (void)hipFuncSetAttribute((const void *)k_ntt_contig_last_sub_count<22>, hipFuncAttributeMaxDynamicSharedMemorySize, 160 * 1024);
+#define MI_LAST_COUNT_LDS(CW) (void)hipFuncSetAttribute((const void *)k_ntt_contig_last_sub_count<CW, false>, hipFuncAttributeMaxDynamicSharedMemorySize, 160 * 1024); \
+                             (void)hipFuncSetAttribute((const void *)k_ntt_contig_last_sub_count<CW, true>, hipFuncAttributeMaxDynamicSharedMemorySize, 160 * 1024)
+    MI_LAST_COUNT_LDS(17); MI_LAST_COUNT_LDS(18); MI_LAST_COUNT_LDS(19); MI_LAST_COUNT_LDS(20); MI_LAST_COUNT_LDS(21); MI_LAST_COUNT_LDS(22);
+#undef MI_LAST_COUNT_LDS
 }
 bool mi_ntt_set_knob(mi_ctx *ctx, const char *name, int64_t value) {
     if (!std::strcmp(name, "ntt_lds_floor_kb") && value >= 0 && value <= 160) { state_of(ctx)->lds_floor = (u32)value * 1024u; return true; }
@@ -60,7 +60,8 @@
 void mi_ntt_state_free(mi_ctx *ctx) {
     NttState *st = state_of(ctx);
     Fr **all[] = {&st->small_f, &st->small_i, &st->tw64k_f, &st->tw64k_i, &st->g_hi_n, &st->gi_hi_nd, &st->tw_lo_f, &st->tw_hi_f, &st->tw_lo_i, &st->tw_hi_i,
-                  &st->g_lo, &st->g_hi, &st->gi_lo, &st->gi_hi, &st->ninv, &st->ninv_den, &st->d_tw_inv, &st->d_tw_fwd, &st->d_sc_fwd, &st->d_sc_inv};
+                  &st->g_lo, &st->g_hi, &st->gi_lo, &st->gi_hi, &st->ninv, &st->ninv_den, &st->d_tw_inv, &st->d_tw_fwd, &st->d_sc_fwd, &st->d_sc_inv,
+                  &st->gi_hi_nd_plain, &st->ninv_den_plain, &st->d_sc_inv_plain};
     for (Fr **p : all) if (*p) { (void)hipFree(*p); *p = nullptr; }
 }
 
@@ -68,6 +69,7 @@
     mi_ntt_state_free(ctx);
     NttState *st = state_of(ctx);
     st->log_n = 0xffffffffu; st->d_log_n = 0xffffffffu; st->d_log_r0 = 0; st->d_npass = 0;
+    st->p_log_n = 0xffffffffu; st->dp_log_n = 0xffffffffu;
 }
 size_t mi_ntt_table_bytes(mi_ctx *ctx) {
     const NttState *st = state_of(ctx);
@@ -78,6 +80,8 @@
         b += (4 * nlo + 6 * nhi + 2) * sizeof(Fr);
     }
     for (const Fr *p : {st->d_tw_inv, st->d_tw_fwd, st->d_sc_fwd, st->d_sc_inv}) if (p) b += sizeof(Fr) << st->d_log_n;
+    if (st->gi_hi_nd_plain && st->log_n != 0xffffffffu) b += (((size_t)1 << (st->log_n - st->tw_h)) + 1) * sizeof(Fr);
+    if (st->d_sc_inv_plain) b += sizeof(Fr) << st->dp_log_n;
     return b;
 }
 
@@ -281,7 +285,7 @@
     }
     __syncthreads();
 }
-template <int CC>
+template <int CC, bool PLAIN>
 __device__ __forceinline__ void ntt_contig_last_sub_body(Fr *A, const Fr *Cin, const NttPass &pa, const NttTables &ta, const NttPass &pc, const NttTables &tc,
                                                          const Msm2Shape &zs, u32 *C1) {
     extern __shared__ U4 lds[];
@@ -315,7 +319,7 @@
         A[g] = hv;
         if (CC >= 0 && g < zs.n) {
             Msm2Digits dg;
-            dg.start(hv, true);
+            dg.start(hv, !PLAIN);
             msm2_count_one<(CC >= 0 ? (u32)CC : 0u)>(zs, dg, cnt + (e / MSM2_SLICE) * zs.ngroups);
         }
     }
@@ -329,11 +333,11 @@
     }
 }
 __global__ void __launch_bounds__(256) k_ntt_contig_last_sub(Fr *A, const Fr *Cin, NttPass pa, NttTables ta, NttPass pc, NttTables tc) {
-    ntt_contig_last_sub_body<-1>(A, Cin, pa, ta, pc, tc, Msm2Shape{}, nullptr);
-}
-template <int CC>
+    ntt_contig_last_sub_body<-1, false>(A, Cin, pa, ta, pc, tc, Msm2Shape{}, nullptr);
+}
+template <int CC, bool PLAIN>
 __global__ void __launch_bounds__(256) k_ntt_contig_last_sub_count(Fr *A, const Fr *Cin, NttPass pa, NttTables ta, NttPass pc, NttTables tc, Msm2Shape zs, u32 *C1) {
-    ntt_contig_last_sub_body<CC>(A, Cin, pa, ta, pc, tc, zs, C1);
+    ntt_contig_last_sub_body<CC, PLAIN>(A, Cin, pa, ta, pc, tc, zs, C1);
 }
 
 __global__ void k_tw_layout(Fr *out, u32 log_n, u32 log_r, Fr w) {
@@ -373,6 +377,7 @@
         MI_TRY(build_table(ctx, &st->tw64k_i, 65536, fe_inv(w64k), Fr::one(), 0));
     }
     if (st->log_n == log_n) return MI_OK;
+    st->p_log_n = 0xffffffffu;
     Fr w = fr_domain_generator(log_n), wi = fe_inv(w);
     Fr g = fe_from_u32<FrParams>(5), gi = fe_inv(g);
     Fr nn = Fr::zero();
@@ -407,7 +412,8 @@
     if (st->d_log_n == log_n && st->d_log_r0 == pl.log_r[0] && st->d_npass == pl.n_pass) return MI_OK;
     Fr **four[] = {&st->d_tw_inv, &st->d_tw_fwd, &st->d_sc_fwd, &st->d_sc_inv};
     for (Fr **p : four) if (*p) { (void)hipFree(*p); *p = nullptr; }
-    st->d_log_n = 0xffffffffu;
+    if (st->d_sc_inv_plain) { (void)hipFree(st->d_sc_inv_plain); st->d_sc_inv_plain = nullptr; }
+    st->d_log_n = 0xffffffffu; st->dp_log_n = 0xffffffffu;
     if (log_n < st->direct_min_log_n) return MI_OK;
     MI_TRY(ensure_tables(ctx, log_n));
     const size_t bytes = sizeof(Fr) << log_n;
@@ -436,10 +442,42 @@
     return MI_OK;
 }
 
+static Fr ninv_den_plain_of(u32 log_n) {
+    const Fr g = fe_from_u32<FrParams>(5);
+    Fr nn = Fr::zero();
+    nn.l[0] = (u32)(1u << log_n);
+    Fr gn = g;
+    for (u32 k = 0; k < log_n; k++) gn = fe_sqr(gn);
+    return fe_from_mont(fe_inv(fe_to_mont(nn)) * fe_inv(gn - Fr::one()));
+}
+static int32_t ensure_plain(mi_ctx *ctx, u32 log_n) {
+    NttState *st = state_of(ctx);
+    MI_TRY(ensure_tables(ctx, log_n));
+    const Fr gi = fe_inv(fe_from_u32<FrParams>(5));
+    if (st->p_log_n != log_n) {
+        const Fr c = ninv_den_plain_of(log_n);
+        MI_TRY(build_table(ctx, &st->gi_hi_nd_plain, 1u << (log_n - st->tw_h), gi, c, st->tw_h));
+        MI_TRY(build_table(ctx, &st->ninv_den_plain, 1, Fr::one(), c, 0));
+        st->p_log_n = log_n;
+    }
+    if (st->d_log_n == log_n && st->d_sc_inv && st->dp_log_n != log_n) {
+        if (st->d_sc_inv_plain) { (void)hipFree(st->d_sc_inv_plain); st->d_sc_inv_plain = nullptr; }
+        if (hipMalloc((void **)&st->d_sc_inv_plain, sizeof(Fr) << log_n) != hipSuccess) { (void)hipGetLastError(); st->d_sc_inv_plain = nullptr; return MI_OK; }
+        hipLaunchKernelGGL(k_sc_layout, dim3((unsigned)((((size_t)1 << log_n) + 255) / 256)), dim3(256), 0, ctx->stream, st->d_sc_inv_plain, log_n, gi, ninv_den_plain_of(log_n));
+        MI_CHECK_HIP(ctx, hipGetLastError());
+        st->dp_log_n = log_n;
+    }
+    return MI_OK;
+}
+
+static constexpr u32 NTT_PLAIN_OUT = 8;
 static int32_t ntt_run(mi_ctx *ctx, Fr *dst, const Fr *src, u32 n_valid, u32 log_n, u32 flags, u32 variant = 0,
                        const Fr *load_mul = nullptr, const Fr *store_sub = nullptr, u32 skip = 0, NttPass *cap = nullptr, NttTables *cap_t = nullptr) {
     NttState *st = state_of(ctx);
     MI_TRY(ensure_tables(ctx, log_n));
+    const bool plain = (variant & NTT_PLAIN_OUT) != 0;
+    variant &= ~NTT_PLAIN_OUT;
+    if (plain && ((variant != 3 && variant != 4) || st->p_log_n != log_n)) MI_FAIL(ctx, MI_EINVAL, "internal: plain output asked of a transform without plain tables");
     const bool inverse = flags & MI_NTT_INVERSE, coset = flags & MI_NTT_COSET, dit = flags & MI_NTT_DIT;
     NttTables t{};
     t.small = inverse ? st->small_i : st->small_f;
@@ -449,8 +487,8 @@
     t.tw_64k = inverse ? st->tw64k_i : st->tw64k_f;
     u32 load_scale = 0, store_scale = 0;
     if (coset && !inverse) { t.sc_lo = st->g_lo; t.sc_hi = variant == 2 ? st->g_hi_n : st->g_hi; load_scale = dit ? 1 : 2; }
-    else if (coset && inverse) { t.sc_lo = st->gi_lo; t.sc_hi = variant == 3 ? st->gi_hi_nd : st->gi_hi; store_scale = dit ? 4 : 3; }
-    else if (inverse && variant != 1) { t.sc_lo = t.sc_hi = variant == 4 ? st->ninv_den : st->ninv; store_scale = 5; }
+    else if (coset && inverse) { t.sc_lo = st->gi_lo; t.sc_hi = variant == 3 ? (plain ? st->gi_hi_nd_plain : st->gi_hi_nd) : st->gi_hi; store_scale = dit ? 4 : 3; }
+    else if (inverse && variant != 1) { t.sc_lo = t.sc_hi = variant == 4 ? (plain ? st->ninv_den_plain : st->ninv_den) : st->ninv; store_scale = 5; }
     if (load_mul && (load_scale || dit)) MI_FAIL(ctx, MI_EINVAL, "internal: load_mul on a pass whose load side already has a factor");
 
     const NttKnobs kn = knobs_for(st, log_n);
@@ -480,7 +518,7 @@
         const bool direct = variant != 0 && st->d_log_n == log_n && st->d_sc_fwd;
         if (direct && p.twiddle && i == 0 && pl.n_pass > 1) p.tw_direct = inverse ? st->d_tw_inv : st->d_tw_fwd;
         if (direct && variant == 2 && p.scale == 1) p.sc_direct = st->d_sc_fwd;
-        if (direct && variant == 3 && p.scale == 3) p.sc_direct = st->d_sc_inv;
+        if (direct && variant == 3 && p.scale == 3) p.sc_direct = !plain ? st->d_sc_inv : st->dp_log_n == log_n ? st->d_sc_inv_plain : nullptr;
         const bool wave = p.log_r >= 7 && st->wave_stages;
         p.lds_pad = wave && p.log_s != 0 ? 1 : 0;
         if (((skip & 1) && step == 0) || ((skip & 2) && step == pl.n_pass - 1)) {
@@ -536,11 +574,13 @@
     }
     return MI_OK;
 }
-int32_t mi_compute_h_part(mi_ctx *ctx, uint32_t log_n, int part, const mi_fr *src, size_t n_constraints, mi_fr *h_out, const mi_fr *src2) {
+int32_t mi_compute_h_part(mi_ctx *ctx, uint32_t log_n, int part, const mi_fr *src, size_t n_constraints, mi_fr *h_out, const mi_fr *src2, bool plain_h) {
     static const char *const range_names[4] = {"mi.computeH.a.enqueue", "mi.computeH.b.enqueue", "mi.computeH.c.enqueue", "mi.computeH.last.enqueue"};
     const MiRange range(range_names[part & 3]);
     const size_t n = (size_t)1 << log_n;
     MI_TRY(ensure_direct(ctx, log_n));
+    const u32 pv = plain_h && part >= 2 ? NTT_PLAIN_OUT : 0u;
+    if (pv) MI_TRY(ensure_plain(ctx, log_n));
     MI_TRY(mi_reserve(ctx, ctx->ws[WS_H_B], n * sizeof(Fr)));
     MI_TRY(mi_reserve(ctx, ctx->ws[WS_H_C], n * sizeof(Fr)));
     Fr *A = (Fr *)h_out, *B = (Fr *)ctx->ws[WS_H_B].p, *C = (Fr *)ctx->ws[WS_H_C].p;
@@ -568,13 +608,13 @@
     if (part == 2) {
         NttPass px{};
         NttTables tx{};
-        return ntt_run(ctx, C, (const Fr *)src, (u32)n_constraints, log_n, MI_NTT_INVERSE, 4, (const Fr *)src2, nullptr, cp.last ? 2u : 0u, &px, &tx);
+        return ntt_run(ctx, C, (const Fr *)src, (u32)n_constraints, log_n, MI_NTT_INVERSE, 4 | pv, (const Fr *)src2, nullptr, cp.last ? 2u : 0u, &px, &tx);
     }
     auto last_fused = [&]() -> int32_t {
         NttPass pa{}, pcl{};
         NttTables ta{}, tcl{};
-        MI_TRY(ntt_run(ctx, C, C, (u32)n, log_n, MI_NTT_INVERSE, 4, nullptr, nullptr, 2 | 4, &pcl, &tcl));
-        MI_TRY(ntt_run(ctx, A, A, (u32)n, log_n, MI_NTT_INVERSE | MI_NTT_COSET, 3, nullptr, nullptr, 2 | 4, &pa, &ta));
+        MI_TRY(ntt_run(ctx, C, C, (u32)n, log_n, MI_NTT_INVERSE, 4 | pv, nullptr, nullptr, 2 | 4, &pcl, &tcl));
+        MI_TRY(ntt_run(ctx, A, A, (u32)n, log_n, MI_NTT_INVERSE | MI_NTT_COSET, 3 | pv, nullptr, nullptr, 2 | 4, &pa, &ta));
         if (pa.log_r != pcl.log_r || pa.log_c != pcl.log_c || pa.log_s || pcl.log_s || pa.dit || pcl.dit || pa.lds_pad != pcl.lds_pad)
             MI_FAIL(ctx, MI_EINVAL, "internal: the two last passes of computeH do not match");
         const u32 E = 1u << (pa.log_r + pa.log_c);
@@ -589,12 +629,14 @@
         if (count) {
             const size_t lds_bytes = (size_t)32 * ntt_plane_slots(pa) + (size_t)(E / MSM2_SLICE) * zs.ngroups * 4;
 #define MI_LAST_COUNT(CW) do { \
-            hipLaunchKernelGGL(k_ntt_contig_last_sub_count<CW>, dim3(1u << (log_n - pa.log_r - pa.log_c)), dim3(256), lds_bytes, ctx->stream, A, (const Fr *)C, pa, ta, pcl, tcl, zs, ctx->zhook.C1); } while (0)
+            if (pv) hipLaunchKernelGGL((k_ntt_contig_last_sub_count<CW, true>), dim3(1u << (log_n - pa.log_r - pa.log_c)), dim3(256), lds_bytes, ctx->stream, A, (const Fr *)C, pa, ta, pcl, tcl, zs, ctx->zhook.C1); \
+            else hipLaunchKernelGGL((k_ntt_contig_last_sub_count<CW, false>), dim3(1u << (log_n - pa.log_r - pa.log_c)), dim3(256), lds_bytes, ctx->stream, A, (const Fr *)C, pa, ta, pcl, tcl, zs, ctx->zhook.C1); } while (0)
             switch (zs.c) { case 17: MI_LAST_COUNT(17); break; case 18: MI_LAST_COUNT(18); break; case 19: MI_LAST_COUNT(19); break; case 20: MI_LAST_COUNT(20); break;
                             case 21: MI_LAST_COUNT(21); break; default: MI_LAST_COUNT(22); break; }
 #undef MI_LAST_COUNT
-            ctx->zhook.done = true; ctx->zhook.h = A;
+            ctx->zhook.done = true; ctx->zhook.h = A; ctx->zhook.plain = pv != 0;
             ctx->z_count_fused_launches++;
+            if (!pv) ctx->scalar_decodes += zs.n;
         } else {
             hipLaunchKernelGGL(k_ntt_contig_last_sub, dim3(1u << (log_n - pa.log_r - pa.log_c)), dim3(256), (size_t)32 * ntt_plane_slots(pa), ctx->stream, A, (const Fr *)C, pa, ta, pcl, tcl);
         }
@@ -603,10 +645,10 @@
         return MI_OK;
     };
     if (!cp.triple) {
-        if (!cp.last) return ntt_run(ctx, A, A, (u32)n, log_n, MI_NTT_INVERSE | MI_NTT_COSET, 3, B, C);
+        if (!cp.last) return ntt_run(ctx, A, A, (u32)n, log_n, MI_NTT_INVERSE | MI_NTT_COSET, 3 | pv, B, C);
         NttPass px{};
         NttTables tx{};
-        MI_TRY(ntt_run(ctx, A, A, (u32)n, log_n, MI_NTT_INVERSE | MI_NTT_COSET, 3, B, nullptr, 2, &px, &tx));
+        MI_TRY(ntt_run(ctx, A, A, (u32)n, log_n, MI_NTT_INVERSE | MI_NTT_COSET, 3 | pv, B, nullptr, 2, &px, &tx));
         return last_fused();
     }
     const NttPass &pc = cp.pc;
@@ -618,10 +660,10 @@
                            A, (const Fr *)B, pc, cp.tc, cp.plast, cp.tlast);
     MI_CHECK_HIP(ctx, hipGetLastError());
     ctx->stats.ntt_launches++;
-    if (!cp.last) return ntt_run(ctx, A, A, (u32)n, log_n, MI_NTT_INVERSE | MI_NTT_COSET, 3, nullptr, C, 1);
+    if (!cp.last) return ntt_run(ctx, A, A, (u32)n, log_n, MI_NTT_INVERSE | MI_NTT_COSET, 3 | pv, nullptr, C, 1);
     NttPass px{};
     NttTables tx{};
-    MI_TRY(ntt_run(ctx, A, A, (u32)n, log_n, MI_NTT_INVERSE | MI_NTT_COSET, 3, nullptr, nullptr, 1 | 2, &px, &tx));
+    MI_TRY(ntt_run(ctx, A, A, (u32)n, log_n, MI_NTT_INVERSE | MI_NTT_COSET, 3 | pv, nullptr, nullptr, 1 | 2, &px, &tx));
     return last_fused();
 }
 int32_t mi_compute_h_dev_impl(mi_ctx *ctx, uint32_t log_n, const mi_fr *a, const mi_fr *b, const mi_fr *c,
@@ -692,6 +734,16 @@
     MI_CHECK_HIP(ctx, hipEventSynchronize(ctx->ev[EV_T1]));
     MI_CHECK_HIP(ctx, hipEventElapsedTime(&ctx->stats.compute_h_ms, ctx->ev[EV_T0], ctx->ev[EV_T1]));
     ctx->stats.ntt_kernel_ms = ctx->stats.compute_h_ms;
+    return MI_OK;
+}
+int32_t mi_debug_compute_h_plain_dev(mi_ctx *ctx, uint32_t log_n, const mi_fr *a, const mi_fr *b, const mi_fr *c, size_t n_constraints, mi_fr *h_out) {
+    if (!ctx || !a || !b || !h_out || log_n > 28 || n_constraints > ((size_t)1 << log_n)) return MI_EINVAL;
+    stats_begin(ctx);
+    MI_TRY(mi_compute_h_part(ctx, log_n, 0, a, n_constraints, h_out));
+    MI_TRY(mi_compute_h_part(ctx, log_n, 1, b, n_constraints, h_out));
+    MI_TRY(mi_compute_h_part(ctx, log_n, 2, c ? c : a, n_constraints, h_out, c ? nullptr : b, true));
+    MI_TRY(mi_compute_h_part(ctx, log_n, 3, nullptr, n_constraints, h_out, nullptr, true));
+    MI_CHECK_HIP(ctx, hipStreamSynchronize(ctx->stream));
     return MI_OK;
 }
 int32_t mi_compute_h(mi_ctx *ctx, uint32_t log_n, const mi_fr *a, const mi_fr *b, const mi_fr *c,
diff --git a/gnark-whir_amd/csrc/prove.hip b/gnark-whir_amd/csrc/prove.hip
--- a/gnark-whir_amd/csrc/prove.hip
+++ b/gnark-whir_amd/csrc/prove.hip
@@ -12,6 +12,10 @@
 __global__ void k_gather_fr(Fr *out, const Fr *W, const u32 *idx, size_t n) {
     size_t i = (size_t)blockIdx.x * blockDim.x + threadIdx.x;
     if (i < n) out[i] = W[idx[i]];
+}
+__global__ void __launch_bounds__(256) k_fr_from_mont(Fr *out, const Fr *W, size_t n) {
+    size_t i = (size_t)blockIdx.x * blockDim.x + threadIdx.x;
+    if (i < n) out[i] = fe_from_mont(W[i]);
 }
 
 static size_t point_bytes(int curve) { return curve == 1 ? sizeof(G1Aff) : sizeof(G2Aff); }
@@ -284,9 +288,9 @@
 }
 
 static void arm_accum_gate(mi_ctx *ctx, int slot, const std::function<hipEvent_t()> *accum_gate) { ctx->msm[slot].accum_gate = accum_gate; }
-static int32_t enqueue_b_msms(mi_ctx *ctx, mi_pk *pk, const mi_fr *W, hipEvent_t ev_w, bool defer, const std::function<hipEvent_t()> *accum_gate) {
+static int32_t enqueue_b_msms(mi_ctx *ctx, mi_pk *pk, const mi_fr *W, hipEvent_t ev_w, bool defer, const std::function<hipEvent_t()> *accum_gate, uint32_t scalar_flags) {
     (void)hipSetDevice(ctx->dev);
-    const uint32_t fl = (defer ? MI_MSM_DEFER_REDUCE : 0) | MI_MSM_EXACT_SIZE | (pk->rprime ? MI_MSM_PTS_RPRIME : 0);
+    const uint32_t fl = (defer ? MI_MSM_DEFER_REDUCE : 0) | MI_MSM_EXACT_SIZE | (pk->rprime ? MI_MSM_PTS_RPRIME : 0) | scalar_flags;
     const KeyGroup &B = pk->group[KEY_B];
     MI_TRY(mi_reserve(ctx, ctx->ws[WS_B_WIRES], (B.n + 1) * sizeof(Fr)));
     hipStream_t st = ctx->msm[MSM_SLOT_B1].stream;
@@ -298,22 +302,22 @@
     arm_accum_gate(ctx, MSM_SLOT_B2, accum_gate);
     return mi_msm_enqueue(ctx, MSM_SLOT_B2, MSM_SLOT_B1, 2, B.bases[1].pts, nullptr, B.n, fl, nullptr, false, B.c, B.bases[1].stat_pairs);
 }
-static int32_t enqueue_ak_msms(mi_ctx *ctx, mi_pk *pk, const mi_fr *W, hipEvent_t ev_w, bool defer, const std::function<hipEvent_t()> *accum_gate) {
+static int32_t enqueue_ak_msms(mi_ctx *ctx, mi_pk *pk, const mi_fr *W, hipEvent_t ev_w, bool defer, const std::function<hipEvent_t()> *accum_gate, uint32_t scalar_flags) {
     (void)hipSetDevice(ctx->dev);
-    const uint32_t fl = (defer ? MI_MSM_DEFER_REDUCE : 0) | MI_MSM_EXACT_SIZE | (pk->rprime ? MI_MSM_PTS_RPRIME : 0);
+    const uint32_t fl = (defer ? MI_MSM_DEFER_REDUCE : 0) | MI_MSM_EXACT_SIZE | (pk->rprime ? MI_MSM_PTS_RPRIME : 0) | scalar_flags;
     const KeyGroup &AK = pk->group[KEY_AK];
     arm_accum_gate(ctx, MSM_SLOT_A, accum_gate);
     MI_TRY(mi_msm_enqueue(ctx, MSM_SLOT_A, -1, 1, AK.bases[0].pts, W, AK.n, fl, ev_w, true, AK.c, AK.bases[0].stat_pairs, AK.gen_c));
     arm_accum_gate(ctx, MSM_SLOT_K, accum_gate);
     return mi_msm_enqueue(ctx, MSM_SLOT_K, MSM_SLOT_A, 1, AK.bases[1].pts, nullptr, AK.n, fl, nullptr, false, AK.c, AK.bases[1].stat_pairs);
 }
-void WireMsms::start(mi_ctx *ctx, mi_pk *pk, const mi_fr *W, hipEvent_t ev_w, bool defer, const std::function<hipEvent_t()> *accum_gate) {
-    auto group = [&](std::future<int32_t> &f, int32_t (*enqueue)(mi_ctx *, mi_pk *, const mi_fr *, hipEvent_t, bool, const std::function<hipEvent_t()> *)) {
+void WireMsms::start(mi_ctx *ctx, mi_pk *pk, const mi_fr *W, hipEvent_t ev_w, bool defer, const std::function<hipEvent_t()> *accum_gate, uint32_t scalar_flags) {
+    auto group = [&](std::future<int32_t> &f, int32_t (*enqueue)(mi_ctx *, mi_pk *, const mi_fr *, hipEvent_t, bool, const std::function<hipEvent_t()> *, uint32_t)) {
         try {
-            f = std::async(std::launch::async, [=]() -> int32_t { try { return enqueue(ctx, pk, W, ev_w, defer, accum_gate); } catch (...) { return MI_ENOMEM; } });
+            f = std::async(std::launch::async, [=]() -> int32_t { try { return enqueue(ctx, pk, W, ev_w, defer, accum_gate, scalar_flags); } catch (...) { return MI_ENOMEM; } });
         } catch (...) {
             int32_t r = MI_ENOMEM;
-            try { r = enqueue(ctx, pk, W, ev_w, defer, nullptr); } catch (...) {}
+            try { r = enqueue(ctx, pk, W, ev_w, defer, nullptr, scalar_flags); } catch (...) {}
             if (rc_inline == MI_OK) rc_inline = r;
         }
     };
@@ -331,8 +335,8 @@
     wires.start(ctx, pk, W, ev_w, defer, nullptr);
     return wires.join();
 }
-int32_t mi_prove_enqueue_z_msm(mi_ctx *ctx, mi_pk *pk, const mi_fr *h, hipEvent_t ev_h, bool defer) {
-    const uint32_t fl = (defer ? MI_MSM_DEFER_REDUCE : 0) | (pk->rprime ? MI_MSM_PTS_RPRIME : 0);
+int32_t mi_prove_enqueue_z_msm(mi_ctx *ctx, mi_pk *pk, const mi_fr *h, hipEvent_t ev_h, bool defer, uint32_t scalar_flags) {
+    const uint32_t fl = (defer ? MI_MSM_DEFER_REDUCE : 0) | (pk->rprime ? MI_MSM_PTS_RPRIME : 0) | scalar_flags;
     const KeyGroup &Z = pk->group[KEY_Z];
     return mi_msm_enqueue(ctx, MSM_SLOT_Z, -1, 1, Z.bases[0].pts, h, Z.n, fl, ev_h, true, Z.c, Z.bases[0].stat_pairs, Z.gen_c);
 }
@@ -407,6 +411,8 @@
     MI_TRY(check_key_fits(ctx, pk, n_wires));
     if (n_constraints > N) MI_FAIL(ctx, MI_EINVAL, "prove: witness size does not match the proving key");
     std::memset(&ctx->stats, 0, sizeof(ctx->stats));
+    ctx->scalar_decodes = 0;
+    const bool once = ctx->scalars_once != 0;
     const auto t_begin = std::chrono::steady_clock::now();
     hipEvent_t *ev = ctx->ev;
     MI_TRY(mi_reserve(ctx, ctx->ws[WS_H], N * sizeof(Fr)));
@@ -451,20 +457,31 @@
         MI_CHECK_HIP(ctx, hipEventRecord(ev[EV_PROVE_BEGIN], ctx->stream));
         hipEvent_t ev_w = nullptr;
         MI_TRY(arrival.w_resident(&ev_w));
-        wires.start(ctx, pk, W, ev_w, false, hold ? &h_gate : nullptr);
+        const mi_fr *W_sort = W;
+        if (once && n_wires) {
+            MI_TRY(mi_reserve(ctx, ctx->ws[WS_W_CANON], n_wires * sizeof(Fr)));
+            hipStream_t sa = ctx->msm[MSM_SLOT_A].stream;
+            if (ev_w) MI_CHECK_HIP(ctx, hipStreamWaitEvent(sa, ev_w, 0));
+            hipLaunchKernelGGL(k_fr_from_mont, dim3((unsigned)((n_wires + 255) / 256)), dim3(256), 0, sa, (Fr *)ctx->ws[WS_W_CANON].p, (const Fr *)W, n_wires);
+            MI_CHECK_HIP(ctx, hipGetLastError());
+            MI_CHECK_HIP(ctx, hipEventRecord(ev[EV_W_CANON], sa));
+            ctx->scalar_decodes += n_wires;
+            W_sort = (const mi_fr *)ctx->ws[WS_W_CANON].p; ev_w = ev[EV_W_CANON];
+        }
+        wires.start(ctx, pk, W_sort, ev_w, false, hold ? &h_gate : nullptr, once && n_wires ? MI_MSM_SCALARS_CANONICAL : 0u);
         MI_TRY(arrival.make_abc(0));
         MI_TRY(mi_compute_h_part(ctx, pk->log_n, 0, abc[0], n_constraints, h));
         MI_TRY(arrival.make_abc(1));
         MI_TRY(mi_compute_h_part(ctx, pk->log_n, 1, abc[1], n_constraints, h));
-        if (derive_c) MI_TRY(mi_compute_h_part(ctx, pk->log_n, 2, abc[0], n_constraints, h, abc[1]));
-        else { MI_TRY(arrival.make_abc(2)); MI_TRY(mi_compute_h_part(ctx, pk->log_n, 2, abc[2], n_constraints, h)); }
+        if (derive_c) MI_TRY(mi_compute_h_part(ctx, pk->log_n, 2, abc[0], n_constraints, h, abc[1], once));
+        else { MI_TRY(arrival.make_abc(2)); MI_TRY(mi_compute_h_part(ctx, pk->log_n, 2, abc[2], n_constraints, h, nullptr, once)); }
         if (pk->group[KEY_Z].c) MI_TRY(mi_msm_z_count_arm(ctx, MSM_SLOT_Z, pk->n_z_msm, pk->group[KEY_Z].c));
-        const int32_t rc_h = mi_compute_h_part(ctx, pk->log_n, 3, nullptr, n_constraints, h);
+        const int32_t rc_h = mi_compute_h_part(ctx, pk->log_n, 3, nullptr, n_constraints, h, nullptr, once);
         ctx->zhook.armed = false;
         MI_TRY(rc_h);
         MI_CHECK_HIP(ctx, hipEventRecord(ev[EV_H_READY], ctx->stream));
         h_recorded.set_value(ev[EV_H_READY]); h_promised = true;
-        return mi_prove_enqueue_z_msm(ctx, pk, h, ev[EV_H_READY]);
+        return mi_prove_enqueue_z_msm(ctx, pk, h, ev[EV_H_READY], false, once ? MI_MSM_SCALARS_CANONICAL : 0u);
     };
     {
         int32_t rc = main_part();
@@ -512,6 +529,7 @@
     st.assemble_ms = ms(t_gpu_done, t_end);
     st.filter_ms = ms(t_asm0, t_gpu_done);
     st.total_ms = ms(t_begin, t_end);
+    st.scalar_decodes = ctx->scalar_decodes.load();
     if (stats) *stats = st;
     return MI_OK;
 }
diff --git a/gnark-whir_amd/csrc/prove_internal.h b/gnark-whir_amd/csrc/prove_internal.h
--- a/gnark-whir_amd/csrc/prove_internal.h
+++ b/gnark-whir_amd/csrc/prove_internal.h
@@ -41,11 +41,12 @@
 struct WireMsms {
     std::future<int32_t> f_b, f_ak;
     int32_t rc_inline = MI_OK;
-    void start(mi_ctx *ctx, mi_pk *pk, const mi_fr *W_dev, hipEvent_t ev_w, bool defer_reduce, const std::function<hipEvent_t()> *accum_gate);
+    void start(mi_ctx *ctx, mi_pk *pk, const mi_fr *W_dev, hipEvent_t ev_w, bool defer_reduce, const std::function<hipEvent_t()> *accum_gate, uint32_t scalar_flags = 0);
     int32_t join();
 };
 int32_t mi_prove_enqueue_wire_msms(mi_ctx *ctx, mi_pk *pk, const mi_fr *W_dev, hipEvent_t ev_w, bool defer_reduce = false);
-int32_t mi_prove_enqueue_z_msm(mi_ctx *ctx, mi_pk *pk, const mi_fr *h_dev, hipEvent_t ev_h, bool defer_reduce = false);
+int32_t mi_prove_enqueue_z_msm(mi_ctx *ctx, mi_pk *pk, const mi_fr *h_dev, hipEvent_t ev_h, bool defer_reduce = false,
+                               uint32_t scalar_flags = 0 );
 
 int32_t mi_groth16_prove_dev_gated(mi_ctx *ctx, mi_pk *pk, const mi_fr *W_dev, size_t n_wires, const mi_fr *a_dev, const mi_fr *b_dev, const mi_fr *c_dev,
                                    size_t n_constraints, const mi_fr *r, const mi_fr *s, mi_proof_out *out, mi_stats *stats,
diff --git a/include/mi355x_groth16.h b/include/mi355x_groth16.h
--- a/include/mi355x_groth16.h
+++ b/include/mi355x_groth16.h
@@ -66,6 +66,7 @@
     uint32_t ntt_launches;
     uint64_t g1_accum_entries;
     uint64_t g1_level1_additions;
+    uint64_t scalar_decodes;
 } mi_stats;
 
 int32_t mi_init(int device_id, mi_ctx **out);
diff --git a/include/mi355x_groth16_debug.h b/include/mi355x_groth16_debug.h
--- a/include/mi355x_groth16_debug.h
+++ b/include/mi355x_groth16_debug.h
@@ -68,6 +68,8 @@
 int32_t mi_debug_set_msm_precompute_batched(mi_ctx *ctx, uint32_t on);
 int32_t mi_debug_set_knob(mi_ctx *ctx, const char *name, int64_t value);
 int32_t mi_debug_get_counter(mi_ctx *ctx, const char *name, uint64_t *out);
+int32_t mi_debug_compute_h_plain_dev(mi_ctx *ctx, uint32_t log_n, const mi_fr *a_dev, const mi_fr *b_dev, const mi_fr *c_dev_or_null, size_t n_constraints,
+                                     mi_fr *h_out_dev);
 int32_t mi_debug_set_stream_plan(int32_t plan);
 int32_t mi_debug_set_trace_ranges(int32_t on);
 int32_t mi_debug_inject_hip_failure(int32_t nth);
```

After: 33.54, median of 6. No clear change (+0.4%).
